# vita-epfl/collaborative-gan-sampling

Measured on AMD Instinct MI355X. Metric: refined samples/sec @ 20 refinement steps, higher is better.
Workload: dtype f32; 1 GPU; dcgan64 collaborative refinement (propose + K-step refine + render), batch 1024/GPU, K=20, momentum rate 0.1, refine at feature [8, 8, 256], random-init weights, z~U(-1,1) seed 2019+rank; global_batch=1024, refine_steps=20, parallelism=single GPU, hipgraph=True, batches_in_flight=2, fused_per_launch=1, sync_bn=False, contraction=f32

## Files before the change

collaborative-gan-sampling_amd/csrc/api.hip:

```cpp
#include <stdarg.h>
#include <stdio.h>

#include "cgs_internal.h"

static thread_local char g_err[512] = "";
static thread_local const char* g_last_kernel = "";

static thread_local double g_last_flops = 0.0;
static thread_local int g_last_tail[2] = {0, 0};
void cgs_note_tail(int tiles, int split) { g_last_tail[0] = tiles; g_last_tail[1] = split; }
static thread_local int g_contraction = CGS_CONTRACTION_F32;
int cgs_contraction_mode() { return g_contraction; }

void cgs_note_kernel(const char* name) { g_last_kernel = name; }
void cgs_note_flops(double f) { g_last_flops = f; }
void cgs_add_flops(double f) { g_last_flops += f; }

int cgs_set_error(int code, const char* fmt, ...) {
    va_list ap;
    va_start(ap, fmt);
    vsnprintf(g_err, sizeof(g_err), fmt, ap);
    va_end(ap);
    return code;
}

extern "C" {

int cgs_version(void) { return 116; }
const char* cgs_last_error(void) { return g_err; }
const char* cgs_last_kernel(void) { return g_last_kernel; }
double cgs_last_executed_flops(void) { return g_last_flops; }
int cgs_last_tail_tiles(void) { return g_last_tail[0]; }
int cgs_last_tail_split(void) { return g_last_tail[1]; }
int cgs_set_contraction(int mode) {
    if (mode < CGS_CONTRACTION_F32 || mode > CGS_CONTRACTION_BX6_ALL) return cgs_set_error(CGS_EINVAL, "set_contraction: mode %d", mode);
    g_contraction = mode;
    return CGS_OK;
}
int cgs_get_contraction(void) { return g_contraction; }

}

struct ConvCall { CgsLayer L; bool dirT, deconv, bwd; };

static ConvCall conv_call_of(int op, int H, int W, int Cin, int Ho, int Wo, int Cout, int kh, int kw, int sh, int sw) {
    ConvCall c;
    c.deconv = (op == CGS_DECONV_FWD || op == CGS_DECONV_BWD_DATA);
    c.bwd = (op == CGS_CONV_BWD_DATA || op == CGS_DECONV_BWD_DATA);
    c.dirT = (op == CGS_CONV_BWD_DATA || op == CGS_DECONV_FWD);
    CgsLayer& L = c.L;
    L.kh = kh; L.kw = kw; L.sh = sh; L.sw = sw;
    if (!c.deconv) { L.Hb = H; L.Wb = W; L.Cb = Cin; L.Hs = cgs_ceil_div(H, sh > 0 ? sh : 1); L.Ws = cgs_ceil_div(W, sw > 0 ? sw : 1); L.Cs = Cout; }
    else { L.Hs = H; L.Ws = W; L.Cs = Cin; L.Hb = Ho; L.Wb = Wo; L.Cb = Cout; }
    return c;
}

static int check_layer(const CgsLayer& L, const char* who) {
    if (L.kh <= 0 || L.kw <= 0 || L.sh <= 0 || L.sw <= 0 || L.Hb <= 0 || L.Wb <= 0 || L.Cb <= 0 || L.Cs <= 0)
        return cgs_set_error(CGS_EINVAL, "%s: non-positive dimension", who);
    if (L.Hs != cgs_ceil_div(L.Hb, L.sh) || L.Ws != cgs_ceil_div(L.Wb, L.sw))
        return cgs_set_error(CGS_EINVAL, "%s: 'SAME' geometry mismatch: big %dx%d stride %dx%d needs small %dx%d, got %dx%d", who,
                             L.Hb, L.Wb, L.sh, L.sw, cgs_ceil_div(L.Hb, L.sh), cgs_ceil_div(L.Wb, L.sw), L.Hs, L.Ws);
    return CGS_OK;
}

static IgemmParams igemm_geometry(const CgsLayer& L, bool dirT, int B, int epilogue) {
    IgemmParams p{};
    p.B = B; p.epilogue = epilogue;
    if (!dirT) cgs_geom_F(L, p);
    else if (L.sh <= 2 && L.sw <= 2) cgs_geom_T(L, p);
    return p;
}

static size_t in_image_floats(const IgemmParams& p) { return (size_t)p.Hin * p.Win * p.Cred; }
static size_t out_image_floats(const IgemmParams& p) { return (size_t)p.Hout * p.Wout * p.N; }
static size_t images_per_launch(const IgemmParams& p) {
    const size_t in_img = in_image_floats(p) * 4, out_img = out_image_floats(p) * 4;
    return 0x7fffffffUL / (in_img > out_img ? in_img : out_img);
}
static bool whole_batch_in_one_launch(const IgemmParams& p) { return images_per_launch(p) >= (size_t)p.B; }

static bool smalln_ok(const CgsLayer& L, int epilogue) {
    return L.Cb <= 4 && L.sh == 2 && L.sw == 2 && L.Hb == 2 * L.Hs && L.Wb == 2 * L.Ws && (L.Cs % 4) == 0 &&
           epilogue != CGS_EPI_AFFINE_RELU;
}

static int choose_family(const CgsLayer& L, bool dirT, const IgemmParams& g, bool have_ws, size_t ws_bytes, bool in_al, bool ws_al,
                         bool rest_al) {
    const int B = g.B, epilogue = g.epilogue;
    if (dirT && smalln_ok(L, epilogue)) {
        if ((L.Cs % 16) == 0 && have_ws && cgs_convt_quad_fits(L)) return CGS_FAMILY_QUAD;
        if (epilogue < CGS_EPI_RELU_BWD_AFFINE) return CGS_FAMILY_SMALLN_T;
    }
    if (!dirT && cgs_conv_smalln_f_ok(L, B, epilogue) && have_ws && ws_bytes >= cgs_conv_smalln_f_ws_floats(L) * sizeof(float) &&
        in_al && ws_al)
        return CGS_FAMILY_SMALLN_F;
    if (!dirT && cgs_conv_taps_ok(L, epilogue)) return CGS_FAMILY_TAPS;
    if (!dirT && cgs_conv_dot_ok(L, epilogue) && in_al) return CGS_FAMILY_DOT;
    const bool patch_f = !dirT && cgs_conv_patch_ok(L, epilogue), patch_t = dirT && cgs_conv_patch_T_ok(L);
    if ((patch_f || patch_t) && have_ws && ws_bytes >= cgs_conv_patch_ws_floats(L, dirT) * sizeof(float) && ws_al && rest_al)
        return CGS_FAMILY_PATCH;
    if (g_contraction != CGS_CONTRACTION_F32 && cgs_igemm_bx6_ok(L, dirT, B, g_contraction == CGS_CONTRACTION_BX6_ALL)) {
        if (have_ws && ws_bytes >= cgs_igemm_bx6_packed_bytes(g)) return CGS_FAMILY_IGEMM_BX6;
    }
    return CGS_FAMILY_IGEMM;
}

static int planned_family(const ConvCall& c, const IgemmParams& g, size_t ws_bytes) { return choose_family(c.L, c.dirT, g, ws_bytes > 0, ws_bytes, true, true, true); }

struct NsArgs { const float *mean, *invstd, *gamma, *beta; float leak; int group_images; };

enum ConvForm { FORM_PLAIN, FORM_STATS, FORM_NSTATS, FORM_SIGNS };
struct ConvExtras {
    ConvForm form = FORM_PLAIN;
    float* stat_part = nullptr; size_t stat_part_bytes = 0;
    NsArgs ns = {};
    unsigned* sign_out = nullptr; const unsigned* aux_signs = nullptr;
};

static int run_dir(const ConvCall& c, int B, const float* in, const float* w, const float* bias, float* out, int epilogue,
                   const float* ep_a, const float* ep_b, const float* ep_aux, void* ws, size_t ws_bytes, int prepacked, hipStream_t s,
                   const char* who, const ConvExtras& x) {
    const CgsLayer& L = c.L;
    const bool dirT = c.dirT, nstats = x.form == FORM_NSTATS;
    cgs_note_flops(0.0);
    cgs_note_tail(0, 0);
    if (B <= 0) return cgs_set_error(CGS_EINVAL, "%s: B=%d", who, B);
    if (!in || !w || !out) return cgs_set_error(CGS_EINVAL, "%s: null tensor", who);
    if (epilogue < CGS_EPI_NONE || epilogue > CGS_EPI_TANH_BWD) return cgs_set_error(CGS_EINVAL, "%s: epilogue %d", who, epilogue);
    if (epilogue == CGS_EPI_AFFINE_RELU && (!ep_a || !ep_b)) return cgs_set_error(CGS_EINVAL, "%s: affine epilogue needs a,b", who);
    if (epilogue >= CGS_EPI_RELU_BWD_AFFINE && ((!ep_aux && !x.aux_signs) || (epilogue == CGS_EPI_RELU_BWD_AFFINE && !ep_a)))
        return cgs_set_error(CGS_EINVAL, "%s: backward epilogue %d needs aux%s", who, epilogue, epilogue == CGS_EPI_RELU_BWD_AFFINE ? " and a" : "");
    if (dirT && (L.sh > 2 || L.sw > 2)) return cgs_set_error(CGS_EINVAL, "%s: transposed direction supports stride <= 2", who);
    const bool rest_al = !(((uintptr_t)out & 15) || ((uintptr_t)bias & 15) || ((uintptr_t)ep_a & 15) || ((uintptr_t)ep_b & 15) ||
                           ((uintptr_t)ep_aux & 15));
    IgemmParams p = igemm_geometry(L, dirT, B, epilogue);
    const int fam = choose_family(L, dirT, p, ws != nullptr, ws_bytes, !((uintptr_t)in & 15), !((uintptr_t)ws & 15), rest_al);
    if (x.stat_part && fam != CGS_FAMILY_IGEMM && fam != CGS_FAMILY_IGEMM_BX6) return cgs_set_error(CGS_EINVAL, "%s: fused statistics are an implicit-GEMM feature (see cgs_conv_stat_partials)", who);
    if (nstats && (!x.stat_part || fam != CGS_FAMILY_IGEMM)) return cgs_set_error(CGS_EINVAL, "%s: norm-backward statistics are a feature of the exact-fp32 implicit GEMM (see cgs_conv_stat_layout)", who);
    if (x.sign_out && fam != CGS_FAMILY_IGEMM && fam != CGS_FAMILY_IGEMM_BX6) return cgs_set_error(CGS_EINVAL, "%s: this call cannot leave a sign mask (see cgs_conv_signs_ok)", who);
    if (x.aux_signs && fam != CGS_FAMILY_PATCH && fam != CGS_FAMILY_TAPS) return cgs_set_error(CGS_EINVAL, "%s: this call cannot take a sign mask (see cgs_conv_signs_ok)", who);
    if (((uintptr_t)x.sign_out & 3) || ((uintptr_t)x.aux_signs & 3)) return cgs_set_error(CGS_EINVAL, "%s: sign mask must be 4-byte aligned", who);
    switch (fam) {
        case CGS_FAMILY_QUAD:
            return cgs_convt_quad_launch(L, B, in, w, bias, out, epilogue, ep_a, ep_aux, (float*)ws, ws_bytes, prepacked, s);
        case CGS_FAMILY_SMALLN_T:
            return cgs_convt_smalln_launch(L, B, in, w, bias, out, epilogue, s);
        case CGS_FAMILY_SMALLN_F:
            return cgs_conv_smalln_f_launch(L, B, in, w, bias, out, epilogue, (float*)ws, ws_bytes, prepacked, s);
        case CGS_FAMILY_DOT:
            return cgs_conv_dot_launch(L, B, in, w, bias, out, epilogue, ep_a, ep_b, s);
        case CGS_FAMILY_TAPS:
            return cgs_conv_taps_launch(L, B, in, w, bias, out, epilogue, ep_a, ep_b, ep_aux, x.aux_signs, s);
        case CGS_FAMILY_PATCH:
            return cgs_conv_patch_launch(L, dirT, B, in, w, bias, out, epilogue, ep_a, ep_b, ep_aux, (float*)ws, ws_bytes, prepacked, s, x.aux_signs);
        default: break;
    }
    p.in = in; p.bias = bias; p.ep_a = ep_a; p.ep_b = ep_b; p.ep_aux = ep_aux; p.out = out;
    p.stat_part = x.stat_part;
    if (nstats) { p.ns_mean = x.ns.mean; p.ns_inv = x.ns.invstd; p.ns_gamma = x.ns.gamma; p.ns_beta = x.ns.beta; p.ns_leak = x.ns.leak; p.ns_gimg = x.ns.group_images >= B ? 0 : x.ns.group_images; }
    p.sign_out = x.sign_out;
    p.sign_plane = (long)B * (dirT ? L.Hb * L.Wb : L.Hs * L.Ws);
    const bool bx6 = fam == CGS_FAMILY_IGEMM_BX6;
    const size_t need = bx6 ? cgs_igemm_bx6_packed_bytes(p) : cgs_packed_floats(p) * sizeof(float);
    if (!ws || ws_bytes < need) return cgs_set_error(CGS_EWORKSPACE, "%s: workspace %zu < %zu bytes", who, ws_bytes, need);
    if (((uintptr_t)ws & 15) || ((uintptr_t)in & 15) || ((uintptr_t)out & 15) || ((uintptr_t)bias & 15) ||
        ((uintptr_t)ep_a & 15) || ((uintptr_t)ep_b & 15) || ((uintptr_t)ep_aux & 15))
        return cgs_set_error(CGS_EINVAL, "%s: pointers must be 16-byte aligned", who);
    p.wp = (const float*)ws;
    if (!prepacked) {
        int rc = bx6 ? cgs_pack_weights_bx6(p, L, dirT, w, ws, s) : cgs_pack_weights(p, L, dirT, w, (float*)ws, s);
        if (rc) return rc;
    }
    const size_t chunk = images_per_launch(p), in_img = in_image_floats(p), out_img = out_image_floats(p);
    if (chunk < 1) return cgs_set_error(CGS_EINVAL, "%s: one image exceeds 2 GiB", who);
    if (x.stat_part && !whole_batch_in_one_launch(p)) return cgs_set_error(CGS_EINVAL, "%s: fused statistics need the batch in one launch", who);
    for (size_t b0 = 0; b0 < (size_t)B; b0 += chunk) {
        p.B = (int)(B - b0 < chunk ? B - b0 : chunk);
        p.in = in + b0 * in_img;
        p.out = out + b0 * out_img;
        p.ep_aux = ep_aux ? ep_aux + b0 * out_img : nullptr;
        p.sign_out = x.sign_out ? x.sign_out + b0 * p.Hout * p.Wout : nullptr;
        int rc = bx6 ? cgs_igemm_bx6_launch(p, s) : cgs_igemm_launch(p, (char*)ws + need, ws_bytes - need, s);
        if (rc) return rc;
    }
    return CGS_OK;
}

struct ConvPlan { int fam; ConvCall c; IgemmParams g; };

static ConvPlan conv_plan_of(int op, int B, int H, int W, int Cin, int Ho, int Wo, int Cout, int kh, int kw, int sh, int sw, int epilogue,
                             size_t ws_bytes) {
    ConvPlan q{};
    if (op < CGS_CONV_FWD || op > CGS_DECONV_BWD_DATA || B <= 0 || H <= 0 || W <= 0 || Cin <= 0 || Cout <= 0 || kh <= 0 || kw <= 0 ||
        sh <= 0 || sw <= 0) {
        q.fam = cgs_set_error(CGS_EINVAL, "conv_family: bad argument");
    } else {
        q.c = conv_call_of(op, H, W, Cin, Ho, Wo, Cout, kh, kw, sh, sw);
        q.g = igemm_geometry(q.c.L, q.c.dirT, B, epilogue);
        q.fam = planned_family(q.c, q.g, ws_bytes);
    }
    return q;
}

static int nstats_check(const char* who, const float* x_norm, const NsArgs& ns, const float* stat_part) {
    if (!x_norm || !ns.mean || !ns.invstd || !ns.gamma || !ns.beta) return cgs_set_error(CGS_EINVAL, "%s: null statistics argument", who);
    if (((uintptr_t)x_norm | (uintptr_t)ns.mean | (uintptr_t)ns.invstd | (uintptr_t)ns.gamma | (uintptr_t)ns.beta | (uintptr_t)stat_part) & 15)
        return cgs_set_error(CGS_EINVAL, "%s: pointers must be 16-byte aligned", who);
    return CGS_OK;
}

static int conv_entry(const char* who, int op, const float* in, const float* w, const float* bias, float* out, int B, int H, int W, int Cin,
                      int Ho, int Wo, int Cout, int kh, int kw, int sh, int sw, int epilogue, const float* ep_a, const float* ep_b,
                      const float* ep_aux, void* ws, size_t ws_bytes, int prepacked, void* stream, const ConvExtras& x = ConvExtras()) {
    const ConvCall c = conv_call_of(op, H, W, Cin, Ho, Wo, Cout, kh, kw, sh, sw);
    if (x.form == FORM_SIGNS) {
        if (!x.sign_out && !x.aux_signs) return cgs_set_error(CGS_EINVAL, "%s: null sign mask", who);
        if (!cgs_conv_signs_ok(op, B, H, W, Cin, Ho, Wo, Cout, kh, kw, sh, sw, epilogue, ws_bytes))
            return cgs_set_error(CGS_EINVAL, "%s: not available for this call (cgs_conv_signs_ok == 0)", who);
    }
    if (x.form == FORM_PLAIN && c.bwd && epilogue != CGS_EPI_NONE && epilogue < CGS_EPI_RELU_BWD_AFFINE)
        return cgs_set_error(CGS_EINVAL, "%s: epilogue %d", who, epilogue);
    int rc = check_layer(c.L, who);
    if (rc) return rc;
    if (x.form == FORM_STATS || x.form == FORM_NSTATS) {
        const bool conv_fwd = x.form == FORM_STATS && !c.deconv;
        int a, b, d;
        const int G = conv_fwd ? cgs_conv_stat_partials(B, H, W, Cin, Cout, kh, kw, sh, sw, ws_bytes)
                               : cgs_conv_stat_layout(op, B, H, W, Cin, Ho, Wo, Cout, kh, kw, sh, sw, x.form == FORM_NSTATS ? x.ns.group_images : B,
                                                      ws_bytes, &a, &b, &d);
        if (G == 0) return cgs_set_error(CGS_EINVAL, "%s: not available for this call (%s == 0)", who, conv_fwd ? "cgs_conv_stat_partials" : "cgs_conv_stat_layout");
        if (x.form == FORM_NSTATS && (rc = nstats_check(who, ep_aux, x.ns, x.stat_part))) return rc;
        const size_t need = (size_t)G * 2 * (c.bwd ? Cin : Cout) * sizeof(float);
        if (!x.stat_part || x.stat_part_bytes < need) return cgs_set_error(CGS_EWORKSPACE, "%s: partials buffer %zu < %zu bytes", who, x.stat_part_bytes, need);
        if ((uintptr_t)x.stat_part & 15) return cgs_set_error(CGS_EINVAL, "%s: partials buffer must be 16-byte aligned", who);
    }
    return run_dir(c, B, in, w, bias, out, epilogue, ep_a, ep_b, ep_aux, ws, ws_bytes, prepacked, (hipStream_t)stream, who, x);
}

extern "C" {

size_t cgs_conv_ws_bytes(int op, int kh, int kw, int sh, int sw, int Cin, int Cout) {
    if (kh <= 0 || kw <= 0 || sh <= 0 || sw <= 0 || Cin <= 0 || Cout <= 0) return 0;
    const ConvCall c = conv_call_of(op, 0, 0, Cin, 0, 0, Cout, kh, kw, sh, sw);
    const int Cb = c.L.Cb, Cs = c.L.Cs;
    const bool dirT = c.dirT;
    const int Cred = dirT ? Cs : Cb, Nn = dirT ? Cb : Cs;
    const size_t per_w = ((Cred % 32) == 0 && (Nn % 64) == 0 && kh <= 16 && kw <= 16) ? 6 : sizeof(float);
    if (!dirT) return (size_t)cgs_round_up(kh * kw * Cb, CGS_BK) * cgs_round_up(Cs, 64) * per_w;
    size_t n = 0;
    for (int a = 0; a < sh; ++a)
        for (int b = 0; b < sw; ++b) {
            const int nty = a < kh ? (kh - a + sh - 1) / sh : 0, ntx = b < kw ? (kw - b + sw - 1) / sw : 0;
            n += (size_t)cgs_round_up(nty * ntx * Cs, CGS_BK) * cgs_round_up(Cb, 64);
        }
    if (Cb <= 4 && sh == 2 && sw == 2) {
        const size_t q = cgs_convt_quad_ws_floats_bound(kh, kw, Cs);
        if (q > n) n = q;
    }
    return n * (per_w > sizeof(float) && !(Cb <= 4 && sh == 2 && sw == 2) ? per_w : sizeof(float));
}

size_t cgs_conv_ws_bytes_for(int op, int B, int H, int W, int Cin, int Cout, int kh, int kw, int sh, int sw) {
    const size_t packed = cgs_conv_ws_bytes(op, kh, kw, sh, sw, Cin, Cout);
    if (B <= 0 || H <= 0 || W <= 0 || packed == 0) return packed;
    const ConvCall c = conv_call_of(op, H, W, Cin, H * sh, W * sw, Cout, kh, kw, sh, sw);
    if (c.dirT && (sh > 2 || sw > 2)) return packed;
    return packed + cgs_igemm_slab_bytes(igemm_geometry(c.L, c.dirT, B, CGS_EPI_NONE));
}

int cgs_conv_family(int op, int B, int H, int W, int Cin, int Ho, int Wo, int Cout, int kh, int kw, int sh, int sw, int epilogue,
                    size_t ws_bytes) {
    return conv_plan_of(op, B, H, W, Cin, Ho, Wo, Cout, kh, kw, sh, sw, epilogue, ws_bytes).fam;
}

int cgs_conv_stat_partials(int B, int H, int W, int Cin, int Cout, int kh, int kw, int sh, int sw, size_t ws_bytes) {
    const ConvCall c = conv_call_of(CGS_CONV_FWD, H, W, Cin, 0, 0, Cout, kh, kw, sh, sw);
    if (check_layer(c.L, "conv_stat_partials")) return 0;
    const IgemmParams g = igemm_geometry(c.L, c.dirT, B, CGS_EPI_NONE);
    const int fam = planned_family(c, g, ws_bytes);
    if (B <= 0 || (Cout & 3) || (fam != CGS_FAMILY_IGEMM && fam != CGS_FAMILY_IGEMM_BX6)) return 0;
    if (!whole_batch_in_one_launch(g)) return 0;
    const long M = (long)B * c.L.Hs * c.L.Ws;
    return (int)(2 * ((M + 127) / 128));
}

int cgs_conv_stat_layout(int op, int B, int H, int W, int Cin, int Ho, int Wo, int Cout, int kh, int kw, int sh, int sw, int group_images,
                         size_t ws_bytes, int* rows_per_seg, int* nseg, int* seg_stride) {
    if (op < CGS_CONV_FWD || op > CGS_DECONV_BWD_DATA || B <= 0 || group_images <= 0 || (B % group_images) || !rows_per_seg || !nseg || !seg_stride)
        return 0;
    const ConvCall c = conv_call_of(op, H, W, Cin, Ho, Wo, Cout, kh, kw, sh, sw);
    if ((c.bwd ? Cin : Cout) & 3) return 0;
    if (check_layer(c.L, "conv_stat_layout")) return 0;
    if (c.dirT && (sh > 2 || sw > 2)) return 0;
    const IgemmParams p = igemm_geometry(c.L, c.dirT, B, CGS_EPI_NONE);
    const int fam = planned_family(c, p, ws_bytes);
    if (fam != CGS_FAMILY_IGEMM && (c.bwd || fam != CGS_FAMILY_IGEMM_BX6)) return 0;
    if (!whole_batch_in_one_launch(p)) return 0;
    const int RC = p.cls[0].R * p.cls[0].C;
    for (int i = 1; i < p.nclasses; ++i)
        if (p.cls[i].R * p.cls[i].C != RC) return 0;
    if (RC <= 0) return 0;
    const long M = (long)B * RC;
    const long cls_rows = 2 * ((M + 127) / 128);
    if (cls_rows * p.nclasses > 0x7fffffffL) return 0;
    if (group_images == B) {
        *rows_per_seg = (int)(cls_rows * p.nclasses); *nseg = 1; *seg_stride = 0;
        return (int)(cls_rows * p.nclasses);
    }
    const int order = cgs_igemm_row_order(p);
    if (order == 0) {
        if (((long)group_images * RC) % 64) return 0;
        *rows_per_seg = (int)((long)group_images * RC / 64); *nseg = p.nclasses; *seg_stride = (int)cls_rows;
    } else if (order == 2) {
        if (group_images % 64) return 0;
        *rows_per_seg = group_images / 64; *nseg = p.nclasses * RC; *seg_stride = B / 64;
    } else {
        return 0;
    }
    return (int)(cls_rows * p.nclasses);
}

int cgs_conv_signs_ok(int op, int B, int H, int W, int Cin, int Ho, int Wo, int Cout, int kh, int kw, int sh, int sw, int epilogue,
                      size_t ws_bytes) {
    const ConvPlan q = conv_plan_of(op, B, H, W, Cin, Ho, Wo, Cout, kh, kw, sh, sw, epilogue, ws_bytes);
    const int fam = q.fam;
    if (fam < 0) return 0;
    if (epilogue >= CGS_EPI_RELU_BWD_AFFINE)
        return (fam == CGS_FAMILY_PATCH && cgs_conv_patch_signs_ok(q.c.L, q.c.dirT, epilogue)) || (fam == CGS_FAMILY_TAPS && cgs_conv_taps_signs_ok(q.c.L, epilogue));
    if (fam == CGS_FAMILY_IGEMM_BX6)
        return (epilogue == CGS_EPI_AFFINE_RELU || epilogue == CGS_EPI_LRELU) && whole_batch_in_one_launch(q.g);
    if (fam != CGS_FAMILY_IGEMM || (q.c.dirT && (sh > 2 || sw > 2))) return 0;
    if (!whole_batch_in_one_launch(q.g)) return 0;
    return cgs_igemm_signs_ok(q.g);
}

int cgs_conv2d_nhwc_fwd(const float* x, const float* w, const float* bias, float* y, int B, int H, int W, int Cin,
                        int Cout, int kh, int kw, int sh, int sw, int epilogue, const float* ep_a, const float* ep_b,
                        void* ws, size_t ws_bytes, int ws_prepacked, void* stream) {
    return conv_entry("conv2d_nhwc_fwd", CGS_CONV_FWD, x, w, bias, y, B, H, W, Cin, 0, 0, Cout, kh, kw, sh, sw, epilogue, ep_a, ep_b, nullptr, ws, ws_bytes,
                      ws_prepacked, stream);
}

int cgs_conv2d_nhwc_bwd_data(const float* dy, const float* w, float* dx, int B, int H, int W, int Cin, int Cout, int kh,
                             int kw, int sh, int sw, int epilogue, const float* ep_a, const float* ep_aux, void* ws,
                             size_t ws_bytes, int ws_prepacked, void* stream) {
    return conv_entry("conv2d_nhwc_bwd_data", CGS_CONV_BWD_DATA, dy, w, nullptr, dx, B, H, W, Cin, 0, 0, Cout, kh, kw, sh, sw, epilogue, ep_a, nullptr, ep_aux, ws,
                      ws_bytes, ws_prepacked, stream);
}

int cgs_deconv2d_nhwc_fwd(const float* x, const float* w, const float* bias, float* y, int B, int H, int W, int Cin,
                          int Ho, int Wo, int Cout, int kh, int kw, int sh, int sw, int epilogue, const float* ep_a,
                          const float* ep_b, void* ws, size_t ws_bytes, int ws_prepacked, void* stream) {
    return conv_entry("deconv2d_nhwc_fwd", CGS_DECONV_FWD, x, w, bias, y, B, H, W, Cin, Ho, Wo, Cout, kh, kw, sh, sw, epilogue, ep_a, ep_b, nullptr, ws, ws_bytes,
                      ws_prepacked, stream);
}

int cgs_deconv2d_nhwc_bwd_data(const float* dy, const float* w, float* dx, int B, int H, int W, int Cin, int Ho, int Wo,
                               int Cout, int kh, int kw, int sh, int sw, int epilogue, const float* ep_a,
                               const float* ep_aux, void* ws, size_t ws_bytes, int ws_prepacked, void* stream) {
    return conv_entry("deconv2d_nhwc_bwd_data", CGS_DECONV_BWD_DATA, dy, w, nullptr, dx, B, H, W, Cin, Ho, Wo, Cout, kh, kw, sh, sw, epilogue, ep_a, nullptr, ep_aux,
                      ws, ws_bytes, ws_prepacked, stream);
}

int cgs_conv2d_nhwc_fwd_stats(const float* x, const float* w, const float* bias, float* y, int B, int H, int W, int Cin,
                              int Cout, int kh, int kw, int sh, int sw, void* ws, size_t ws_bytes, int ws_prepacked,
                              float* stat_part, size_t stat_part_bytes, void* stream) {
    return conv_entry("conv2d_nhwc_fwd_stats", CGS_CONV_FWD, x, w, bias, y, B, H, W, Cin, 0, 0, Cout, kh, kw, sh, sw, CGS_EPI_NONE, nullptr, nullptr, nullptr, ws,
                      ws_bytes, ws_prepacked, stream, ConvExtras{FORM_STATS, stat_part, stat_part_bytes});
}

int cgs_deconv2d_nhwc_fwd_stats(const float* x, const float* w, const float* bias, float* y, int B, int H, int W, int Cin, int Ho, int Wo,
                                int Cout, int kh, int kw, int sh, int sw, void* ws, size_t ws_bytes, int ws_prepacked, float* stat_part,
                                size_t stat_part_bytes, void* stream) {
    return conv_entry("deconv2d_nhwc_fwd_stats", CGS_DECONV_FWD, x, w, bias, y, B, H, W, Cin, Ho, Wo, Cout, kh, kw, sh, sw, CGS_EPI_NONE, nullptr, nullptr, nullptr,
                      ws, ws_bytes, ws_prepacked, stream, ConvExtras{FORM_STATS, stat_part, stat_part_bytes});
}

int cgs_conv2d_nhwc_bwd_data_nstats(const float* dy, const float* w, float* dx, int B, int H, int W, int Cin, int Cout, int kh, int kw, int sh,
                                    int sw, const float* x_norm, const float* mean, const float* invstd, const float* gamma, const float* beta,
                                    float leak, int group_images, void* ws, size_t ws_bytes, int ws_prepacked, float* stat_part,
                                    size_t stat_part_bytes, void* stream) {
    return conv_entry("conv2d_nhwc_bwd_data_nstats", CGS_CONV_BWD_DATA, dy, w, nullptr, dx, B, H, W, Cin, 0, 0, Cout, kh, kw, sh, sw, CGS_EPI_NONE, nullptr, nullptr,
                      x_norm, ws, ws_bytes, ws_prepacked, stream, ConvExtras{FORM_NSTATS, stat_part, stat_part_bytes, NsArgs{mean, invstd, gamma, beta, leak,
                      group_images}});
}

int cgs_deconv2d_nhwc_bwd_data_nstats(const float* dy, const float* w, float* dx, int B, int H, int W, int Cin, int Ho, int Wo, int Cout, int kh,
                                      int kw, int sh, int sw, const float* x_norm, const float* mean, const float* invstd, const float* gamma,
                                      const float* beta, float leak, int group_images, void* ws, size_t ws_bytes, int ws_prepacked,
                                      float* stat_part, size_t stat_part_bytes, void* stream) {
    return conv_entry("deconv2d_nhwc_bwd_data_nstats", CGS_DECONV_BWD_DATA, dy, w, nullptr, dx, B, H, W, Cin, Ho, Wo, Cout, kh, kw, sh, sw, CGS_EPI_NONE, nullptr,
                      nullptr, x_norm, ws, ws_bytes, ws_prepacked, stream, ConvExtras{FORM_NSTATS, stat_part, stat_part_bytes, NsArgs{mean, invstd, gamma, beta,
                      leak, group_images}});
}

int cgs_deconv2d_nhwc_fwd_signs(const float* x, const float* w, const float* bias, float* y, int B, int H, int W, int Cin,
                                int Ho, int Wo, int Cout, int kh, int kw, int sh, int sw, int epilogue, const float* ep_a,
                                const float* ep_b, unsigned* signs, void* ws, size_t ws_bytes, int ws_prepacked, void* stream) {
    return conv_entry("deconv2d_nhwc_fwd_signs", CGS_DECONV_FWD, x, w, bias, y, B, H, W, Cin, Ho, Wo, Cout, kh, kw, sh, sw, epilogue, ep_a, ep_b, nullptr, ws,
                      ws_bytes, ws_prepacked, stream, ConvExtras{FORM_SIGNS, nullptr, 0, NsArgs{}, signs, nullptr});
}

int cgs_deconv2d_nhwc_bwd_data_signs(const float* dy, const float* w, float* dx, int B, int H, int W, int Cin, int Ho, int Wo,
                                     int Cout, int kh, int kw, int sh, int sw, int epilogue, const float* ep_a,
                                     const unsigned* aux_signs, void* ws, size_t ws_bytes, int ws_prepacked, void* stream) {
    return conv_entry("deconv2d_nhwc_bwd_data_signs", CGS_DECONV_BWD_DATA, dy, w, nullptr, dx, B, H, W, Cin, Ho, Wo, Cout, kh, kw, sh, sw, epilogue, ep_a, nullptr,
                      nullptr, ws, ws_bytes, ws_prepacked, stream, ConvExtras{FORM_SIGNS, nullptr, 0, NsArgs{}, nullptr, aux_signs});
}

}

__global__ __launch_bounds__(256) void linear_out1_fwd_kernel(const float* __restrict__ x, const float* __restrict__ w,
                                                              const float* __restrict__ bias, float* __restrict__ y,
                                                              int B, int K, int epilogue) {
    const int b = blockIdx.x * 4 + (threadIdx.x >> 6);
    const int lane = threadIdx.x & 63;
    if (b >= B) return;
    const float* row = x + (size_t)b * K;
    float s = 0.f;
    if ((K & 3) == 0) {
        for (int k = lane * 4; k < K; k += 256) {
            const float4 a = *(const float4*)(row + k), ww = *(const float4*)(w + k);
            s = fmaf(a.x, ww.x, s); s = fmaf(a.y, ww.y, s); s = fmaf(a.z, ww.z, s); s = fmaf(a.w, ww.w, s);
        }
    } else {
        for (int k = lane; k < K; k += 64) s = fmaf(row[k], w[k], s);
    }
#pragma unroll
    for (int off = 32; off > 0; off >>= 1) s += __shfl_down(s, off, 64);
    if (lane == 0) {
        float v = s + (bias ? bias[0] : 0.f);
        if (epilogue == CGS_EPI_LRELU) v = fmaxf(v, 0.2f * v);
        y[b] = v;
    }
}

template <int KIND, bool LADAM>
__device__ __forceinline__ void linear_out1_seed_body(const float* __restrict__ x, const float* __restrict__ w, const float* __restrict__ bias,
                                                      float* __restrict__ y, float* __restrict__ dl, float* __restrict__ lm, int B, int K,
                                                      const cgs_ladam_seed& la) {
    const int b = blockIdx.x * 4 + (threadIdx.x >> 6);
    const int lane = threadIdx.x & 63;
    if (b >= B) return;
    const float* row = x + (size_t)b * K;
    float s = 0.f;
    if ((K & 3) == 0) {
        for (int k = lane * 4; k < K; k += 256) {
            const float4 a = *(const float4*)(row + k), ww = *(const float4*)(w + k);
            s = fmaf(a.x, ww.x, s); s = fmaf(a.y, ww.y, s); s = fmaf(a.z, ww.z, s); s = fmaf(a.w, ww.w, s);
        }
    } else {
        for (int k = lane; k < K; k += 64) s = fmaf(row[k], w[k], s);
    }
#pragma unroll
    for (int off = 32; off > 0; off >>= 1) s += __shfl_down(s, off, 64);
    if (lane == 0) {
        const float v = s + (bias ? bias[0] : 0.f);
        y[b] = v;
        dl[b] = loss_seed1<KIND>(v);
        lm[b] = v;
        if (LADAM) ladam_seed1(la, b, sigmoid_stable(v));
    }
}

__global__ __launch_bounds__(256) void linear_out1_bce_kernel(const float* __restrict__ x, const float* __restrict__ w, const float* __restrict__ bias,
                                                              float* __restrict__ y, float* __restrict__ dl, float* __restrict__ lm, int B, int K) {
    linear_out1_seed_body<CGS_LOSS_BCE, false>(x, w, bias, y, dl, lm, B, K, cgs_ladam_seed{});
}

template <int KIND, bool LADAM>
__global__ __launch_bounds__(256) void linear_out1_seed_kernel(const float* __restrict__ x, const float* __restrict__ w, const float* __restrict__ bias,
                                                               float* __restrict__ y, float* __restrict__ dl, float* __restrict__ lm, int B, int K,
                                                               cgs_ladam_seed la) {
    linear_out1_seed_body<KIND, LADAM>(x, w, bias, y, dl, lm, B, K, la);
}

// ... 66 lines not shown
```

collaborative-gan-sampling_amd/csrc/cgs_internal.h:

```cpp
#pragma once
#include <hip/hip_runtime.h>
#include <stddef.h>
#include <stdint.h>

#include "cgs_hip.h"

int cgs_set_error(int code, const char* fmt, ...);
void cgs_note_kernel(const char* name);
void cgs_note_flops(double executed);
void cgs_add_flops(double executed);
void cgs_note_tail(int tiles, int split);

#define CGS_CHECK_LAUNCH(name)                                                        \
    do {                                                                              \
        hipError_t e_ = hipGetLastError();                                            \
        if (e_ != hipSuccess) return cgs_set_error(CGS_ELAUNCH, "%s: %s", name, hipGetErrorString(e_)); \
    } while (0)

static inline int cgs_ceil_div(int a, int b) { return (a + b - 1) / b; }
static inline int cgs_round_up(int a, int b) { return cgs_ceil_div(a, b) * b; }

static inline int cgs_same_pad_before(int size, int k, int s) {
    int out = cgs_ceil_div(size, s);
    int tot = (out - 1) * s + k - size;
    if (tot < 0) tot = 0;
    return tot / 2;
}

struct CgsLayer {
    int kh, kw, sh, sw;
    int Hb, Wb, Cb, Hs, Ws, Cs;
};

#define CGS_BN_MAX_BLOCKS 512
size_t cgs_bn_stat2_offset(int C);
size_t cgs_instnorm_stat2_offset(int B, int HW, int C);
#define CGS_BK 32
#define CGS_MAX_CLASSES 4

struct IgemmClass {
    int R, C;
    int py, px;
    int nty, ntx;
    int dy0, dx0;
    int ky0, kx0;
    int K;
    int w_off;
    int slab_off;
};

struct IgemmParams {
    const float* in;
    const float* wp;
    const float* bias;
    const float* ep_a;
    const float* ep_b;
    const float* ep_aux;
    float* out;
    int B, Hin, Win, Cred;
    int Hout, Wout, N, Np;
    int S, So, dstep, kstep;
    int epilogue;
    int pix_major;
    int splitk;
    float* slab;
    int tap_parity;
    int xcd_map;
    int cls_flip;
    int uni;
    int lpt;
    unsigned* sign_out;
    long sign_plane;
    float* stat_part;
    int stat_cls_rows;
    const float* ns_mean = nullptr;
    const float* ns_inv = nullptr;
    const float* ns_gamma = nullptr;
    const float* ns_beta = nullptr;
    float ns_leak = 1.f;
    int ns_gimg = 0;
    int vec;
    int prio_t[3];
    int tail_from, tail_n, tail_s;
    int nclasses;
    IgemmClass cls[CGS_MAX_CLASSES];
    unsigned char perm[CGS_MAX_CLASSES][256];
};

__host__ __device__ inline int cgs_tap_order(int i, int n, int parity_first) {
    if (!parity_first) return i;
    const int ne = (n + 1) >> 1;
    return i < ne ? 2 * i : 2 * (i - ne) + 1;
}

void cgs_geom_F(const CgsLayer& L, IgemmParams& p);
void cgs_geom_T(const CgsLayer& L, IgemmParams& p);
size_t cgs_packed_floats(const IgemmParams& p);

int cgs_pack_weights(const IgemmParams& p, const CgsLayer& L, bool dirT, const float* w, float* packed, hipStream_t s);
int cgs_igemm_launch(const IgemmParams& p, void* slab, size_t slab_bytes, hipStream_t s);
size_t cgs_igemm_splitk_bytes(const IgemmParams& p);
size_t cgs_igemm_slab_bytes(const IgemmParams& p);
void cgs_igemm_row_policy(IgemmParams& p, int BM);
void cgs_igemm_count_flops(const IgemmParams& p, int BM);
int cgs_igemm_bx6_ok(const CgsLayer& L, bool dirT, int B, bool any_size);
size_t cgs_igemm_bx6_packed_bytes(const IgemmParams& p);
int cgs_pack_weights_bx6(const IgemmParams& p, const CgsLayer& L, bool dirT, const float* w, void* packed, hipStream_t s);
int cgs_igemm_bx6_launch(const IgemmParams& p, hipStream_t s);
int cgs_contraction_mode();
int cgs_igemm_row_order(const IgemmParams& p);
size_t cgs_convt_quad_ws_floats_bound(int kh, int kw, int Cs);
int cgs_convt_taps_ok(const CgsLayer& L);
int cgs_convt_taps_launch(const CgsLayer& L, int B, const float* in, const float* w, const float* bias, float* out, int epilogue,
                          const float* ep_a, const float* ep_aux, hipStream_t s);
int cgs_conv_dot_ok(const CgsLayer& L, int epilogue);
int cgs_conv_dot_launch(const CgsLayer& L, int B, const float* in, const float* w, const float* bias, float* out, int epilogue,
                        const float* ep_a, const float* ep_b, hipStream_t s);
int cgs_conv_taps_ok(const CgsLayer& L, int epilogue);
int cgs_conv_taps_signs_ok(const CgsLayer& L, int epilogue);
int cgs_conv_taps_launch(const CgsLayer& L, int B, const float* in, const float* w, const float* bias, float* out, int epilogue,
                         const float* ep_a, const float* ep_b, const float* ep_aux, const unsigned* aux_signs, hipStream_t s);
int cgs_convt_quad_launch(const CgsLayer& L, int B, const float* in, const float* w, const float* bias, float* out,
                          int epilogue, const float* ep_a, const float* ep_aux, float* ws, size_t ws_bytes, int prepacked,
                          hipStream_t s);
int cgs_convt_smalln_launch(const CgsLayer& L, int B, const float* in, const float* w, const float* bias,
                            float* out, int epilogue, hipStream_t s);

#ifdef __HIPCC__
__device__ __forceinline__ float epilogue_apply(float v, int mode, float a, float b, float aux) {
    switch (mode) {
        case CGS_EPI_LRELU: return fmaxf(v, 0.2f * v);
        case CGS_EPI_AFFINE_RELU: return fmaxf(fmaf(a, v, b), 0.f);
        case CGS_EPI_TANH: return tanhf(v);
        case CGS_EPI_RELU_BWD_AFFINE: return aux > 0.f ? v * a : 0.f;
        case CGS_EPI_LRELU_BWD: return aux > 0.f ? v : 0.2f * v;
        case CGS_EPI_TANH_BWD: return v * (1.f - aux * aux);
        default: return v;
    }
}

__device__ __forceinline__ float norm_fwd1(float x, float sc, float sh, float leak) {
    const float o = fmaf(x, sc, sh);
    return o > 0.f ? o : leak * o;
}
__device__ __forceinline__ float norm_d1(float x, float dy, float sc, float sh, float leak) {
    const float u = fmaf(x, sc, sh);
    return dy * (u > 0.f ? 1.f : leak);
}
__device__ __forceinline__ float norm_d_acc1(float x, float dy, float mu, float inv, float sc, float sh, float leak, float& sa, float& sb) {
    const float d = norm_d1(x, dy, sc, sh, leak);
    sa += d; sb = fmaf(d, (x - mu) * inv, sb);
    return d;
}
__device__ __forceinline__ float norm_dx1(float x, float d, float mu, float inv, float sc, float m1, float m2) {
    const float xh = (x - mu) * inv;
    return sc * (d - m1 - xh * m2);
}

__device__ __forceinline__ float sigmoid_stable(float v) { return v >= 0.f ? 1.f / (1.f + expf(-v)) : expf(v) / (1.f + expf(v)); }
template <int KIND>
__device__ __forceinline__ float loss_seed1(float v) {
    if (KIND == CGS_LOSS_BCE) return v >= 0.f ? -expf(-v) / (1.f + expf(-v)) : -1.f / (1.f + expf(v));
    if (KIND == CGS_LOSS_LSQ) return 2.f * (v - 1.f);
    return -1.f;
}
__device__ __forceinline__ void ladam_seed1(const cgs_ladam_seed& la, int b, float sig, const float* loss_in = nullptr) {
#pragma clang fp contract(off)
    const float loss = loss_in ? loss_in[b] : la.s_real[0] - sig;
    const float avg = la.first ? loss : 0.5f * la.loss_avg[b] + 0.5f * loss;
    la.loss_avg[b] = avg;
    const float c = fminf(fmaxf(avg + 0.5f, 0.f), 10000.f);
    la.gain[b] = c * c;
}
#endif


#define CGS_SMEM_ATTR(bytes, who, ...)                                                                                  \
    do {                                                                                                                \
        static bool smem_done_[64] = {};                                                                                \
        int smem_dev_ = 0;                                                                                              \
        (void)hipGetDevice(&smem_dev_);                                                                                 \
        smem_dev_ &= 63;                                                                                                \
        if (!smem_done_[smem_dev_]) {                                                                                   \
            hipError_t smem_e_ = hipFuncSetAttribute((const void*)(__VA_ARGS__), hipFuncAttributeMaxDynamicSharedMemorySize, (int)(bytes)); \
            if (smem_e_ != hipSuccess) return cgs_set_error(CGS_ELAUNCH, "%s: MaxDynamicSharedMemorySize: %s", who, hipGetErrorString(smem_e_)); \
            smem_done_[smem_dev_] = true;                                                                               \
        }                                                                                                               \
    } while (0)

int cgs_mlp2d_wide_saliency(const float* const* w, const float* const* b, int nlayers, int nh, const float* x, float* sig, float* sal, int B,
                            float inv_batch, hipStream_t st);
int cgs_refine2d_wide(const float* const* w, const float* const* b, int nlayers, int nh, const float* x, float mean_host,
                      const float* mean_dev, float inv_batch, int steps, float rate, int method, float* best_x, float* best_step,
                      float* traj, int B, hipStream_t st);
size_t cgs_mlp2d_wide_train_ws(int Bt, int nlayers, int nh);
int cgs_mlp2d_wide_train(float* const* w, float* const* b, int nlayers, int nh, const float* real, int B_real, const float* fake, int B_fake,
                         float lr, float* const* gw, float* const* gb, float* loss, void* ws, hipStream_t st);

bool cgs_convt_quad_fits(const CgsLayer& L);
int cgs_conv_smalln_f_ok(const CgsLayer& L, int B, int epilogue);
size_t cgs_conv_smalln_f_ws_floats(const CgsLayer& L);
int cgs_conv_smalln_f_launch(const CgsLayer& L, int B, const float* in, const float* w, const float* bias, float* out,
                             int epilogue, float* ws, size_t ws_bytes, int prepacked, hipStream_t s);
int cgs_conv_patch_ok(const CgsLayer& L, int epilogue);
int cgs_conv_patch_T_ok(const CgsLayer& L);
size_t cgs_conv_patch_ws_floats(const CgsLayer& L, bool dirT);
int cgs_conv_patch_launch(const CgsLayer& L, bool dirT, int B, const float* in, const float* w, const float* bias, float* out,
                          int epilogue, const float* ep_a, const float* ep_b, const float* ep_aux, float* ws, size_t ws_bytes,
                          int prepacked, hipStream_t s, const unsigned* aux_signs = nullptr);
int cgs_conv_patch_signs_ok(const CgsLayer& L, bool dirT, int epilogue);
int cgs_igemm_signs_ok(const IgemmParams& p);
```

collaborative-gan-sampling_amd/csrc/elementwise.hip:

```cpp
#include "cgs_internal.h"

static unsigned ew_blocks(size_t n) {
    size_t b = (n + 255) / 256;
    if (b > 8192) b = 8192;
    if (b == 0) b = 1;
    return (unsigned)b;
}

#define GRID_STRIDE(i, n) for (size_t i = (size_t)blockIdx.x * blockDim.x + threadIdx.x; i < (n); i += (size_t)gridDim.x * blockDim.x)

__global__ void bn_fold_kernel(const float* g, const float* b, const float* mm, const float* mv, float eps, float* a,
                               float* bo, int C) {
    const int c = blockIdx.x * blockDim.x + threadIdx.x;
    if (c >= C) return;
    const float s = g[c] / sqrtf(mv[c] + eps);
    a[c] = s; bo[c] = b[c] - s * mm[c];
}

int cgs_bn_fold(const float* gamma, const float* beta, const float* mm, const float* mv, float eps, float* a, float* b,
                int C, void* stream) {
    if (C <= 0) return cgs_set_error(CGS_EINVAL, "bn_fold: C=%d", C);
    hipLaunchKernelGGL(bn_fold_kernel, dim3(cgs_ceil_div(C, 128)), dim3(128), 0, (hipStream_t)stream, gamma, beta, mm, mv, eps, a, b, C);
    CGS_CHECK_LAUNCH("bn_fold");
    return CGS_OK;
// ... 188 lines not shown
    float s = 0.f;
    for (int i = lane; i < P; i += 64) s += sigmoid_stable(l[(size_t)b * P + i]);
#pragma unroll
    for (int o = 32; o > 0; o >>= 1) s += __shfl_xor(s, o);
    if (lane == 0) sig[b] = s / (float)P;
}

int cgs_sigmoid_rowmean(const float* logits, float* sigmoids, int B, int P, void* stream) {
    if (B <= 0 || P <= 0) return cgs_set_error(CGS_EINVAL, "sigmoid_rowmean: B=%d P=%d", B, P);
    if (P >= 64)
        hipLaunchKernelGGL(sigmoid_rowmean_wave_kernel, dim3(cgs_ceil_div(B, 4)), dim3(256), 0, (hipStream_t)stream, logits, sigmoids, B, P);
    else
        hipLaunchKernelGGL(sigmoid_rowmean_kernel, dim3(cgs_ceil_div(B, 128)), dim3(128), 0, (hipStream_t)stream, logits, sigmoids, B, P);
    CGS_CHECK_LAUNCH("sigmoid_rowmean");
    return CGS_OK;
}

template <int OP>
__global__ __launch_bounds__(256) void loss_unary_kernel(const float* __restrict__ p0, const float* __restrict__ p1, float lo, float hi,
                                                         float* __restrict__ o, size_t n) {
    GRID_STRIDE(i, n) {
        float r;
        if (OP == 0) { const float v = p0[i]; r = fmaxf(-v, 0.f) + log1pf(expf(-fabsf(v))); }
        else if (OP == 1) { const float v = p1[i]; r = p0[i] * (v >= 0.f ? -expf(-v) / (1.f + expf(-v)) : -1.f / (1.f + expf(v))); }
        else r = fminf(fmaxf(p0[i], lo), hi);
        o[i] = r;
    }
}

int cgs_bce_ones_fwd(const float* logits, float* loss, size_t n, void* stream) {
    if (n == 0) return CGS_OK;
    hipLaunchKernelGGL(loss_unary_kernel<0>, dim3(ew_blocks(n)), dim3(256), 0, (hipStream_t)stream, logits, nullptr, 0.f, 0.f, loss, n);
    CGS_CHECK_LAUNCH("bce_ones_fwd");
    return CGS_OK;
}

int cgs_bce_ones_bwd(const float* dloss, const float* logits, float* dlogits, size_t n, void* stream) {
    if (n == 0) return CGS_OK;
    hipLaunchKernelGGL(loss_unary_kernel<1>, dim3(ew_blocks(n)), dim3(256), 0, (hipStream_t)stream, dloss, logits, 0.f, 0.f, dlogits, n);
    CGS_CHECK_LAUNCH("bce_ones_bwd");
    return CGS_OK;
}

template <int KIND>
__global__ __launch_bounds__(256) void gan_loss_kernel(const float* __restrict__ l, float target, const float* __restrict__ dloss,
                                                       float* __restrict__ o, size_t n) {
#pragma clang fp contract(off)
    GRID_STRIDE(i, n) {
        const float v = l[i];
        float e, d;
        if (KIND == CGS_LOSS_LSQ) { const float r = v - target; e = r * r; d = 2.f * r; }
        else if (KIND == CGS_LOSS_HINGE) {
            const float u = target > 0.5f ? 1.f - v : 1.f + v;
            e = fmaxf(u, 0.f);
            d = u > 0.f ? (target > 0.5f ? -1.f : 1.f) : 0.f;
        } else { e = -v; d = -1.f; }
        o[i] = dloss ? dloss[i] * d : e;
    }
}

int cgs_gan_loss(const float* logits, int kind, float target, const float* dloss, float* out, size_t n, void* stream) {
    if (n == 0) return CGS_OK;
    if (!logits || !out) return cgs_set_error(CGS_EINVAL, "gan_loss: null pointer");
    const hipStream_t st = (hipStream_t)stream;
    if (kind == CGS_LOSS_LSQ) hipLaunchKernelGGL(gan_loss_kernel<CGS_LOSS_LSQ>, dim3(ew_blocks(n)), dim3(256), 0, st, logits, target, dloss, out, n);
    else if (kind == CGS_LOSS_HINGE && (target == 0.f || target == 1.f))
        hipLaunchKernelGGL(gan_loss_kernel<CGS_LOSS_HINGE>, dim3(ew_blocks(n)), dim3(256), 0, st, logits, target, dloss, out, n);
    else if (kind == CGS_LOSS_LINEAR) hipLaunchKernelGGL(gan_loss_kernel<CGS_LOSS_LINEAR>, dim3(ew_blocks(n)), dim3(256), 0, st, logits, target, dloss, out, n);
    else return cgs_set_error(CGS_EINVAL, "gan_loss: kind %d target %g", kind, (double)target);
    CGS_CHECK_LAUNCH("gan_loss");
    return CGS_OK;
}

int cgs_clip(const float* x, float vmin, float vmax, float* y, size_t n, void* stream) {
    if (n == 0) return CGS_OK;
    hipLaunchKernelGGL(loss_unary_kernel<2>, dim3(ew_blocks(n)), dim3(256), 0, (hipStream_t)stream, x, nullptr, vmin, vmax, y, n);
    CGS_CHECK_LAUNCH("clip");
    return CGS_OK;
}

__global__ __launch_bounds__(256) void refine_update_kernel(float* __restrict__ theta, float* __restrict__ m,
                                                            const float* __restrict__ g, float rate, float alpha,
                                                            int first, int use_clip, float vmin, float vmax, size_t n) {
#pragma clang fp contract(off)
    GRID_STRIDE(i, n) {
        const float lg = rate * g[i];
        const float am = alpha * m[i];
        const float mv = first ? lg : am + lg;
        m[i] = mv;
        float t = theta[i] - mv;
        if (use_clip) t = fminf(fmaxf(t, vmin), vmax);
        theta[i] = t;
    }
}

int cgs_refine_update(float* theta, float* m, const float* g, float rate, float alpha, int first, int use_clip,
                      float vmin, float vmax, size_t n, void* stream) {
    if (n == 0) return CGS_OK;
    hipLaunchKernelGGL(refine_update_kernel, dim3(ew_blocks(n)), dim3(256), 0, (hipStream_t)stream, theta, m, g, rate, alpha, first, use_clip, vmin, vmax, n);
    CGS_CHECK_LAUNCH("refine_update");
    return CGS_OK;
}

__global__ void ladam_gain_kernel(const float* __restrict__ loss, cgs_ladam_seed la, int B) {
    const int b = blockIdx.x * blockDim.x + threadIdx.x;
    if (b < B) ladam_seed1(la, b, 0.f, loss);
}

int cgs_ladam_gain(const float* loss, float* loss_avg, float* gain, int first, int B, void* stream) {
    if (B <= 0 || !loss || !loss_avg || !gain) return cgs_set_error(CGS_EINVAL, "ladam_gain: B=%d or a null pointer", B);
    hipLaunchKernelGGL(ladam_gain_kernel, dim3(cgs_ceil_div(B, 128)), dim3(128), 0, (hipStream_t)stream, loss, cgs_ladam_seed{nullptr, loss_avg, gain, first}, B);
    CGS_CHECK_LAUNCH("ladam_gain");
    return CGS_OK;
}

__device__ __forceinline__ void ladam_update1(float& th, float& m, float& v, float g, float gain, float rate, float c1, float c2, int first,
                                              int use_clip, float vmin, float vmax) {
#pragma clang fp contract(off)
    const float sq = g * g;
    const float mm = first ? g : 0.9f * m + c1 * g;
    const float vv = first ? sq : 0.5f * v + c2 * sq;
    m = mm; v = vv;
    const float dir = rate * mm / (sqrtf(vv) + 1e-8f);
    float t = th - dir * gain;
    if (use_clip) t = fminf(fmaxf(t, vmin), vmax);
    th = t;
}

template <bool VEC>
__global__ __launch_bounds__(256) void refine_update_ladam_kernel(float* __restrict__ theta, float* __restrict__ m, float* __restrict__ v,
                                                                  const float* __restrict__ g, const float* __restrict__ gain, float rate,
                                                                  float c1, float c2, int first, int use_clip, float vmin, float vmax,
                                                                  size_t n, int F) {
    if (VEC) {
        float4* t4 = (float4*)theta; float4* m4 = (float4*)m; float4* v4 = (float4*)v;
        const float4* g4 = (const float4*)g;
        GRID_STRIDE(i, n >> 2) {
            const float gn = gain[(i << 2) / (size_t)F];
            float4 t = t4[i], mm = first ? float4{0.f, 0.f, 0.f, 0.f} : m4[i], vv = first ? float4{0.f, 0.f, 0.f, 0.f} : v4[i];
            const float4 gg = g4[i];
            ladam_update1(t.x, mm.x, vv.x, gg.x, gn, rate, c1, c2, first, use_clip, vmin, vmax);
            ladam_update1(t.y, mm.y, vv.y, gg.y, gn, rate, c1, c2, first, use_clip, vmin, vmax);
            ladam_update1(t.z, mm.z, vv.z, gg.z, gn, rate, c1, c2, first, use_clip, vmin, vmax);
            ladam_update1(t.w, mm.w, vv.w, gg.w, gn, rate, c1, c2, first, use_clip, vmin, vmax);
            t4[i] = t; m4[i] = mm; v4[i] = vv;
        }
    } else {
        GRID_STRIDE(i, n) {
            float t = theta[i], mm = first ? 0.f : m[i], vv = first ? 0.f : v[i];
            ladam_update1(t, mm, vv, g[i], gain[i / (size_t)F], rate, c1, c2, first, use_clip, vmin, vmax);
            theta[i] = t; m[i] = mm; v[i] = vv;
        }
    }
}

int cgs_refine_update_ladam(float* theta, float* m, float* v, const float* g, const float* gain, float rate, int first, int use_clip,
                            float vmin, float vmax, int B, int F, void* stream) {
    if (B <= 0 || F <= 0 || !theta || !m || !v || !g || !gain) return cgs_set_error(CGS_EINVAL, "refine_update_ladam: B=%d F=%d or a null pointer", B, F);
    const size_t n = (size_t)B * F;
    const float c1 = (float)(1.0 - 0.9), c2 = (float)(1.0 - 0.5);
    const bool vec = (F & 3) == 0 && (((uintptr_t)theta | (uintptr_t)m | (uintptr_t)v | (uintptr_t)g) & 15) == 0;
    if (vec)
        hipLaunchKernelGGL(refine_update_ladam_kernel<true>, dim3(ew_blocks(n >> 2)), dim3(256), 0, (hipStream_t)stream, theta, m, v, g, gain, rate, c1, c2,
                           first, use_clip, vmin, vmax, n, F);
    else
        hipLaunchKernelGGL(refine_update_ladam_kernel<false>, dim3(ew_blocks(n)), dim3(256), 0, (hipStream_t)stream, theta, m, v, g, gain, rate, c1, c2,
                           first, use_clip, vmin, vmax, n, F);
    CGS_CHECK_LAUNCH("refine_update_ladam");
    return CGS_OK;
}

__device__ __forceinline__ void copy_row(const float* __restrict__ src, float* __restrict__ dst, int F, bool vec4) {
    const int t = blockIdx.x * blockDim.x + threadIdx.x, nt = gridDim.x * blockDim.x;
    if (vec4) {
// ... 95 lines not shown
```

collaborative-gan-sampling_amd/csrc/igemm.hip:

```cpp
#include <stdarg.h>
#include <stdio.h>

#include "cgs_internal.h"
#include "igemm_epilogue.h"

typedef float f32x16 __attribute__((ext_vector_type(16)));

static constexpr int BK = CGS_BK;

void cgs_geom_F(const CgsLayer& L, IgemmParams& p) {
    p.Hin = L.Hb; p.Win = L.Wb; p.Cred = L.Cb;
    p.Hout = L.Hs; p.Wout = L.Ws; p.N = L.Cs; p.Np = cgs_round_up(L.Cs, 64);
    p.S = L.sh; p.So = 1; p.dstep = 1; p.kstep = 1; p.nclasses = 1;
    p.tap_parity = (L.sh == 2 && L.sw == 2 && L.Hs * L.Ws > 64) ? 1 : 0;
    IgemmClass& c = p.cls[0];
    c.R = L.Hs; c.C = L.Ws; c.py = 0; c.px = 0; c.nty = L.kh; c.ntx = L.kw;
    c.dy0 = -cgs_same_pad_before(L.Hb, L.kh, L.sh); c.dx0 = -cgs_same_pad_before(L.Wb, L.kw, L.sw);
    c.ky0 = 0; c.kx0 = 0; c.K = L.kh * L.kw * L.Cb; c.w_off = 0;
    p.vec = (p.Cred % BK) == 0 && c.nty <= 16 && c.ntx <= 16;
}

void cgs_geom_T(const CgsLayer& L, IgemmParams& p) {
    p.Hin = L.Hs; p.Win = L.Ws; p.Cred = L.Cs;
    p.Hout = L.Hb; p.Wout = L.Wb; p.N = L.Cb; p.Np = cgs_round_up(L.Cb, 64);
    p.S = 1; p.So = L.sh; p.dstep = -1; p.kstep = L.sh; p.nclasses = L.sh * L.sw;
    p.tap_parity = 0;
    const int pt = cgs_same_pad_before(L.Hb, L.kh, L.sh), pl = cgs_same_pad_before(L.Wb, L.kw, L.sw);
    int off = 0;
    for (int py = 0; py < L.sh; ++py)
        for (int px = 0; px < L.sw; ++px) {
            IgemmClass& c = p.cls[py * L.sw + px];
            c.py = py; c.px = px;
            c.R = py < L.Hb ? (L.Hb - py + L.sh - 1) / L.sh : 0;
            c.C = px < L.Wb ? (L.Wb - px + L.sw - 1) / L.sw : 0;
            c.ky0 = (py + pt) % L.sh; c.kx0 = (px + pl) % L.sw;
            c.nty = c.ky0 < L.kh ? (L.kh - c.ky0 + L.sh - 1) / L.sh : 0;
            c.ntx = c.kx0 < L.kw ? (L.kw - c.kx0 + L.sw - 1) / L.sw : 0;
            c.dy0 = (py + pt - c.ky0) / L.sh; c.dx0 = (px + pl - c.kx0) / L.sw;
            c.K = c.nty * c.ntx * L.Cs; c.w_off = off;
            off += cgs_round_up(c.K, BK) * p.Np;
        }
    p.vec = (p.Cred % BK) == 0;
    for (int i = 0; i < p.nclasses; ++i) p.vec = p.vec && p.cls[i].nty <= 16 && p.cls[i].ntx <= 16;
    for (int i = 1; i < p.nclasses; ++i)
        for (int j = i; j > 0 && p.cls[j].K > p.cls[j - 1].K; --j) { IgemmClass t = p.cls[j]; p.cls[j] = p.cls[j - 1]; p.cls[j - 1] = t; }
}

size_t cgs_packed_floats(const IgemmParams& p) {
    size_t n = 0;
    for (int i = 0; i < p.nclasses; ++i) n += (size_t)cgs_round_up(p.cls[i].K, BK) * p.Np;
    return n;
}

__global__ void pack_weights_kernel(IgemmParams p, const float* __restrict__ w, float* __restrict__ packed,
                                    int kw, int Cb, int Cs, int dirT) {
    const IgemmClass& c = p.cls[blockIdx.y];
    const int Kpad = (c.K + BK - 1) / BK * BK;
    const size_t total = (size_t)Kpad * p.Np;
    for (size_t i = (size_t)blockIdx.x * blockDim.x + threadIdx.x; i < total; i += (size_t)gridDim.x * blockDim.x) {
        const int e = (int)(i & 3);
        const int n = (int)((i >> 2) % p.Np);
        const int k = (int)((i >> 2) / p.Np) * 4 + e;
        float v = 0.f;
        if (k < c.K && n < p.N) {
            int t, ci, ta, tb;
            if (p.vec) {
                const int ntaps = c.nty * c.ntx;
                const int kt = k / BK, chunk = kt / ntaps;
                t = kt - chunk * ntaps; ci = chunk * BK + (k - kt * BK);
                ta = t / c.ntx; tb = t - ta * c.ntx;
                ta = cgs_tap_order(ta, c.nty, p.tap_parity); tb = cgs_tap_order(tb, c.ntx, p.tap_parity);
            } else {
                t = k / p.Cred; ci = k - t * p.Cred;
                ta = t / c.ntx; tb = t - ta * c.ntx;
            }
            const int tap = (c.ky0 + ta * p.kstep) * kw + (c.kx0 + tb * p.kstep);
            const size_t src = dirT ? ((size_t)tap * Cb + n) * Cs + ci
                                    : ((size_t)tap * Cb + ci) * Cs + n;
            v = w[src];
        }
        packed[c.w_off + i] = v;
    }
}

int cgs_pack_weights(const IgemmParams& p, const CgsLayer& L, bool dirT, const float* w, float* packed, hipStream_t s) {
    size_t mx = 0;
    for (int i = 0; i < p.nclasses; ++i) {
        size_t n = (size_t)cgs_round_up(p.cls[i].K, BK) * p.Np;
        if (n > mx) mx = n;
    }
    if (mx == 0) return CGS_OK;
    int blocks = (int)((mx + 255) / 256);
    if (blocks > 4096) blocks = 4096;
    hipLaunchKernelGGL(pack_weights_kernel, dim3(blocks, p.nclasses), dim3(256), 0, s, p, w, packed, L.kw, L.Cb, L.Cs,
                       dirT ? 1 : 0);
    CGS_CHECK_LAUNCH("pack_weights");
    return CGS_OK;
}

template <int BM, int BN, int NW, bool VEC, int TBK, bool PAR, bool NS>
__device__ __forceinline__ void igemm_body(const IgemmParams& p) {
    constexpr int BK = TBK;
    constexpr int LDA = BK + 4;
    constexpr int NT = 64 * NW;
    constexpr int WM = BM / 64;
    constexpr int WN = NW / WM;
    constexpr int TM = BM / (32 * WM), TN = BN / (32 * WN);
    constexpr int QPR = BK / 4;
    constexpr int AI = BM * QPR / NT, BI = BN * QPR / NT;
    constexpr int AR = NT / QPR;
    extern __shared__ __attribute__((aligned(16))) float smem[];
    float* As = smem;
    float* Bs = smem + 2 * BM * LDA;
    constexpr int KLOOP_F = 2 * BM * LDA + 2 * BK * BN;
    constexpr int EH = (VEC && TBK == 16) ? 2 : 1;
    constexpr int STAGE_F = NW * (BM / WM / EH) * (BN / WN + 4);
    int* rowpix = (int*)(smem + (KLOOP_F > STAGE_F ? KLOOP_F : STAGE_F));

    const int nblk_n = p.Np / BN;
    unsigned wi = blockIdx.x;
    int cls_i = blockIdx.y;
    if (p.xcd_map == 2) {
        const unsigned xcd = wi & 7u;
        unsigned q = wi >> 3;
        cls_i = (int)(q % (unsigned)p.nclasses);
        q /= (unsigned)p.nclasses;
        wi = (q << 3) | xcd;
    }
    if (p.cls_flip && (((((unsigned)blockIdx.z * gridDim.y + (unsigned)cls_i) * gridDim.x) >> 8) & 1u)) {
        const int grp = cls_i / p.cls_flip;
        cls_i = grp * p.cls_flip + (p.cls_flip - 1 - (cls_i - grp * p.cls_flip));
    }
    int tsplit = 1, tz = 0, ttile = 0;
    if (p.tail_s > 1 && cls_i == p.nclasses - 1 && wi >= (unsigned)p.tail_from) {
        const unsigned t = wi - (unsigned)p.tail_from;
        ttile = (int)(t / (unsigned)p.tail_s); tz = (int)(t - (unsigned)ttile * (unsigned)p.tail_s); tsplit = p.tail_s;
        if (ttile >= p.tail_n) return;
        wi = (unsigned)p.tail_from + (unsigned)ttile;
    }
    int nb, mb;
    if (p.xcd_map) {
        const unsigned xcd = wi & 7u, q = wi >> 3;
        nb = (int)(q % (unsigned)nblk_n);
        mb = (int)(q / (unsigned)nblk_n) * 8 + (int)xcd;
    } else {
        nb = (int)(wi % (unsigned)nblk_n);
        mb = (int)(wi / (unsigned)nblk_n);
    }
    const IgemmClass& c = p.cls[cls_i];
    const int RC = c.R * c.C;
    const int M = p.B * RC;
    if (mb * BM >= M) return;
    if (p.lpt) {
        const int gpp = p.B / BM;
        const int rank = mb / gpp, grp = mb - rank * gpp;
        mb = (int)p.perm[cls_i][rank] * gpp + grp;
    }
    const int m0 = mb * BM, n0 = nb * BN;

    const int tid = threadIdx.x;
    __builtin_amdgcn_s_setprio(3);
    const int lane = tid & 63, wave = tid >> 6;
    const int wm = wave / WN, wn = wave - wm * WN;
    const int h = lane >> 5, j = lane & 31;

    const int mlast_ = m0 + BM - 1 < M ? m0 + BM - 1 : M - 1;
    const bool one_pix = p.pix_major && (m0 / p.B) == (mlast_ / p.B);
    const int t_pix = one_pix ? m0 / p.B : 0;
    const int t_b0 = m0 - t_pix * p.B, t_r = t_pix / c.C, t_cc = t_pix - (t_pix / c.C) * c.C;
#define DECODE_ROW(m_, b_, r_, cc_)                                        \
    do {                                                                   \
        if (one_pix) { b_ = t_b0 + ((m_) - m0); r_ = t_r; cc_ = t_cc; }    \
        else {                                                             \
            int rem_;                                                      \
            if (p.pix_major) { rem_ = (m_) / p.B; b_ = (m_) - rem_ * p.B; } \
            else { b_ = (m_) / RC; rem_ = (m_) - b_ * RC; }                \
            r_ = rem_ / c.C; cc_ = rem_ - r_ * c.C;                        \
        }                                                                  \
    } while (0)

    if (tid < BM) {
        const int m = m0 + tid;
        int pix = -1;
        if (m < M) {
// ... 377 lines not shown
            LOAD_TILE(kl);
#pragma unroll
            for (int jj = 1; jj < NG - 1; ++jj) MFMA_GROUP(jj);
            STORE_TILE(buf ^ 1);
            if (NG > 1) MFMA_GROUP(NG - 1);
            __syncthreads();
            kt = kn;
        }
    }
#undef KIT_SEL
#undef FRAG_READ
#undef MFMA_EXEC
#undef ADDR_TILE_V
#undef ISSUE_TILE_V
#undef ADDR_TILE_U
#undef ISSUE_TILE_U
#undef PRIO_STEP
#undef MFMA_GROUP

#undef LOAD_TILE
#undef STORE_TILE
#undef DECODE_ROW
    __builtin_amdgcn_s_setprio(3);
    if (tsplit > 1) {
        float* slab = p.slab + ((size_t)ttile * tsplit + tz) * (BM * BN);
#pragma unroll
        for (int tn = 0; tn < TN; ++tn) {
            const int nl = wn * (BN / WN) + tn * 32 + j;
#pragma unroll
            for (int tm = 0; tm < TM; ++tm)
#pragma unroll
                for (int r = 0; r < 16; ++r) {
                    const int ml = wm * (BM / WM) + tm * 32 + (r & 3) + 8 * (r >> 2) + 4 * h;
                    slab[ml * BN + nl] = acc[tm][tn][r];
                }
        }
        return;
    }
    if (p.splitk > 1) {
        float* slab = p.slab + c.slab_off + (size_t)blockIdx.z * M * p.Np;
#pragma unroll
        for (int tn = 0; tn < TN; ++tn) {
            const int n = n0 + wn * (BN / WN) + tn * 32 + j;
#pragma unroll
            for (int tm = 0; tm < TM; ++tm)
#pragma unroll
                for (int r = 0; r < 16; ++r) {
                    const int m = m0 + wm * (BM / WM) + tm * 32 + (r & 3) + 8 * (r >> 2) + 4 * h;
                    if (m < M) slab[(size_t)m * p.Np + n] = acc[tm][tn][r];
                }
        }
        return;
    }
    constexpr int WTN = BN / WN;
    if ((p.N & 3) == 0) {
        constexpr int LDE = WTN + 4;
        constexpr int ER = BM / WM / EH;
        float* E = smem + wave * ER * LDE;
        constexpr int LPR = WTN / 4;
        constexpr int RPP = 64 / LPR;
        const int c4 = (lane % LPR) * 4, rsub = lane / LPR;
        const int n = n0 + wn * WTN + c4;
        f32x4 bias = {0.f, 0.f, 0.f, 0.f}, ea = {1.f, 1.f, 1.f, 1.f}, eb = {0.f, 0.f, 0.f, 0.f};
        if (n < p.N) {
            if (p.bias) bias = *(const f32x4*)(p.bias + n);
            if (p.epilogue == CGS_EPI_AFFINE_RELU) { ea = *(const f32x4*)(p.ep_a + n); eb = *(const f32x4*)(p.ep_b + n); }
            if (p.epilogue == CGS_EPI_RELU_BWD_AFFINE) ea = *(const f32x4*)(p.ep_a + n);
        }
        f32x4 st_a = {0.f, 0.f, 0.f, 0.f}, st_b = {0.f, 0.f, 0.f, 0.f};
#pragma unroll
        for (int ph = 0; ph < EH; ++ph) {
#pragma unroll
            for (int tm = ph * (TM / EH); tm < (ph + 1) * (TM / EH); ++tm)
#pragma unroll
                for (int tn = 0; tn < TN; ++tn)
#pragma unroll
                    for (int r = 0; r < 16; ++r)
                        E[((tm - ph * (TM / EH)) * 32 + (r & 3) + 8 * (r >> 2) + 4 * h) * LDE + tn * 32 + j] = acc[tm][tn][r];
            __builtin_amdgcn_fence(__ATOMIC_RELEASE, "wavefront");
            __builtin_amdgcn_wave_barrier();
            __builtin_amdgcn_fence(__ATOMIC_ACQUIRE, "wavefront");
            if (n < p.N) {
                const int* rp = rowpix + wm * (BM / WM) + ph * ER;
                if constexpr (NS) {
                    const int mw = min(m0 + wm * (BM / WM), M - 1);
                    const int grp = p.ns_gimg <= 0 ? 0 : (p.pix_major ? (mw % p.B) : (mw / RC)) / p.ns_gimg;
                    const NsLane ns = ns_lane_params(p, grp, n);
                    epilogue_rows<CGS_EPI_NONE, ER, RPP, LDE, 2, ((VEC && TBK == 32) ? 4 : 1)>(p, E, rp, rsub, c4, n, bias, ea, eb, &st_a, &st_b, &ns);
                } else if (p.stat_part) {
                    epilogue_rows<CGS_EPI_NONE, ER, RPP, LDE, 1>(p, E, rp, rsub, c4, n, bias, ea, eb, &st_a, &st_b);
                } else if (p.sign_out) {
                    if (p.epilogue == CGS_EPI_AFFINE_RELU) epilogue_rows_signs<CGS_EPI_AFFINE_RELU, ER, RPP, LDE, true>(p, E, rp, rsub, c4, n, bias, ea, eb);
                    else epilogue_rows_signs<CGS_EPI_LRELU, ER, RPP, LDE, true>(p, E, rp, rsub, c4, n, bias, ea, eb);
                } else
                switch (p.epilogue) {
                    case CGS_EPI_NONE: epilogue_rows<CGS_EPI_NONE, ER, RPP, LDE>(p, E, rp, rsub, c4, n, bias, ea, eb); break;
                    case CGS_EPI_LRELU: epilogue_rows<CGS_EPI_LRELU, ER, RPP, LDE>(p, E, rp, rsub, c4, n, bias, ea, eb); break;
                    case CGS_EPI_AFFINE_RELU: epilogue_rows<CGS_EPI_AFFINE_RELU, ER, RPP, LDE>(p, E, rp, rsub, c4, n, bias, ea, eb); break;
                    case CGS_EPI_TANH: epilogue_rows<CGS_EPI_TANH, ER, RPP, LDE>(p, E, rp, rsub, c4, n, bias, ea, eb); break;
                    case CGS_EPI_RELU_BWD_AFFINE: epilogue_rows<CGS_EPI_RELU_BWD_AFFINE, ER, RPP, LDE>(p, E, rp, rsub, c4, n, bias, ea, eb); break;
                    case CGS_EPI_LRELU_BWD: epilogue_rows<CGS_EPI_LRELU_BWD, ER, RPP, LDE>(p, E, rp, rsub, c4, n, bias, ea, eb); break;
                    default: epilogue_rows<CGS_EPI_TANH_BWD, ER, RPP, LDE>(p, E, rp, rsub, c4, n, bias, ea, eb); break;
                }
            }
            if (ph + 1 < EH) {
                __builtin_amdgcn_fence(__ATOMIC_RELEASE, "wavefront");
                __builtin_amdgcn_wave_barrier();
                __builtin_amdgcn_fence(__ATOMIC_ACQUIRE, "wavefront");
            }
        }
        if (p.stat_part) {
#pragma unroll
            for (int off = LPR; off < 64; off <<= 1)
#pragma unroll
                for (int e = 0; e < 4; ++e) { st_a[e] += __shfl_xor(st_a[e], off); st_b[e] += __shfl_xor(st_b[e], off); }
            if (rsub == 0 && n < p.N) {
                float* dst = p.stat_part + ((size_t)(cls_i * p.stat_cls_rows + m0 / 64 + wm) * 2) * p.N + n;
                *(f32x4*)dst = st_a;
                *(f32x4*)(dst + p.N) = st_b;
            }
        }
        return;
    }
#pragma unroll
    for (int tn = 0; tn < TN; ++tn) {
        const int n = n0 + wn * WTN + tn * 32 + j;
        if (n >= p.N) continue;
        const float bias = p.bias ? p.bias[n] : 0.f;
        float ea = 1.f, eb = 0.f;
        if (p.epilogue == CGS_EPI_AFFINE_RELU) { ea = p.ep_a[n]; eb = p.ep_b[n]; }
        if (p.epilogue == CGS_EPI_RELU_BWD_AFFINE) ea = p.ep_a[n];
        const bool use_aux = p.epilogue >= CGS_EPI_RELU_BWD_AFFINE;
#pragma unroll
        for (int tm = 0; tm < TM; ++tm)
#pragma unroll
            for (int r = 0; r < 16; ++r) {
                const int row = wm * (BM / WM) + tm * 32 + (r & 3) + 8 * (r >> 2) + 4 * h;
                const int pix = rowpix[row];
                if (pix >= 0) {
                    const size_t o = (size_t)pix * p.N + n;
                    const float aux = use_aux ? p.ep_aux[o] : 0.f;
                    p.out[o] = epilogue_apply(acc[tm][tn][r] + bias, p.epilogue, ea, eb, aux);
                }
            }
    }
}

template <int BM, int BN, int NW, bool VEC, int TBK, bool PAR>
__global__ __launch_bounds__(64 * NW, 2) void igemm_kernel(IgemmParams p) { igemm_body<BM, BN, NW, VEC, TBK, PAR, false>(p); }
template <int BM, int BN, int NW, bool VEC, int TBK, bool PAR>
__global__ __launch_bounds__(64 * NW, 2) void igemm_ns_kernel(IgemmParams p) { igemm_body<BM, BN, NW, VEC, TBK, PAR, true>(p); }

__global__ __launch_bounds__(256) void splitk_reduce_kernel(IgemmParams p) {
    const IgemmClass& c = p.cls[blockIdx.y];
    const int RC = c.R * c.C;
    const int M = p.B * RC;
    const int nq = p.Np / 4;
    const long total = (long)M * nq;
    const float* slab = p.slab + c.slab_off;
    const int g = threadIdx.x & 3;
    const long stride = (long)gridDim.x * (blockDim.x >> 2);
    const long total_pad = (total + stride - 1) / stride * stride;
    for (long i = (long)blockIdx.x * (blockDim.x >> 2) + (threadIdx.x >> 2); i < total_pad; i += stride) {
        const bool live = i < total;
        const int m = live ? (int)(i / nq) : 0, n = live ? (int)(i - (long)m * nq) * 4 : 0;
        f32x4 a = {0.f, 0.f, 0.f, 0.f};
        if (live)
            for (int sidx = g; sidx < p.splitk; sidx += 4) a += *(const f32x4*)(slab + ((size_t)sidx * M + m) * p.Np + n);
#pragma unroll
        for (int e = 0; e < 4; ++e) {
            a[e] += __shfl_xor(a[e], 1);
            a[e] += __shfl_xor(a[e], 2);
        }
        if (!live || g != 0) continue;
        int b, r, cc, rem;
        if (p.pix_major) { rem = m / p.B; b = m - rem * p.B; } else { b = m / RC; rem = m - b * RC; }
        r = rem / c.C; cc = rem - r * c.C;
        const size_t o = (size_t)((b * p.Hout + r * p.So + c.py) * p.Wout + cc * p.So + c.px) * p.N;
#pragma unroll
        for (int e = 0; e < 4; ++e) {
            if (n + e >= p.N) break;
            const float bias = p.bias ? p.bias[n + e] : 0.f;
            float ea = 1.f, eb = 0.f;
            if (p.epilogue == CGS_EPI_AFFINE_RELU) { ea = p.ep_a[n + e]; eb = p.ep_b[n + e]; }
            if (p.epilogue == CGS_EPI_RELU_BWD_AFFINE) ea = p.ep_a[n + e];
            const float aux = p.epilogue >= CGS_EPI_RELU_BWD_AFFINE ? p.ep_aux[o + n + e] : 0.f;
            p.out[o + n + e] = epilogue_apply(a[e] + bias, p.epilogue, ea, eb, aux);
        }
    }
}

__global__ __launch_bounds__(256) void splitk_reduce_stats_kernel(IgemmParams p) {
    const int cls_i = blockIdx.z;
    const IgemmClass& c = p.cls[cls_i];
    const int RC = c.R * c.C;
    const int M = p.B * RC;
    const float* slab = p.slab + c.slab_off;
    const int cq = threadIdx.x & 7, rl = threadIdx.x >> 3;
    const int n = blockIdx.y * 32 + cq * 4;
    __shared__ f32x4 red[2][32][8];
    f32x4 sa = {0.f, 0.f, 0.f, 0.f}, sb = {0.f, 0.f, 0.f, 0.f};
    if (n < p.N) {
        f32x4 bias = {0.f, 0.f, 0.f, 0.f};
        if (p.bias) bias = *(const f32x4*)(p.bias + n);
#pragma unroll
        for (int i = 0; i < 2; ++i) {
            const int m = blockIdx.x * 64 + i * 32 + rl;
            if (m >= M) continue;
            f32x4 a = *(const f32x4*)(slab + (size_t)m * p.Np + n);
#pragma unroll 4
            for (int z = 1; z < p.splitk; ++z) a += *(const f32x4*)(slab + ((size_t)z * M + m) * p.Np + n);
            int b, rem;
            if (p.pix_major) { rem = m / p.B; b = m - rem * p.B; } else { b = m / RC; rem = m - b * RC; }
            const int r = rem / c.C, cc = rem - r * c.C;
            const size_t o = (size_t)((b * p.Hout + r * p.So + c.py) * p.Wout + cc * p.So + c.px) * p.N + n;
            const f32x4 y = a + bias;
            *(f32x4*)(p.out + o) = y;
            if (p.ns_mean) {
                const int grp = p.ns_gimg <= 0 ? 0 : b / p.ns_gimg;
                const NsLane ns = ns_lane_params(p, grp, n);
                const f32x4 xv = *(const f32x4*)(p.ep_aux + o);
#pragma unroll
                for (int e = 0; e < 4; ++e) {
                    const float u = fmaf(xv[e], ns.sc[e], ns.sh[e]);
                    const float d = y[e] * (u > 0.f ? 1.f : ns.leak);
                    sa[e] += d; sb[e] = fmaf(d, (xv[e] - ns.mu[e]) * ns.inv[e], sb[e]);
                }
            } else {
#pragma unroll
                for (int e = 0; e < 4; ++e) { sa[e] += y[e]; sb[e] = fmaf(y[e], y[e], sb[e]); }
            }
        }
    }
    red[0][rl][cq] = sa; red[1][rl][cq] = sb;
    __syncthreads();
    if (rl < 2 && n < p.N) {
        f32x4 t = red[rl][0][cq];
#pragma unroll 8
        for (int r = 1; r < 32; ++r) t += red[rl][r][cq];
        *(f32x4*)(p.stat_part + ((size_t)(cls_i * p.stat_cls_rows + blockIdx.x) * 2 + rl) * p.N + n) = t;
    }
}

#define TAIL_RSPLIT 16
__global__ __launch_bounds__(256) void tail_reduce_kernel(IgemmParams p, int BM, int BN) {
    const int cls_i = p.nclasses - 1;
    const IgemmClass& c = p.cls[cls_i];
    const int RC = c.R * c.C, M = p.B * RC;
    const int nblk_n = p.Np / BN;
    const unsigned wi = (unsigned)p.tail_from + blockIdx.x;
    int nb, mb;
    if (p.xcd_map) {
        const unsigned xcd = wi & 7u, q = wi >> 3;
        nb = (int)(q % (unsigned)nblk_n);
        mb = (int)(q / (unsigned)nblk_n) * 8 + (int)xcd;
    } else {
        nb = (int)(wi % (unsigned)nblk_n);
        mb = (int)(wi / (unsigned)nblk_n);
    }
    if (mb * BM >= M) return;
    if (p.lpt) {
        const int gpp = p.B / BM;
        const int rank = mb / gpp, grp = mb - rank * gpp;
        mb = (int)p.perm[cls_i][rank] * gpp + grp;
    }
    const int m0 = mb * BM, n0 = nb * BN;
    const float* slab = p.slab + (size_t)blockIdx.x * p.tail_s * (BM * BN);
    const int qpr = BN / 4;
    const int cq = threadIdx.x % qpr, rstep = 256 / qpr;
    const int rbeg = blockIdx.y * (BM / TAIL_RSPLIT), rend = rbeg + BM / TAIL_RSPLIT;
    const int r0 = rbeg + threadIdx.x / qpr;
    const int n = n0 + cq * 4;
    if (n >= p.N) return;
    f32x4 bias = {0.f, 0.f, 0.f, 0.f}, ea = {1.f, 1.f, 1.f, 1.f}, eb = {0.f, 0.f, 0.f, 0.f};
    if (p.bias) bias = *(const f32x4*)(p.bias + n);
    if (p.epilogue == CGS_EPI_AFFINE_RELU) { ea = *(const f32x4*)(p.ep_a + n); eb = *(const f32x4*)(p.ep_b + n); }
    if (p.epilogue == CGS_EPI_RELU_BWD_AFFINE) ea = *(const f32x4*)(p.ep_a + n);
    for (int rl = r0; rl < rend; rl += rstep) {
        const int m = m0 + rl;
        if (m >= M) break;
        f32x4 a = *(const f32x4*)(slab + rl * BN + cq * 4);
        for (int z = 1; z < p.tail_s; ++z) a += *(const f32x4*)(slab + (size_t)z * (BM * BN) + rl * BN + cq * 4);
        int b, rem;
        if (p.pix_major) { rem = m / p.B; b = m - rem * p.B; } else { b = m / RC; rem = m - b * RC; }
        const int r = rem / c.C, cc = rem - r * c.C;
        const size_t o = (size_t)((b * p.Hout + r * p.So + c.py) * p.Wout + cc * p.So + c.px) * p.N + n;
        f32x4 aux = {0.f, 0.f, 0.f, 0.f};
        if (p.epilogue >= CGS_EPI_RELU_BWD_AFFINE) aux = *(const f32x4*)(p.ep_aux + o);
        f32x4 y;
#pragma unroll
        for (int e = 0; e < 4; ++e) y[e] = epilogue_apply(a[e] + bias[e], p.epilogue, ea[e], eb[e], aux[e]);
        *(f32x4*)(p.out + o) = y;
    }
}

static long igemm_blocks(const IgemmParams& p, int BN, int BM = 128) {
    long blocks = 0;
    for (int i = 0; i < p.nclasses; ++i) blocks += (((long)p.B * p.cls[i].R * p.cls[i].C + BM - 1) / BM) * (p.Np / BN);
    return blocks;
}

static int choose_splitk(const IgemmParams& p) {
    const int BN = (p.Np % 128) == 0 ? 128 : 64;
    const long blocks = igemm_blocks(p, BN);
    int nk_min = 1 << 30;
    for (int i = 0; i < p.nclasses; ++i) {
        const int nk = cgs_ceil_div(p.cls[i].K, BK);
        if (p.cls[i].R * p.cls[i].C > 0 && nk < nk_min) nk_min = nk;
    }
    if (blocks == 0 || blocks >= 256 || nk_min < 8) return 1;
    long cap = nk_min / 4;
    if (cap > 64) cap = 64;
    if (cap < 2) return 1;
    int nk_max = 0;
    double slice_mb = 0.0;
    long maxM = 0;
    for (int i = 0; i < p.nclasses; ++i) {
        const long m = (long)p.B * p.cls[i].R * p.cls[i].C;
        if (m <= 0) continue;
        const int nk = cgs_ceil_div(p.cls[i].K, BK);
        if (nk > nk_max) nk_max = nk;
        if (m > maxM) maxM = m;
        slice_mb += (double)m * p.Np * 4e-6;
    }
    const double tile = (BN == 128 ? 1.0 : 0.5) * (maxM <= 64 ? 0.5 : 1.0);
    int best = 1;
    double best_cost = 1e30;
    for (long s = 2; s <= cap; ++s) {
        const long cps = (nk_max + s - 1) / s;
        if ((nk_max + cps - 1) / cps != s) continue;
        const long load = (blocks * s + 255) / 256;
        const double cost = (load == 1 ? 1.41 : (double)load) * (double)cps * tile + 0.3 * slice_mb * (double)s;
        if (cost < best_cost) { best_cost = cost; best = (int)s; }
    }
    return best;
}

struct IgemmTiles { bool wide, mid, deep, tall, wide_for_tail; };
struct IgemmTail { int from, n, s; };
static IgemmTail igemm_choose_tail(const IgemmParams& p, const IgemmTiles& t);

#define IGEMM_CUS 256
static bool igemm_round_rules_apply() {
    static int cus = -1;
    if (cus < 0) {
        int dev = 0, n = 0;
        if (hipGetDevice(&dev) != hipSuccess || hipDeviceGetAttribute(&n, hipDeviceAttributeMultiprocessorCount, dev) != hipSuccess) n = 0;
        cus = n;
    }
    return cus == IGEMM_CUS || cus == 0;
}

static IgemmTiles igemm_choose_tiles(const IgemmParams& p, bool tail_wide = true) {
    const bool vec = p.vec != 0;
    int maxRC = 0;
    for (int i = 0; i < p.nclasses; ++i) maxRC = p.cls[i].R * p.cls[i].C > maxRC ? p.cls[i].R * p.cls[i].C : maxRC;
    bool wide = (p.Np % 128) == 0, wide_for_tail = false;
    if (wide && p.lpt && maxRC <= 64) {
        long blocks = 0;
        for (int i = 0; i < p.nclasses; ++i) blocks += ((long)p.B * p.cls[i].R * p.cls[i].C / 128) * (p.Np / 128);
        if (blocks < 1024) wide = false;
        if (!wide && tail_wide && vec && p.splitk == 1 && !p.stat_part && !p.sign_out && (p.N & 3) == 0 && p.nclasses == 1 && blocks >= 512 && blocks <= 1024 &&
            (blocks % 256) != 0 && (blocks % 256) <= 176 && igemm_choose_tail(p, IgemmTiles{true, false, false, false, true}).s > 1) {
            wide = true;
            wide_for_tail = true;
        }
    }
    bool mid = false;
    if (wide && vec && p.splitk == 1) {
        const long wb = igemm_blocks(p, 128);
        if (wb >= 256 && wb < 512) { wide = false; mid = true; }
        else if (wb < 256 && (p.stat_part || p.sign_out)) { wide = false; mid = true; }
    }
    bool deep = true;
    if (vec && p.splitk == 1 && !mid) {
        long min_blocks = 1L << 40, tot_blocks = 0;
        for (int i = 0; i < p.nclasses; ++i) {
            const long m = (long)p.B * p.cls[i].R * p.cls[i].C;
            if (m > 0) { const long bl = (m + 127) / 128 * (p.Np / (wide ? 128 : 64)); if (bl < min_blocks) min_blocks = bl; tot_blocks += bl; }
        }
        deep = min_blocks < 512;
        if (deep && !p.pix_major && p.nclasses > 1 && tot_blocks >= 1024) deep = false;
    }
    bool tall = false;
    {
        int kmax = 0;
        for (int i = 0; i < p.nclasses; ++i) kmax = p.cls[i].K > kmax ? p.cls[i].K : kmax;
        tall = vec && !wide && !mid && !deep && p.splitk == 1 && p.Np == 64 && p.pix_major && (p.B % 256) == 0 && kmax <= 512 &&
               igemm_blocks(p, 64, 256) >= 1536;
    }
    return IgemmTiles{wide, mid, deep, tall, wide_for_tail && wide};
}

static int igemm_blocks_per_cu(bool wide, bool deep) { return deep ? (wide ? 2 : 3) : (wide ? 4 : 5); }

static IgemmTail igemm_choose_tail(const IgemmParams& p, const IgemmTiles& t) {
    IgemmTail none{0, 0, 0};
    if (!igemm_round_rules_apply()) return none;
    if (!p.vec || p.splitk > 1 || p.stat_part || p.sign_out || (p.N & 3) || t.tall) return none;
    const int bn = t.wide ? 128 : 64, tbk = t.deep ? 32 : 16;
    const IgemmClass& cl = p.cls[p.nclasses - 1];
    const long Ml = (long)p.B * cl.R * cl.C;
    if (Ml <= 0) return none;
    const long mtl = (Ml + 127) / 128, Tl = mtl * (p.Np / bn);
    const long T = igemm_blocks(p, bn);
    const long L = 256L * igemm_blocks_per_cu(t.wide, t.deep);
    const int nk = cgs_ceil_div(cl.K, tbk);
    if (T < 256) return none;
    if (T > L) return none;
    long r = T % 256;
    if (r == 0 || r > 176) return none;
    int S = (int)((256 + r / 2) / r);
    if (S > 16) S = 16;
    if (S > nk / 4) S = nk / 4;
    if (S < 2) return none;
    if (r > Tl) r = Tl;
    for (int i = 0; i < p.nclasses; ++i)
        if ((long)p.B * p.cls[i].R * p.cls[i].C != Ml) return none;
    const bool xcd_map = (mtl % 8 == 0 || mtl >= 64);
    const long ids = (xcd_map ? (mtl + 7) / 8 * 8 : mtl) * (p.Np / bn);
    if (xcd_map && (mtl % 8) != 0) return none;
    return IgemmTail{(int)(ids - r), (int)r, S};
}

static size_t igemm_tail_bytes(const IgemmTail& tl, bool wide) { return (size_t)tl.n * tl.s * 128 * (wide ? 128 : 64) * sizeof(float); }

size_t cgs_igemm_slab_bytes(const IgemmParams& p_in) {
    const size_t sk = cgs_igemm_splitk_bytes(p_in);
    if (sk) return sk;
    IgemmParams p = p_in;
    p.splitk = 1; p.stat_part = nullptr; p.sign_out = nullptr;
    cgs_igemm_row_policy(p, 128);
    const IgemmTiles t = igemm_choose_tiles(p);
    const IgemmTail tl = igemm_choose_tail(p, t);
    return tl.s > 1 ? igemm_tail_bytes(tl, t.wide) : 0;
}

int cgs_igemm_signs_ok(const IgemmParams& p) {
    return (p.N % 32) == 0 && (p.epilogue == CGS_EPI_AFFINE_RELU || p.epilogue == CGS_EPI_LRELU) && choose_splitk(p) <= 1;
}

size_t cgs_igemm_splitk_bytes(const IgemmParams& p) {
    const int s = choose_splitk(p);
    if (s <= 1) return 0;
    size_t n = 0;
    for (int i = 0; i < p.nclasses; ++i) n += (size_t)s * p.B * p.cls[i].R * p.cls[i].C * p.Np;
    return n * sizeof(float);
}

template <int BM, int BN, int NW, bool VEC, int TBK, bool PAR, bool NS>
static int launch_cfg(const IgemmParams& p, hipStream_t s) {
    void (*const kern)(IgemmParams) = NS ? igemm_ns_kernel<BM, BN, NW, VEC, TBK, PAR> : igemm_kernel<BM, BN, NW, VEC, TBK, PAR>;
    constexpr int EH = (VEC && TBK == 16) ? 2 : 1;
    constexpr int WM = BM / 64;
    constexpr size_t kloop_f = (size_t)2 * BM * (TBK + 4) + 2 * TBK * BN, stage_f = (size_t)NW * (BM / WM / EH) * (BN / (NW / WM) + 4);
    constexpr size_t smem = (kloop_f > stage_f ? kloop_f : stage_f) * sizeof(float) + BM * sizeof(int);
    static bool attr_done[64] = {};
    int dev_ = 0;
    (void)hipGetDevice(&dev_);
    dev_ &= 63;
    if (!attr_done[dev_]) {
        hipError_t e = hipFuncSetAttribute((const void*)kern, hipFuncAttributeMaxDynamicSharedMemorySize, (int)smem);
        if (e != hipSuccess) return cgs_set_error(CGS_ELAUNCH, "igemm smem attr: %s", hipGetErrorString(e));
        attr_done[dev_] = true;
    }
    long maxM = 0;
    for (int i = 0; i < p.nclasses; ++i) {
        long m = (long)p.B * p.cls[i].R * p.cls[i].C;
        if (m > maxM) maxM = m;
    }
    if (maxM == 0) return CGS_OK;
    const long mtiles = (maxM + BM - 1) / BM;
    IgemmParams q = p;
    q.xcd_map = (mtiles % 8 == 0 || mtiles >= 64) ? 1 : 0;
    long gx = (q.xcd_map ? (mtiles + 7) / 8 * 8 : mtiles) * (p.Np / BN);
    if (p.tail_s > 1) {
        if ((long)p.tail_from + p.tail_n != gx) return cgs_set_error(CGS_EINVAL, "igemm: tail split planned for another grid (%d + %d != %ld)", p.tail_from, p.tail_n, gx);
        gx = (long)p.tail_from + (long)p.tail_n * p.tail_s;
    }
    unsigned gy = (unsigned)p.nclasses;
    {
        const long total = gx * (long)p.nclasses * (p.splitk > 1 ? p.splitk : 1);
        q.cls_flip = 0;
        if (igemm_round_rules_apply() && p.nclasses > 1 && !p.pix_major && total > 256 && total <= 512 && gx > 0 && (256 % gx) == 0 && p.tail_s <= 1) {
            const long per_round = 256 / gx;
            if (p.splitk > 1 && (per_round % p.nclasses) == 0) q.cls_flip = p.nclasses;
            else if (p.splitk == 1 && per_round < p.nclasses && (p.nclasses % per_round) == 0) q.cls_flip = (int)per_round;
        }
    }
    if (gx > 0x7fffffffL) return cgs_set_error(CGS_EINVAL, "igemm: grid too large");
    hipLaunchKernelGGL(kern, dim3((unsigned)gx, gy, p.splitk > 1 ? p.splitk : 1), dim3(64 * NW), smem, s, q);
    CGS_CHECK_LAUNCH("igemm");
    if (p.tail_s > 1) {
        hipLaunchKernelGGL(tail_reduce_kernel, dim3((unsigned)p.tail_n, TAIL_RSPLIT), dim3(256), 0, s, q, BM, BN);
        CGS_CHECK_LAUNCH("tail_reduce");
    }
    if (p.splitk > 1) {
        long tot = 0;
        for (int i = 0; i < p.nclasses; ++i) { long t = (long)p.B * p.cls[i].R * p.cls[i].C * (p.Np / 4); if (t > tot) tot = t; }
        unsigned rb = (unsigned)((tot + 63) / 64 > 4096 ? 4096 : (tot + 63) / 64);
        if (p.stat_part) hipLaunchKernelGGL(splitk_reduce_stats_kernel, dim3((unsigned)p.stat_cls_rows, (unsigned)((p.N + 31) / 32), p.nclasses), dim3(256), 0, s, p);
        else hipLaunchKernelGGL(splitk_reduce_kernel, dim3(rb, p.nclasses), dim3(256), 0, s, p);
        CGS_CHECK_LAUNCH("splitk_reduce");
    }
    static char name[64];
    snprintf(name, sizeof(name), "%s<%d, %d, %d, %s, %d, %s>", NS ? "igemm_ns_kernel" : "igemm_kernel", BM, BN, NW, VEC ? "true" : "false", TBK, PAR ? "true" : "false");
    cgs_note_kernel(name);
    return CGS_OK;
}

static bool igemm_pix_major(const IgemmParams& p) {
    int maxRC = 0;
    for (int i = 0; i < p.nclasses; ++i) maxRC = p.cls[i].R * p.cls[i].C > maxRC ? p.cls[i].R * p.cls[i].C : maxRC;
    const size_t in_bytes = (size_t)p.B * p.Hin * p.Win * p.Cred * 4;
    return p.vec && p.B >= 128 && maxRC <= 256 && maxRC > 1 && in_bytes <= ((size_t)384 << 20);
}

void cgs_igemm_row_policy(IgemmParams& p, int BM) {
    p.pix_major = igemm_pix_major(p);
    p.lpt = p.pix_major && (p.B % BM) == 0;
    if (p.lpt)
        for (int ci = 0; ci < p.nclasses; ++ci) {
            const IgemmClass& c = p.cls[ci];
            int cnt[256];
            for (int pix = 0; pix < c.R * c.C; ++pix) {
                const int r = pix / c.C, cc = pix - r * c.C;
                int ny = 0, nx = 0;
                for (int ta = 0; ta < c.nty; ++ta) { const int iy = r * p.S + c.dy0 + ta * p.dstep; ny += (iy >= 0 && iy < p.Hin); }
                for (int tb = 0; tb < c.ntx; ++tb) { const int ix = cc * p.S + c.dx0 + tb * p.dstep; nx += (ix >= 0 && ix < p.Win); }
                cnt[pix] = ny * nx;
                p.perm[ci][pix] = (unsigned char)pix;
            }
            for (int i = 1; i < c.R * c.C; ++i)
                for (int j = i; j > 0 && cnt[p.perm[ci][j]] > cnt[p.perm[ci][j - 1]]; --j) {
                    unsigned char t = p.perm[ci][j]; p.perm[ci][j] = p.perm[ci][j - 1]; p.perm[ci][j - 1] = t;
                }
        }
}

void cgs_igemm_count_flops(const IgemmParams& p, int BM) {
    double macs = 0.0;
    for (int ci = 0; ci < p.nclasses; ++ci) {
        const IgemmClass& c = p.cls[ci];
        const long M = (long)p.B * c.R * c.C;
        const int ntaps = c.nty * c.ntx;
        if (!(p.vec && p.pix_major)) { macs += (double)M * p.N * p.Cred * ntaps; continue; }
        for (long m0 = 0; m0 < M; m0 += BM) {
            const long ml = m0 + BM - 1 < M ? m0 + BM - 1 : M - 1;
            const int pf = (int)(m0 / p.B), pl = (int)(ml / p.B);
            int taps = ntaps;
            if (pf == pl) {
                const int r = pf / c.C, cc = pf - r * c.C;
                int ny = 0, nx = 0;
                for (int ta = 0; ta < c.nty; ++ta) { const int iy = r * p.S + c.dy0 + ta * p.dstep; ny += (iy >= 0 && iy < p.Hin); }
                for (int tb = 0; tb < c.ntx; ++tb) { const int ix = cc * p.S + c.dx0 + tb * p.dstep; nx += (ix >= 0 && ix < p.Win); }
                taps = ny * nx;
            }
            macs += (double)(ml - m0 + 1) * p.N * p.Cred * taps;
        }
    }
    cgs_add_flops(2.0 * macs);
}

int cgs_igemm_row_order(const IgemmParams& p) {
    if (!igemm_pix_major(p)) return 0;
    return (p.B % 128) == 0 ? 2 : 1;
}

int cgs_igemm_launch(const IgemmParams& p_in, void* slab, size_t slab_bytes, hipStream_t s) {
    IgemmParams p = p_in;
    p.splitk = 1; p.slab = nullptr;
    p.tail_from = p.tail_n = p.tail_s = 0;
    p.prio_t[0] = p.prio_t[1] = p.prio_t[2] = 0;
    int maxRC = 0;
    for (int i = 0; i < p.nclasses; ++i) maxRC = p.cls[i].R * p.cls[i].C > maxRC ? p.cls[i].R * p.cls[i].C : maxRC;
    cgs_igemm_row_policy(p, 128);
    if ((long)p.B * p.Hout * p.Wout * p.N * 4 > 0x7fffffffL || (long)p.B * p.Hin * p.Win * p.Cred * 4 > 0x7fffffffL)
        return cgs_set_error(CGS_EINVAL, "igemm: a tensor of one launch exceeds 2 GiB (the caller splits the batch)");
    if (p.stat_part && ((p.N & 3) || p.epilogue != CGS_EPI_NONE))
        return cgs_set_error(CGS_EINVAL, "igemm: fused statistics need N %% 4 == 0 and no epilogue");
    if (p.stat_part && p.ns_mean && (!p.ns_inv || !p.ns_gamma || !p.ns_beta || !p.ep_aux || p.ns_gimg < 0))
        return cgs_set_error(CGS_EINVAL, "igemm: norm-backward statistics need x (ep_aux), mean, invstd, gamma and beta");
    p.stat_cls_rows = 0;
    if (p.stat_part) {
        const long M0 = (long)p.B * p.cls[0].R * p.cls[0].C;
        for (int i = 1; i < p.nclasses; ++i)
            if ((long)p.B * p.cls[i].R * p.cls[i].C != M0) return cgs_set_error(CGS_EINVAL, "igemm: fused statistics need parity classes of equal size");
        p.stat_cls_rows = (int)(2 * ((M0 + 127) / 128));
    }
    if (p.sign_out && !cgs_igemm_signs_ok(p))
        return cgs_set_error(CGS_EINVAL, "igemm: a sign mask needs N %% 32 == 0, the relu / lrelu forward epilogues and a grid that is not split over K");
    {
        const size_t need = p.sign_out ? 0 : cgs_igemm_splitk_bytes(p);
        if (need && slab && slab_bytes >= need) {
            p.splitk = choose_splitk(p); p.slab = (float*)slab;
            size_t off = 0;
            for (int i = 0; i < p.nclasses; ++i) {
                p.cls[i].slab_off = (int)off;
                off += (size_t)p.splitk * p.B * p.cls[i].R * p.cls[i].C * p.Np;
            }
        }
    }
    const bool vec = p.vec != 0;
    IgemmTiles tiles = igemm_choose_tiles(p);
    IgemmTail tl = igemm_choose_tail(p, tiles);
    bool tail_fits = tl.s > 1 && slab && slab_bytes >= igemm_tail_bytes(tl, tiles.wide);
    if (tiles.wide_for_tail && !tail_fits) {
        tiles = igemm_choose_tiles(p, false);
        tl = igemm_choose_tail(p, tiles);
        tail_fits = tl.s > 1 && slab && slab_bytes >= igemm_tail_bytes(tl, tiles.wide);
    }
    bool wide = tiles.wide, deep = tiles.deep;
    const bool tall = tiles.tall;
    if (tall) cgs_igemm_row_policy(p, 256);
    cgs_igemm_count_flops(p, tall ? 256 : 128);
    if (tail_fits) {
        p.tail_from = tl.from; p.tail_n = tl.n; p.tail_s = tl.s; p.slab = (float*)slab;
        cgs_note_tail(tl.n, tl.s);
    }
    {
        const int bn_sel = wide ? 128 : 64, per_cu = vec ? igemm_blocks_per_cu(wide, deep) : 2;
        const long total_blocks = igemm_blocks(p, bn_sel);
        const bool one_round = igemm_round_rules_apply() && vec && p.splitk == 1 && !tall && total_blocks <= (long)IGEMM_CUS * per_cu && total_blocks >= IGEMM_CUS;
        if (vec && !deep && p.splitk == 1 && p.pix_major && total_blocks >= 256) { p.prio_t[0] = 85; p.prio_t[1] = 170; p.prio_t[2] = 0; }
        const int nblk_n = p.Np / bn_sel;
        if (one_round && p.lpt && p.nclasses == 1 && p.B / 128 == 8 && (32 % nblk_n) == 0) {
            const IgemmClass& c = p.cls[0];
            const int RC = c.R * c.C, nbins = 32 / nblk_n, cap = (RC + nbins - 1) / nbins;
            int cnt[256], load[32] = {}, used[32] = {};
            unsigned char bin_items[32][256];
            for (int pix = 0; pix < RC; ++pix) {
                const int r = pix / c.C, cc = pix - r * c.C;
                int ny = 0, nx = 0;
                for (int ta = 0; ta < c.nty; ++ta) { const int iy = r * p.S + c.dy0 + ta * p.dstep; ny += (iy >= 0 && iy < p.Hin); }
                for (int tb = 0; tb < c.ntx; ++tb) { const int ix = cc * p.S + c.dx0 + tb * p.dstep; nx += (ix >= 0 && ix < p.Win); }
                cnt[pix] = ny * nx;
            }
            for (int i = 0; i < RC; ++i) {
                const int pix = p.perm[0][i];
                int best = -1;
                for (int b = 0; b < nbins; ++b) {
                    const int slots = (RC - b + nbins - 1) / nbins;
                    if (used[b] < slots && used[b] < cap && (best < 0 || load[b] < load[best])) best = b;
                }
                bin_items[best][used[best]++] = (unsigned char)pix;
                load[best] += cnt[pix];
            }
            for (int b = 0; b < nbins; ++b)
                for (int k = 0; k < used[b]; ++k) p.perm[0][b + k * nbins] = bin_items[b][k];
        }
    }
    p.uni = !(p.nclasses > 1 && wide && maxRC <= 64);
    bool half = vec && wide && deep && p.splitk > 1 && !p.tap_parity && (long)p.B * maxRC <= 64;
    const bool ns = p.stat_part && p.ns_mean;
#define LC(...) (ns ? launch_cfg<__VA_ARGS__, true>(p, s) : launch_cfg<__VA_ARGS__, false>(p, s))
    if (half) return LC(64, 128, 4, true, 32, false);
    if (tall) return p.tap_parity ? LC(256, 64, 4, true, 16, true) : LC(256, 64, 4, true, 16, false);
    if (vec && !deep && !p.tap_parity) return wide ? LC(128, 128, 4, true, 16, false) : LC(128, 64, 4, true, 16, false);
    if (vec && !deep && p.tap_parity) return wide ? LC(128, 128, 4, true, 16, true) : LC(128, 64, 4, true, 16, true);
    if (vec && p.tap_parity) return wide ? LC(128, 128, 4, true, 32, true) : LC(128, 64, 4, true, 32, true);
    if (vec) return wide ? LC(128, 128, 4, true, 32, false) : LC(128, 64, 4, true, 32, false);
    return wide ? LC(128, 128, 4, false, 16, false) : LC(128, 64, 4, false, 16, false);
#undef LC
}
```

collaborative-gan-sampling_amd/csrc/igemm_epilogue.h:

```cpp
#pragma once
#include "cgs_internal.h"

typedef float f32x4 __attribute__((ext_vector_type(4)));

template <int EPI, int ROWS, int RPP, int LDE, bool SG>
__device__ __forceinline__ void epilogue_rows_signs(const IgemmParams& p, const float* E, const int* rowpix_tile, int rsub, int c4,
                                                    int n, f32x4 bias, f32x4 ea, f32x4 eb) {
    const int lane = threadIdx.x & 63;
    unsigned* plane = p.sign_out + (size_t)(n >> 5) * p.sign_plane;
#pragma unroll
    for (int it = 0; it < ROWS / RPP; ++it) {
        const int lrow = it * RPP + rsub;
        const int pix = rowpix_tile[lrow];
        const bool live = pix >= 0;
        const f32x4 v = *(const f32x4*)(E + lrow * LDE + c4);
        const size_t o = (size_t)(live ? pix : 0) * p.N + n;
        f32x4 y;
#pragma unroll
        for (int e = 0; e < 4; ++e) y[e] = epilogue_apply(v[e] + bias[e], EPI, ea[e], eb[e], 0.f);
        if (live) *(f32x4*)(p.out + o) = y;
        unsigned word = 0;
#pragma unroll
        for (int e = 0; e < 4; ++e) {
            const unsigned long long bal = __builtin_amdgcn_ballot_w64(live && y[e] > 0.f);
            word |= ((unsigned)(bal >> (lane & ~7)) & 0xffu) << (8 * e);
        }
        if (live && (lane & 7) == 0) plane[pix] = word;
    }
}

struct NsLane { f32x4 mu, inv, sc, sh; float leak; };
__device__ __forceinline__ NsLane ns_lane_params(const IgemmParams& p, int group, int n) {
    NsLane L;
    L.mu = *(const f32x4*)(p.ns_mean + (size_t)group * p.N + n);
    L.inv = *(const f32x4*)(p.ns_inv + (size_t)group * p.N + n);
    const f32x4 g = *(const f32x4*)(p.ns_gamma + n), b = *(const f32x4*)(p.ns_beta + n);
#pragma unroll
    for (int e = 0; e < 4; ++e) { L.sc[e] = g[e] * L.inv[e]; L.sh[e] = fmaf(-L.mu[e], L.sc[e], b[e]); }
    L.leak = p.ns_leak;
    return L;
}

__device__ __forceinline__ void ns_acc(const NsLane& L, float x, float dy, int e, f32x4& sa, f32x4& sb) {
    float a = sa[e], b = sb[e];
    norm_d_acc1(x, dy, L.mu[e], L.inv[e], L.sc[e], L.sh[e], L.leak, a, b);
    sa[e] = a; sb[e] = b;
}

template <int EPI, int ROWS, int RPP, int LDE, int ST = 0, int NSU = 1>
__device__ __forceinline__ void epilogue_rows(const IgemmParams& p, const float* E, const int* rowpix_tile, int rsub, int c4,
                                              int n, f32x4 bias, f32x4 ea, f32x4 eb, f32x4* sa = nullptr, f32x4* sb = nullptr,
                                              const NsLane* ns = nullptr) {
    if constexpr (ST == 2 && NSU > 1) {
        constexpr int ITERS = ROWS / RPP;
        static_assert(ITERS % NSU == 0, "row groups");
#pragma unroll
        for (int it0 = 0; it0 < ITERS; it0 += NSU) {
            f32x4 xs[NSU];
            int pixs[NSU];
#pragma unroll
            for (int u = 0; u < NSU; ++u) {
                pixs[u] = rowpix_tile[(it0 + u) * RPP + rsub];
                xs[u] = f32x4{0.f, 0.f, 0.f, 0.f};
                if (pixs[u] >= 0) xs[u] = *(const f32x4*)(p.ep_aux + (size_t)pixs[u] * p.N + n);
            }
#pragma unroll
            for (int u = 0; u < NSU; ++u) {
                if (pixs[u] < 0) continue;
                const f32x4 v = *(const f32x4*)(E + ((it0 + u) * RPP + rsub) * LDE + c4);
                f32x4 y;
#pragma unroll
                for (int e = 0; e < 4; ++e) y[e] = v[e] + bias[e];
                *(f32x4*)(p.out + (size_t)pixs[u] * p.N + n) = y;
#pragma unroll
                for (int e = 0; e < 4; ++e) ns_acc(*ns, xs[u][e], y[e], e, *sa, *sb);
            }
        }
        return;
    }
#pragma unroll
    for (int it = 0; it < ROWS / RPP; ++it) {
        const int lrow = it * RPP + rsub;
        const int pix = rowpix_tile[lrow];
        if (pix < 0) continue;
        const f32x4 v = *(const f32x4*)(E + lrow * LDE + c4);
        const size_t o = (size_t)pix * p.N + n;
        f32x4 aux = {0.f, 0.f, 0.f, 0.f};
        if (EPI >= CGS_EPI_RELU_BWD_AFFINE || ST == 2) aux = *(const f32x4*)(p.ep_aux + o);
        f32x4 y;
#pragma unroll
        for (int e = 0; e < 4; ++e) y[e] = epilogue_apply(v[e] + bias[e], EPI, ea[e], eb[e], aux[e]);
        *(f32x4*)(p.out + o) = y;
        if (ST == 1) {
#pragma unroll
            for (int e = 0; e < 4; ++e) { (*sa)[e] += y[e]; (*sb)[e] = fmaf(y[e], y[e], (*sb)[e]); }
        }
        if (ST == 2) {
#pragma unroll
            for (int e = 0; e < 4; ++e) ns_acc(*ns, aux[e], y[e], e, *sa, *sb);
        }
    }
}
```

collaborative-gan-sampling_amd/engine.py:

```python
import gc

import numpy as np
import torch

from . import kernels as K
from . import lib as L
from .nets import ARCHS, _same_out, g_input_shape, layer_ks


class _Stage:
    out = None
    bwd_epi = (L.EPI_NONE, None, None)
    pre_folded = False
    bwd_nstat = None
    bstat = None

    def fwd(self, x):
        raise NotImplementedError

    def bwd(self, dy):
        raise NotImplementedError


class _View(_Stage):
    def __init__(self, in_shape, out_shape):
        self.in_shape, self.out_shape = in_shape, out_shape

    def fwd(self, x):
        return x.view(self.out_shape)

    def bwd(self, dy):
        return dy.view(self.in_shape)


class _Conv(_Stage):

    def __init__(self, B, in_shape, w, b, stride, epi, dev):
        self.w, self.b, self.s, self.epi = w, b, stride, epi
        H, W, _ = in_shape
        self.in_hw = (H, W)
        self.out = torch.empty((B, _same_out(H, stride), _same_out(W, stride), w.shape[3]), dtype=torch.float32, device=dev)
        self.dx = torch.empty((B,) + tuple(in_shape), dtype=torch.float32, device=dev)

    part = None
    part_layout = None

    def want_stats(self, B, group_images=None):
        if self.epi != L.EPI_NONE:
            return None
        H, W, Cin = self.dx.shape[1:]
        kh, kw, _, Cout = self.w.shape
        if group_images is None:
            G = K.conv_stat_partials((B, H, W, Cin), tuple(self.w.shape), self.s, self.s)
            lay = (G, G, 1, 0) if G > 0 else None
        else:
            lay = K.conv_stat_layout(L.CONV_FWD, B, H, W, Cin, 0, 0, Cout, kh, kw, self.s, self.s, group_images)
        if lay is not None:
            self.part = torch.empty((lay[0], 2, Cout), dtype=torch.float32, device=self.out.device)
            self.part_layout = lay
        return self.part

    def fwd(self, x):
        self.x_in = x
        if self.part is not None:
            return K.conv2d_fwd_stats(x, self.w, self.b, self.part, self.s, self.s, out=self.out)
        return K.conv2d_fwd(x, self.w, self.b, self.s, self.s, self.epi, out=self.out)

    def bwd(self, dy):
        if not self.pre_folded:
            if self.epi == L.EPI_LRELU:
                dy = K.lrelu_bwd(dy, self.out, out=dy)
            elif self.epi == L.EPI_TANH:
                dy = K.tanh_bwd(dy, self.out, out=dy)
        e, a, aux = self.bwd_epi
        return K.conv2d_bwd_data(dy, self.w, self.in_hw, self.s, self.s, out=self.dx, epilogue=e, ep_a=a, ep_aux=aux, nstat=self.bwd_nstat)


class _Deconv(_Stage):

    def __init__(self, B, in_shape, out_shape, w, b, stride, epi, a, c, dev):
        self.w, self.b, self.s, self.epi, self.a, self.c = w, b, stride, epi, a, c
        self.in_hw, self.out_hw = (in_shape[0], in_shape[1]), (out_shape[0], out_shape[1])
        self.out = torch.empty((B,) + tuple(out_shape), dtype=torch.float32, device=dev)
        self.dx = torch.empty((B,) + tuple(in_shape), dtype=torch.float32, device=dev)

    signs = None
    bwd_signs = None
    part = None
    part_layout = None

    def want_stats(self, B, group_images=None):
        if self.epi != L.EPI_NONE:
            return None
        lay = K.conv_stat_layout(L.DECONV_FWD, *self.call_dims(), self.s, self.s, group_images or B)
        if lay is not None:
            self.part = torch.empty((lay[0], 2, self.w.shape[2]), dtype=torch.float32, device=self.out.device)
            self.part_layout = lay
        return self.part

    def fwd(self, x):
        return K.deconv2d_fwd(x, self.w, self.b, self.out_hw, self.s, self.s, self.epi, self.a, self.c, out=self.out, signs=self.signs,
                              part=self.part)

    def bwd(self, dy):
        if not self.pre_folded:
            if self.epi == L.EPI_AFFINE_RELU:
                dy = K.affine_relu_bwd(dy, self.out, self.a, out=dy)
            elif self.epi == L.EPI_TANH:
                dy = K.tanh_bwd(dy, self.out, out=dy)
        e, a, aux = self.bwd_epi
        return K.deconv2d_bwd_data(dy, self.w, self.in_hw, self.s, self.s, out=self.dx, epilogue=e, ep_a=a, ep_aux=aux,
                                   ep_signs=self.bwd_signs, nstat=self.bwd_nstat)

    def call_dims(self):
        kh, kw, Cout, Cin = self.w.shape
        return (self.out.shape[0], self.in_hw[0], self.in_hw[1], Cin, self.out_hw[0], self.out_hw[1], Cout, kh, kw)


class _Linear(_Stage):
    def __init__(self, B, w, b, epi, dev):
        self.w, self.b, self.epi = w, b, epi
        self.out = torch.empty((B, w.shape[1]), dtype=torch.float32, device=dev)
        self.dx = torch.empty((B, w.shape[0]), dtype=torch.float32, device=dev)

    def fwd(self, x):
        self.x_in = x
        return K.linear_fwd(x, self.w, self.b, self.epi, out=self.out)

    def bwd(self, dy):
        if self.epi == L.EPI_LRELU:
            dy = K.lrelu_bwd(dy, self.out, out=dy)
        return K.linear_bwd_data(dy, self.w, out=self.dx)


class _BnTrainLrelu(_Stage):

    def __init__(self, B, shape, gamma, beta, leak, dev):
        self.gamma, self.beta, self.leak = gamma, beta, leak
        self.out = torch.empty((B,) + tuple(shape), dtype=torch.float32, device=dev)
        self.mean = torch.empty(shape[-1], dtype=torch.float32, device=dev)
        self.invstd = torch.empty(shape[-1], dtype=torch.float32, device=dev)
        self.x = None

    sync = None
    groups = 1
    part = None

    part_layout = None

    def set_groups(self, groups, producer=None):
        self.groups = int(groups)
        self.part = self.part_layout = None
        if producer is not None:
            producer.part = producer.part_layout = None
            B = self.out.shape[0]
            self.part = producer.want_stats(B, B // self.groups)
            self.part_layout = producer.part_layout
        C = self.out.shape[-1]
        self.mean = torch.empty((self.groups, C), dtype=torch.float32, device=self.out.device)
        self.invstd = torch.empty((self.groups, C), dtype=torch.float32, device=self.out.device)

    def _g(self, t):
        return t.view(self.groups, -1, t.shape[-1])

    def fwd(self, x):
        self.x = x
        if self.bstat is not None:
            self.bstat.x = x
        if self.groups > 1:
            if self.part is not None:
                K.groupnorm_lrelu_fwd_from_partials(x, self.part, self.part_layout, self.groups, self.gamma, self.beta, self.leak,
                                                    out=self.out, stats=(self.mean, self.invstd))
            else:
                K.instnorm_lrelu_fwd(self._g(x), self.gamma, self.beta, self.leak, out=self._g(self.out), stats=(self.mean, self.invstd))
            return self.out
        if self.sync is None:
            if self.part is not None:
                K.bn_train_lrelu_fwd_from_partials(x, self.part, self.gamma, self.beta, self.leak, out=self.out, stats=(self.mean, self.invstd))
            else:
                K.bn_train_lrelu_fwd(x, self.gamma, self.beta, self.leak, out=self.out, stats=(self.mean, self.invstd))
            return self.out
        M = x.numel() // x.shape[-1]
        sums = self.sync.sums(x.shape[-1], x.device)
        K.bn_sync_fwd_sums(x, sums)
        self.sync.all_reduce(sums)
        K.bn_sync_fwd_apply(x, self.gamma, self.beta, sums, self.sync.world * M, self.leak, out=self.out,
                            stats=(self.mean, self.invstd))
        return self.out

    def bwd(self, dy):
        if self.bstat is not None:
            return K.norm_lrelu_bwd_from_partials(dy, self.x, self.bstat, self.groups, out=dy)
        if self.groups > 1:
# ... 143 lines not shown
            w, b = P[f"{scope}/{Lr[1]}/w"], P[f"{scope}/{Lr[1]}/biases"]
            _, stride_l = layer_ks(Lr, k, stride)
            epi, a, c, used = L.EPI_NONE, None, None, 1
            if kind(i + 1) == "bn" and kind(i + 2) == "relu" and not bn_training:
                a, c = fold(layers[i + 1][1]); epi, used = L.EPI_AFFINE_RELU, 3
            elif kind(i + 1) == "tanh":
                epi, used = L.EPI_TANH, 2
            stages.append(_Deconv(B, shape, Lr[2], w, b, stride_l, epi, a, c, dev))
            shape = tuple(Lr[2]); i += used
        elif t == "conv":
            w, b = P[f"{scope}/{Lr[1]}/w"], P[f"{scope}/{Lr[1]}/biases"]
            _, stride_l = layer_ks(Lr, k, stride)
            epi, used = (L.EPI_LRELU, 2) if kind(i + 1) == "lrelu" else (L.EPI_TANH, 2) if kind(i + 1) == "tanh" else (L.EPI_NONE, 1)
            st = _Conv(B, shape, w, b, stride_l, epi, dev)
            stages.append(st)
            shape = tuple(st.out.shape[1:]); i += used
        elif t == "linear":
            w, b = P[f"{scope}/{Lr[1]}/Matrix"], P[f"{scope}/{Lr[1]}/bias"]
            epi, used = (L.EPI_LRELU, 2) if kind(i + 1) == "lrelu" else (L.EPI_NONE, 1)
            stages.append(_Linear(B, w, b, epi, dev))
            shape = (Lr[2],); i += used
        elif t == "bn":
            s = f"{scope}/{Lr[1]}"
            if bn_training:
                leak, used = (K.LEAK, 2) if kind(i + 1) == "lrelu" else (0.0, 2) if kind(i + 1) == "relu" else (1.0, 1)
                bn_stage = _BnTrainLrelu(B, shape, P[s + "/gamma"], P[s + "/beta"], leak, dev)
                if stages and isinstance(stages[-1], _Conv):
                    bn_stage.part = stages[-1].want_stats(B)
                stages.append(bn_stage)
                i += used
            else:
                if kind(i + 1) != "relu":
                    raise NotImplementedError("inference-mode bn is only supported when followed by relu")
                a, c = fold(Lr[1])
                stages.append(_AffineRelu(B, shape, a, c, dev)); i += 2
        elif t == "instnorm":
            sc = f"{scope}/{Lr[1]}"
            leak, used = (K.LEAK, 2) if kind(i + 1) == "lrelu" else (0.0, 2) if kind(i + 1) == "relu" else (1.0, 1)
            in_stage = _InstNormAct(B, shape, P[sc + "/scale"], P[sc + "/offset"], leak, dev)
            if stages and isinstance(stages[-1], (_Conv, _Deconv)):
                in_stage.part = stages[-1].want_stats(B, 1)
                in_stage.part_layout = stages[-1].part_layout
            stages.append(in_stage); i += used
        elif t == "res":
            inner, ishape = compile_layers(Lr[1], shape, P, scope, B, k, stride, bn_training, dev, folds)
            assert tuple(ishape) == tuple(shape)
            stages.append(_Residual(B, shape, inner, dev)); i += 1
        elif t in ("relu", "lrelu", "tanh"):
            stages.append(_Unary(B, shape, t, dev)); i += 1
        elif t == "reshape":
            stages.append(_View((B,) + shape, (B,) + tuple(Lr[1]))); shape = tuple(Lr[1]); i += 1
        elif t == "flatten":
            flat = (int(np.prod(shape)),)
            stages.append(_View((B,) + shape, (B,) + flat)); shape = flat; i += 1
        else:
            raise KeyError(t)
    return stages, shape


def link_backward_fusion(stages):
    for below, above in zip(stages[:-1], stages[1:]):
        if not isinstance(above, (_Conv, _Deconv)) or below.pre_folded:
            continue
        if isinstance(below, _Deconv) and below.epi == L.EPI_AFFINE_RELU:
            above.bwd_epi = (L.EPI_RELU_BWD_AFFINE, below.a, below.out)
            import os
            if isinstance(above, _Deconv) and not os.environ.get("CGS_NO_SIGN_MASKS"):
                s_ = (below.s, below.s)
                if (K.conv_signs_ok(L.DECONV_FWD, *below.call_dims(), *s_, L.EPI_AFFINE_RELU)
                        and K.conv_signs_ok(L.DECONV_BWD_DATA, *above.call_dims(), above.s, above.s, L.EPI_RELU_BWD_AFFINE)):
                    below.signs = torch.empty(below.out.numel() // 32, dtype=torch.int32, device=below.out.device)
                    above.bwd_signs = below.signs
        elif isinstance(below, _Deconv) and below.epi == L.EPI_TANH:
            above.bwd_epi = (L.EPI_TANH_BWD, None, below.out)
        elif isinstance(below, _Conv) and below.epi == L.EPI_LRELU:
            above.bwd_epi = (L.EPI_LRELU_BWD, None, below.out)
        elif isinstance(below, _Conv) and below.epi == L.EPI_TANH:
            above.bwd_epi = (L.EPI_TANH_BWD, None, below.out)
        else:
            continue
        below.pre_folded = True


NSTAT_MAX_BYTES = 48 * 2 ** 20


def link_norm_backward_stats(stages, B):
    for below, above in zip(stages[:-1], stages[1:]):
        if isinstance(below, _Residual):
            link_norm_backward_stats(below.inner, B)
        if not isinstance(above, (_Conv, _Deconv)) or above.bwd_epi[0] != L.EPI_NONE or above.bwd_nstat is not None:
            continue
        if isinstance(below, _BnTrainLrelu) and below.sync is None:
            gamma, beta, gimg = below.gamma, below.beta, B // below.groups
        elif isinstance(below, _InstNormAct):
            gamma, beta, gimg = below.scale, below.offset, 1
        else:
            continue
        C = below.out.shape[-1]
        if below.out.numel() * 4 > NSTAT_MAX_BYTES:
            continue
        if isinstance(above, _Conv):
            H, W, Cin = above.dx.shape[1:]
            kh, kw, _, Cout = above.w.shape
            lay = K.conv_stat_layout(L.CONV_BWD_DATA, B, H, W, Cin, 0, 0, Cout, kh, kw, above.s, above.s, gimg)
        else:
            lay = K.conv_stat_layout(L.DECONV_BWD_DATA, *above.call_dims(), above.s, above.s, gimg)
        if lay is None:
            continue
        part = torch.empty((lay[0], 2, C), dtype=torch.float32, device=below.out.device)
        below.bstat = above.bwd_nstat = K.NormBwdStats(None, below.mean, below.invstd, gamma, beta, below.leak, gimg, part, lay)
    if stages and isinstance(stages[-1], _Residual):
        link_norm_backward_stats(stages[-1].inner, B)


class Tape:

    def __init__(self, layers, in_shape, P, scope, B, k, stride, bn_training, dev):
        self.folds = []
        self.stages, self.out_shape = compile_layers(layers, in_shape, P, scope, B, k, stride, bn_training, dev, self.folds)

    def forward(self, x):
        for st in self.stages:
            x = st.fwd(x)
        return x

    def backward(self, dy):
        for st in reversed(self.stages):
            dy = st.bwd(dy)
        return dy


def _entry(fn):
    import functools

    @functools.wraps(fn)
    def wrapped(self, *a, **kw):
        prev = K.set_contraction(self.contraction)
        try:
            return fn(self, *a, **kw)
        finally:
            if prev != self.contraction:
                K.set_contraction(prev)
    return wrapped


class RefineEngine:

    def __init__(self, arch, params, batch_size, device=None, use_graph=False, sync_bn=None, bn_groups=1, contraction="f32"):
        self.A = ARCHS[arch] if isinstance(arch, str) else arch
        if contraction not in L.CONTRACTIONS:
            raise L.CgsError(f"contraction {contraction!r}: expected one of {sorted(L.CONTRACTIONS)}")
        self.contraction = contraction
        self.dev = torch.device(device if device is not None else "cuda:0")
        if self.dev.type != "cuda":
            raise L.CgsError("RefineEngine needs a GPU device (there is no CPU path)")
        L.load()
        prev_mode = K.set_contraction(self.contraction)
        try:
            self._build(params, batch_size, use_graph, sync_bn, bn_groups)
        finally:
            if prev_mode != self.contraction:
                K.set_contraction(prev_mode)

    def _build(self, params, batch_size, use_graph, sync_bn, bn_groups):
        A, B = self.A, int(batch_size)
        self.B, self.P = B, params
        with torch.cuda.device(self.dev):
            self.g_head = Tape(A["g_head"], g_input_shape(A), params, "generator", B, A["k"], A["stride"], False, self.dev)
            self.g_tail = Tape(A["g_tail"], A["feature"], params, "generator", B, A["k"], A["stride"], False, self.dev)
            self.d = Tape(A["d"], A["img"], params, "discriminator", B, A["k"], A["stride"], True, self.dev)
            link_backward_fusion(self.g_tail.stages + self.d.stages)
            fs = (B,) + tuple(A["feature"])
            f32 = dict(dtype=torch.float32, device=self.dev)
            self.theta, self.mom, self.best_theta = torch.empty(fs, **f32), torch.empty(fs, **f32), torch.empty(fs, **f32)
            self.logit, self.best_logit = torch.empty(B, **f32), torch.empty(B, **f32)
            self.default_logit, self.best_step = torch.empty(B, **f32), torch.empty(B, **f32)
            self.tickets = torch.zeros(B, dtype=torch.int32, device=self.dev)
            self.dlogits = torch.empty((B,) + tuple(self.d.out_shape), **f32)
            self.forced = torch.zeros(B, dtype=torch.int32, device=self.dev)
            self.images = torch.empty((B,) + tuple(A["img"]), **f32)
        self.use_graph = use_graph
        self._graphs = {}
        self._ladam, self.mean_square = None, None
        self._gstream = None
        self._ws_epoch = K.WS.epoch
        self.bn_groups = int(bn_groups)
        if self.bn_groups > 1:
            if B % self.bn_groups:
                raise L.CgsError(f"bn_groups={bn_groups} does not divide the engine batch {B}")
            if sync_bn:
                raise L.CgsError("bn_groups and sync_bn are mutually exclusive")

            def walk_g(stages):
                for below, st in zip([None] + stages[:-1], stages):
                    if isinstance(st, _BnTrainLrelu):
                        st.set_groups(self.bn_groups, below if isinstance(below, _Conv) else None)
                    if isinstance(st, _Residual):
                        walk_g(st.inner)
            walk_g(self.d.stages); walk_g(self.g_tail.stages)
        self.sync_bn = None
        if sync_bn is not None and sync_bn is not False:
            if use_graph:
                raise L.CgsError("sync_bn runs eagerly: the all-reduce between the two halves of a bn pass is not captured")
            self.sync_bn = BnSync(None if sync_bn is True else sync_bn)

            def walk(stages):
                for st in stages:
                    if isinstance(st, _BnTrainLrelu):
                        st.sync = self.sync_bn
                    if isinstance(st, _Residual):
                        walk(st.inner)
            walk(self.d.stages); walk(self.g_tail.stages)

        def drop_partials(stages):
            for below, st in zip([None] + stages[:-1], stages):
                if isinstance(st, _BnTrainLrelu) and st.sync is not None:
                    st.part = None
                    if isinstance(below, _Conv):
                        below.part = None
                if isinstance(st, _Residual):
                    drop_partials(st.inner)
        drop_partials(self.d.stages); drop_partials(self.g_tail.stages)
        link_norm_backward_stats(self.g_tail.stages + self.d.stages, B)

    def _sync_weights(self):
        if self._ws_epoch != K.WS.epoch:
            self._resync()

    def _resync(self):
        K.set_contraction(self.contraction)
        epoch = K.WS.epoch
        with torch.cuda.device(self.dev):
            for tape in (self.g_head, self.g_tail, self.d):
                for a, c, gamma, beta, mm, mv in tape.folds:
                    K.bn_fold(gamma, beta, mm, mv, out=(a, c))
            if self._gstream is not None and self._graphs:
                cur = torch.cuda.current_stream(self.dev)
                self._gstream.wait_stream(cur)
                with torch.cuda.stream(self._gstream):
                    self.forward_logits(self.theta, self.logit)
                    self.backward_to_feature()
                cur.wait_stream(self._gstream)
        self._ws_epoch = epoch

    @_entry
    def input_to_feature(self, z):
        self._sync_weights()
        return self.g_head.forward(z)

    @_entry
    def feature_to_data(self, feat):
        self._sync_weights()
        return self.g_tail.forward(feat)

    @_entry
    def discriminator(self, x):
        self._sync_weights()
        return self.d.forward(x)

    @_entry
    def generate(self, z):
        self._sync_weights()
        return self.g_tail.forward(self.g_head.forward(z))

    @_entry
    def score(self, images, out=None):
        self._sync_weights()
        return K.sigmoid_rowmean(self.d.forward(images), out=out)

    def _feature_stage(self):
        stages = self.d.stages
        head = max(i for i, st in enumerate(stages) if isinstance(st, (_Linear, _Conv)))
        i = head - 1
        while i >= 0 and isinstance(stages[i], _View):
            i -= 1
        st = stages[i] if i >= 0 else None
        active = (isinstance(st, (_Conv, _Linear)) and st.epi != L.EPI_NONE) or (isinstance(st, (_BnTrainLrelu, _InstNormAct)) and st.leak != 1.0) \
            or isinstance(st, _Unary)
        if not active:
            raise L.CgsError("score_with_features: no nonlinearity in front of the discriminator's logit layer")
        return st

    def feature_width(self):
        return int(self._feature_stage().out.shape[-1])

    @_entry
    def score_with_features(self, images, out=None, feat_out=None):
        self._sync_weights()
        st = self._feature_stage()
        sig = K.sigmoid_rowmean(self.d.forward(images), out=out)
        act = st.out
        if act.dim() == 2:
            if feat_out is None:
                return sig, act
            feat_out.copy_(act)
            return sig, feat_out
        if feat_out is None:
            if getattr(self, "_feat", None) is None:
                self._feat = torch.empty((act.shape[0], act.shape[-1]), dtype=torch.float32, device=self.dev)
            feat_out = self._feat
        return sig, K.spatial_mean(act, out=feat_out)

    def forward_logits(self, theta, logit_out, loss="bce", ladam=None, first=False):
        x = self.g_tail.forward(theta)
        head = self.d.stages[-1]
        plain = loss == "bce" and ladam is None
        if isinstance(head, _Linear) and head.w.shape[1] == 1 and head.epi == L.EPI_NONE:
            for st in self.d.stages[:-1]:
                x = st.fwd(x)
            head.x_in = x
            if plain:
                return K.linear_out1_bce(x, head.w, head.b, head.out, self.dlogits, logit_out)
            return K.linear_out1_seed(x, head.w, head.b, head.out, self.dlogits, logit_out, loss, ladam, first)
        logits = self.d.forward(x)
        if plain:
            K.bce_ones_grad_rowmean(logits, self.dlogits, logit_out)
        else:
            K.refine_loss_seed(logits, loss, self.dlogits, logit_out, ladam, first)
        return logits

    def backward_to_feature(self):
        return self.g_tail.backward(self.d.backward(self.dlogits))

    @_entry
    def compute_forward_logits_and_grad(self, feature, loss="bce"):
        if loss not in ("bce", "lsq", "linear"):
            raise L.CgsError(f"loss {loss!r}: the engine differentiates 'bce', 'lsq' and 'linear'")
        self._sync_weights()
        self.forward_logits(feature, self.logit, loss)
        return self.logit, self.backward_to_feature()

    def _program(self, steps, rate, alpha, probabilistic, vmin, vmax, loss="bce", ladam=None):
        th = self.theta
        render = self.g_tail.stages[-1].out
        self.forward_logits(th, self.logit, loss, ladam, True)
        self.default_logit.copy_(self.logit)
        self.best_logit.copy_(self.logit)
        self.best_theta.copy_(th)
        self.images.copy_(render)
        self.best_step.fill_(1.0)
        self.tickets.zero_()
        forced = self.forced if probabilistic else None
        for i in range(steps):
            g = self.backward_to_feature()
            if ladam is None:
                K.refine_update(th, self.mom, g, rate, alpha, first=(i == 0), vmin=vmin, vmax=vmax)
            else:
                K.refine_update_ladam(th, self.mom, self.mean_square, g, ladam.gain, rate, first=(i == 0), vmin=vmin, vmax=vmax)
            self.forward_logits(th, self.logit, loss, ladam, False)
            K.refine_select2(render, self.images, th, self.best_theta, self.logit, forced, i, self.best_logit, self.best_step, self.tickets)

    @_entry
    def refine(self, feature0, steps, rate, method="momentum", mode="deterministic", indices=None,
               vmin=None, vmax=None, loss="bce", real_sigmoid_mean=None):
        ladam = None
        if method == "momentum":
            alpha = 0.9
        elif method == "sgd":
            alpha = 0.0
        elif method == "ladam":
            if real_sigmoid_mean is None:
                raise L.CgsError("ladam needs a loss argument the map-space refiner never passes "
                                 "(sampling/collaborator.py:66 vs policy.py:48-51); use momentum or sgd, or pass real_sigmoid_mean")
            alpha = None
        else:
            raise NotImplementedError(method)
        if loss not in ("bce", "lsq", "linear"):
            raise L.CgsError(f"loss {loss!r}: the engine differentiates 'bce', 'lsq' and 'linear'")
        if mode not in ("deterministic", "probabilistic"):
            raise NotImplementedError(mode)
        prob = mode == "probabilistic"
        if prob:
            if indices is None:
                raise L.CgsError("probabilistic mode needs the step indices (np.random.randint(K+1, size=B))")
            self.forced.copy_(torch.as_tensor(np.asarray(indices), dtype=torch.int32))
        if tuple(feature0.shape) != tuple(self.theta.shape):
            raise L.CgsError(f"feature batch {tuple(feature0.shape)} != engine shape {tuple(self.theta.shape)}")
        self._sync_weights()
        with torch.cuda.device(self.dev):
            self.theta.copy_(feature0)
            if method == "ladam":
                if self._ladam is None:
                    self._ladam = K.LadamState(self.B, self.dev)
                    self.mean_square = torch.empty_like(self.mom)
                ladam = self._ladam
                ladam.set_real(real_sigmoid_mean)
            key = (steps, float(rate), alpha, prob, vmin, vmax, loss, method)
            if not self.use_graph:
                self._program(steps, rate, alpha, prob, vmin, vmax, loss, ladam)
            else:
                g = self._graphs.get(key)
                if g is None:
                    if self._gstream is None:
                        self._gstream = torch.cuda.Stream(self.dev)
                    cur = torch.cuda.current_stream(self.dev)
                    self._gstream.wait_stream(cur)
                    with torch.cuda.stream(self._gstream):
                        self._program(steps, rate, alpha, prob, vmin, vmax, loss, ladam)
                        self.theta.copy_(feature0)
                    torch.cuda.synchronize(self.dev)
                    gc_was_on = gc.isenabled()
                    gc.disable()
                    try:
                        g = torch.cuda.CUDAGraph()
                        with torch.cuda.graph(g, stream=self._gstream, capture_error_mode="thread_local"):
                            self._program(steps, rate, alpha, prob, vmin, vmax, loss, ladam)
                    except L.CgsError:
                        raise
                    except Exception as ex:
                        raise L.GraphCaptureError(f"{type(ex).__name__}: {str(ex)[:300]}") from ex
                    finally:
                        if gc_was_on:
                            gc.enable()
                    cur.wait_stream(self._gstream)
                    self._graphs[key] = g
                g.replay()
        return self.images, self.default_logit, self.best_logit, self.best_step, self.best_theta

    @_entry
    def refresh_weights(self):
        K.WS.invalidate()
        self._resync()

    @_entry
    def refine_from_z(self, z, steps, rate, **kw):
        return self.refine(self.input_to_feature(z), steps, rate, **kw)
```

collaborative-gan-sampling_amd/kernels.py:

```python
import math
import operator
import weakref

import torch

from . import lib as L

LEAK = 0.2
BN_EPS = 1e-5


def _chk(t, name):
    if not (isinstance(t, torch.Tensor) and t.is_cuda and t.dtype == torch.float32 and t.is_contiguous()):
        raise L.CgsError(f"{name}: expected a contiguous fp32 tensor on the GPU, got "
                         f"{type(t).__name__} {getattr(t, 'dtype', None)} {getattr(t, 'device', None)}")
    return t


def _ptr(t):
    return None if t is None else t.data_ptr()


def _stream():
    return torch.cuda.current_stream().cuda_stream
# ... 143 lines not shown
    L.call("cgs_conv2d_nhwc_fwd", _ptr(x), _ptr(w), _ptr(bias), _ptr(y), B, H, W, Cin, Cout, kh, kw, sh, sw,
           epilogue, _ptr(ep_a), _ptr(ep_b), _ptr(ws), ws.numel() * 4, pre, _stream())
    if pr is not None:
        pr.done()
    return y


def conv_stat_partials(x_shape, w_shape, sh=2, sw=2):
    B, H, W, Cin = x_shape
    kh, kw, _, Cout = w_shape
    _, nbytes = WS.plan(L.CONV_FWD, B, H, W, Cin, 0, 0, Cout, kh, kw, sh, sw, L.EPI_NONE)
    return int(L.load().cgs_conv_stat_partials(B, H, W, Cin, Cout, kh, kw, sh, sw, nbytes))


def conv_stat_layout(op, B, H, W, Cin, Ho, Wo, Cout, kh, kw, sh, sw, group_images):
    import ctypes as C
    _, nbytes = WS.plan(op, B, H, W, Cin, Ho, Wo, Cout, kh, kw, sh, sw, L.EPI_NONE)
    a, b, c = C.c_int(0), C.c_int(0), C.c_int(0)
    rows = int(L.load().cgs_conv_stat_layout(op, B, H, W, Cin, Ho, Wo, Cout, kh, kw, sh, sw, int(group_images), nbytes,
                                             C.addressof(a), C.addressof(b), C.addressof(c)))
    return (rows, a.value, b.value, c.value) if rows > 0 else None


def groupnorm_lrelu_fwd_from_partials(x, part, layout, groups, scale, offset, leak=1.0, eps=BN_EPS, out=None, stats=None):
    _chk(x, "x"); _chk(part, "part")
    C_ = x.shape[-1]
    Mg = x.numel() // (groups * C_)
    y = out if out is not None else torch.empty_like(x)
    mean, invstd = stats if stats is not None else (torch.empty((groups, C_), dtype=torch.float32, device=x.device),
                                                     torch.empty((groups, C_), dtype=torch.float32, device=x.device))
    ws = _in_workspace(groups, Mg, C_, x.device)
    pr = _Prof(0.0, "", _nb(x, y), op="groupnorm_lrelu_fwd_from_partials") if PROFILE is not None else None
    L.call("cgs_groupnorm_lrelu_fwd_from_partials", _ptr(x), _ptr(part), groups, layout[1], layout[2], layout[3], _ptr(scale), _ptr(offset),
           eps, leak, _ptr(y), _ptr(mean), _ptr(invstd), Mg, C_, _ptr(ws), ws.numel() * 4, _stream())
    if pr is not None:
        pr.done()
    return y, mean, invstd


def conv2d_fwd_stats(x, w, bias, part, sh=2, sw=2, out=None):
    _chk(x, "x"); _chk(w, "w"); _chk(part, "part")
    B, H, W, Cin = x.shape
    kh, kw, Cin2, Cout = w.shape
    if Cin2 != Cin:
        raise L.CgsError(f"conv2d: weight Cin {Cin2} != input channels {Cin}")
    y = out if out is not None else torch.empty((B, same_out(H, sh), same_out(W, sw), Cout), dtype=torch.float32, device=x.device)
    ws, pre = WS.get(w, L.CONV_FWD, kh, kw, sh, sw, Cin, Cout, (B, H, W), L.EPI_NONE, ptrs=(_ptr(x), _ptr(bias), _ptr(y), _ptr(part)))
    Ho, Wo = y.shape[1], y.shape[2]
    pr = _Prof(2.0 * B * Ho * Wo * Cout * kh * kw * Cin, f"conv_fwd {H}x{W} {Cin}->{Cout}", _nb(x, w, y)) if PROFILE is not None else None
    L.call("cgs_conv2d_nhwc_fwd_stats", _ptr(x), _ptr(w), _ptr(bias), _ptr(y), B, H, W, Cin, Cout, kh, kw, sh, sw,
           _ptr(ws), ws.numel() * 4, pre, _ptr(part), part.numel() * 4, _stream())
    if pr is not None:
        pr.done()
    return y


def bn_train_lrelu_fwd_from_partials(x, part, gamma, beta, leak=LEAK, eps=BN_EPS, out=None, stats=None):
    _chk(x, "x")
    C = x.shape[-1]
    M = x.numel() // C
    y = out if out is not None else torch.empty_like(x)
    mean, invstd = stats if stats is not None else (torch.empty(C, dtype=torch.float32, device=x.device),
                                                    torch.empty(C, dtype=torch.float32, device=x.device))
    ws = _bn_workspace(M, C, x.device)
    pr = _Prof(0.0, "", _nb(x, y), op="bn_train_lrelu_fwd_from_partials") if PROFILE is not None else None
    L.call("cgs_bn_train_lrelu_fwd_from_partials", _ptr(x), _ptr(part), part.shape[0], _ptr(gamma), _ptr(beta), eps, leak, _ptr(y),
           _ptr(mean), _ptr(invstd), M, C, _ptr(ws), ws.numel() * 4, _stream())
    if pr is not None:
        pr.done()
    return y, mean, invstd


class NormBwdStats:
    __slots__ = ("x", "mean", "invstd", "gamma", "beta", "leak", "group_images", "part", "layout")

    def __init__(self, x, mean, invstd, gamma, beta, leak, group_images, part, layout):
        self.x, self.mean, self.invstd, self.gamma, self.beta = x, mean, invstd, gamma, beta
        self.leak, self.group_images, self.part, self.layout = float(leak), int(group_images), part, layout

    def args(self):
        return (_ptr(self.x), _ptr(self.mean), _ptr(self.invstd), _ptr(self.gamma), _ptr(self.beta), self.leak, self.group_images)


def conv2d_bwd_data(dy, w, in_hw, sh=2, sw=2, out=None, epilogue=L.EPI_NONE, ep_a=None, ep_aux=None, nstat=None):
    _chk(dy, "dy"); _chk(w, "w")
    kh, kw, Cin, Cout = w.shape
    B = dy.shape[0]
    H, W = in_hw
    dx = out if out is not None else torch.empty((B, H, W, Cin), dtype=torch.float32, device=dy.device)
    ws, pre = WS.get(w, L.CONV_BWD_DATA, kh, kw, sh, sw, Cin, Cout, (B, H, W), epilogue,
                     ptrs=(_ptr(dy), _ptr(dx), _ptr(ep_a), _ptr(ep_aux)))
    Ho, Wo = dy.shape[1], dy.shape[2]
    pr = _Prof(2.0 * B * Ho * Wo * Cout * kh * kw * Cin, f"conv_bwd {H}x{W} {Cin}<-{Cout}",
               _nb(dy, w, dx, ep_aux, nstat.x if nstat is not None else None)) if PROFILE is not None else None
    if nstat is not None:
        if epilogue != L.EPI_NONE:
            raise L.CgsError("conv2d_bwd_data: norm-backward statistics come with no epilogue")
        L.call("cgs_conv2d_nhwc_bwd_data_nstats", _ptr(dy), _ptr(w), _ptr(dx), B, H, W, Cin, Cout, kh, kw, sh, sw, *nstat.args(),
               _ptr(ws), ws.numel() * 4, pre, _ptr(nstat.part), nstat.part.numel() * 4, _stream())
    else:
        L.call("cgs_conv2d_nhwc_bwd_data", _ptr(dy), _ptr(w), _ptr(dx), B, H, W, Cin, Cout, kh, kw, sh, sw,
               epilogue, _ptr(ep_a), _ptr(ep_aux), _ptr(ws), ws.numel() * 4, pre, _stream())
    if pr is not None:
        pr.done()
    return dx


def conv_signs_ok(op, B, H, W, Cin, Ho, Wo, Cout, kh, kw, sh, sw, epilogue):
    _, nbytes = WS.plan(op, B, H, W, Cin, Ho, Wo, Cout, kh, kw, sh, sw, epilogue)
    return bool(L.load().cgs_conv_signs_ok(op, B, H, W, Cin, Ho, Wo, Cout, kh, kw, sh, sw, epilogue, nbytes))


def deconv2d_fwd(x, w, bias, out_hw, sh=2, sw=2, epilogue=L.EPI_NONE, ep_a=None, ep_b=None, out=None, signs=None, part=None):
    _chk(x, "x"); _chk(w, "w")
    B, H, W, Cin = x.shape
    kh, kw, Cout, Cin2 = w.shape
    if Cin2 != Cin:
        raise L.CgsError(f"deconv2d: weight Cin {Cin2} != input channels {Cin}")
    Ho, Wo = out_hw
    y = out if out is not None else torch.empty((B, Ho, Wo, Cout), dtype=torch.float32, device=x.device)
    ws, pre = WS.get(w, L.DECONV_FWD, kh, kw, sh, sw, Cin, Cout, (B, H, W), epilogue, (Ho, Wo),
                     ptrs=(_ptr(x), _ptr(bias), _ptr(y), _ptr(ep_a), _ptr(ep_b)))
    pr = _Prof(2.0 * B * H * W * Cin * kh * kw * Cout, f"deconv_fwd {H}x{W} {Cin}->{Cout}", _nb(x, w, y)) if PROFILE is not None else None
    if part is not None:
        if epilogue != L.EPI_NONE or signs is not None:
            raise L.CgsError("deconv2d_fwd: the statistics partials are those of the plain output (no epilogue, no sign mask)")
        L.call("cgs_deconv2d_nhwc_fwd_stats", _ptr(x), _ptr(w), _ptr(bias), _ptr(y), B, H, W, Cin, Ho, Wo, Cout, kh, kw, sh, sw,
               _ptr(ws), ws.numel() * 4, pre, _ptr(part), part.numel() * 4, _stream())
    elif signs is not None:
        L.call("cgs_deconv2d_nhwc_fwd_signs", _ptr(x), _ptr(w), _ptr(bias), _ptr(y), B, H, W, Cin, Ho, Wo, Cout, kh, kw, sh, sw,
               epilogue, _ptr(ep_a), _ptr(ep_b), signs.data_ptr(), _ptr(ws), ws.numel() * 4, pre, _stream())
    else:
        L.call("cgs_deconv2d_nhwc_fwd", _ptr(x), _ptr(w), _ptr(bias), _ptr(y), B, H, W, Cin, Ho, Wo, Cout, kh, kw, sh, sw,
               epilogue, _ptr(ep_a), _ptr(ep_b), _ptr(ws), ws.numel() * 4, pre, _stream())
    if pr is not None:
        pr.done()
    return y


def deconv2d_bwd_data(dy, w, in_hw, sh=2, sw=2, out=None, epilogue=L.EPI_NONE, ep_a=None, ep_aux=None, ep_signs=None, nstat=None):
    _chk(dy, "dy"); _chk(w, "w")
    kh, kw, Cout, Cin = w.shape
    B, Ho, Wo, _ = dy.shape
    H, W = in_hw
    dx = out if out is not None else torch.empty((B, H, W, Cin), dtype=torch.float32, device=dy.device)
    ws, pre = WS.get(w, L.DECONV_BWD_DATA, kh, kw, sh, sw, Cin, Cout, (B, H, W), epilogue, (Ho, Wo),
                     ptrs=(_ptr(dy), _ptr(dx), _ptr(ep_a), _ptr(ep_aux)))
    pr = _Prof(2.0 * B * H * W * Cin * kh * kw * Cout, f"deconv_bwd {H}x{W} {Cin}<-{Cout}",
               _nb(dy, w, dx, ep_aux if ep_signs is None else ep_signs, nstat.x if nstat is not None else None)) if PROFILE is not None else None
    if nstat is not None:
        if epilogue != L.EPI_NONE or ep_signs is not None:
            raise L.CgsError("deconv2d_bwd_data: norm-backward statistics come with no epilogue")
        L.call("cgs_deconv2d_nhwc_bwd_data_nstats", _ptr(dy), _ptr(w), _ptr(dx), B, H, W, Cin, Ho, Wo, Cout, kh, kw, sh, sw, *nstat.args(),
               _ptr(ws), ws.numel() * 4, pre, _ptr(nstat.part), nstat.part.numel() * 4, _stream())
    elif ep_signs is not None:
        L.call("cgs_deconv2d_nhwc_bwd_data_signs", _ptr(dy), _ptr(w), _ptr(dx), B, H, W, Cin, Ho, Wo, Cout, kh, kw, sh, sw,
               epilogue, _ptr(ep_a), ep_signs.data_ptr(), _ptr(ws), ws.numel() * 4, pre, _stream())
    else:
        L.call("cgs_deconv2d_nhwc_bwd_data", _ptr(dy), _ptr(w), _ptr(dx), B, H, W, Cin, Ho, Wo, Cout, kh, kw, sh, sw,
               epilogue, _ptr(ep_a), _ptr(ep_aux), _ptr(ws), ws.numel() * 4, pre, _stream())
    if pr is not None:
        pr.done()
    return dx


def linear_fwd(x, w, bias, epilogue=L.EPI_NONE, out=None):
    _chk(x, "x"); _chk(w, "w")
    B, K = x.shape
    K2, N = w.shape
    if K2 != K:
        raise L.CgsError(f"linear: Matrix rows {K2} != input features {K}")
    y = out if out is not None else torch.empty((B, N), dtype=torch.float32, device=x.device)
    if N == 1:
        pr = _Prof(2.0 * B * K, "", _nb(x, w, y), op="linear_out1_fwd") if PROFILE is not None else None
        L.call("cgs_linear_fwd", _ptr(x), _ptr(w), _ptr(bias), _ptr(y), B, K, N, epilogue, None, 0, 0, _stream())
        if pr is not None:
            pr.done()
        return y
    ws, pre = WS.get(w, L.CONV_FWD, 1, 1, 1, 1, K, N, (B, 1, 1), epilogue, ptrs=(_ptr(x), _ptr(bias), _ptr(y)))
    pr = _Prof(2.0 * B * K * N, f"linear_fwd {K}->{N}", _nb(x, w, y)) if PROFILE is not None else None
    L.call("cgs_linear_fwd", _ptr(x), _ptr(w), _ptr(bias), _ptr(y), B, K, N, epilogue, _ptr(ws), ws.numel() * 4, pre, _stream())
    if pr is not None:
        pr.done()
    return y


def linear_bwd_data(dy, w, out=None):
    _chk(dy, "dy"); _chk(w, "w")
    B, N = dy.shape
    K = w.shape[0]
    dx = out if out is not None else torch.empty((B, K), dtype=torch.float32, device=dy.device)
    if N == 1:
        pr = _Prof(2.0 * B * K, "", _nb(dy, w, dx), op="linear_out1_bwd") if PROFILE is not None else None
        L.call("cgs_linear_bwd_data", _ptr(dy), _ptr(w), _ptr(dx), B, K, N, None, 0, 0, _stream())
        if pr is not None:
            pr.done()
        return dx
    ws, pre = WS.get(w, L.CONV_BWD_DATA, 1, 1, 1, 1, K, N, (B, 1, 1), ptrs=(_ptr(dy), _ptr(dx)))
    pr = _Prof(2.0 * B * K * N, f"linear_bwd {K}<-{N}", _nb(dy, w, dx)) if PROFILE is not None else None
    L.call("cgs_linear_bwd_data", _ptr(dy), _ptr(w), _ptr(dx), B, K, N, _ptr(ws), ws.numel() * 4, pre, _stream())
    if pr is not None:
        pr.done()
    return dx


def bn_train_lrelu_fwd(x, gamma, beta, leak=LEAK, eps=BN_EPS, out=None, stats=None):
    _chk(x, "x")
    C = x.shape[-1]
    M = x.numel() // C
    y = out if out is not None else torch.empty_like(x)
    if stats is not None:
        mean, invstd = stats
    else:
        mean = torch.empty(C, dtype=torch.float32, device=x.device)
        invstd = torch.empty(C, dtype=torch.float32, device=x.device)
    ws = _bn_workspace(M, C, x.device)
    pr = _Prof(0.0, "", _nb(x, x, y), op="bn_train_lrelu_fwd") if PROFILE is not None else None
    L.call("cgs_bn_train_lrelu_fwd", _ptr(x), _ptr(gamma), _ptr(beta), eps, leak, _ptr(y), _ptr(mean), _ptr(invstd),
           M, C, _ptr(ws), ws.numel() * 4, _stream())
    if pr is not None:
        pr.done()
    return y, mean, invstd


def bn_train_lrelu_bwd_data(dy, x, gamma, beta, mean, invstd, leak=LEAK, out=None):
    _chk(dy, "dy"); _chk(x, "x")
    C = x.shape[-1]
# ... 848 lines not shown
```

collaborative-gan-sampling_amd/lib.py:

```python
import ctypes as C
import os

_HERE = os.path.dirname(os.path.abspath(__file__))
LIB_PATH = os.environ.get("CGS_LIB") or os.path.join(_HERE, "libcgs_hip.so")

OK, EINVAL, EWORKSPACE, ELAUNCH = 0, -1, -2, -3
EPI_NONE, EPI_LRELU, EPI_AFFINE_RELU, EPI_TANH = 0, 1, 2, 3
EPI_RELU_BWD_AFFINE, EPI_LRELU_BWD, EPI_TANH_BWD = 4, 5, 6
CONV_FWD, CONV_BWD_DATA, DECONV_FWD, DECONV_BWD_DATA = 0, 1, 2, 3
FAMILY_IGEMM, FAMILY_QUAD, FAMILY_SMALLN_T, FAMILY_SMALLN_F, FAMILY_PATCH, FAMILY_TAPS, FAMILY_DOT, FAMILY_IGEMM_BX6 = 0, 1, 2, 3, 4, 5, 6, 7
CONTRACTION_F32, CONTRACTION_BX6, CONTRACTION_BX6_ALL = 0, 1, 2
CONTRACTIONS = {"f32": CONTRACTION_F32, "bx6": CONTRACTION_BX6, "bx6_all": CONTRACTION_BX6_ALL}
LOSS_BCE, LOSS_LSQ, LOSS_LINEAR, LOSS_HINGE = 0, 1, 2, 3
LOSSES = {"bce": LOSS_BCE, "lsq": LOSS_LSQ, "linear": LOSS_LINEAR, "hinge": LOSS_HINGE}


class LadamSeed(C.Structure):
    _fields_ = [("s_real", C.c_void_p), ("loss_avg", C.c_void_p), ("gain", C.c_void_p), ("first", C.c_int)]


_p, _i, _f, _z = C.c_void_p, C.c_int, C.c_float, C.c_size_t
_ll = C.c_longlong

SIGNATURES = {
    "cgs_version": (_i, []),
    "cgs_source_sha": (C.c_char_p, []),
    "cgs_last_error": (C.c_char_p, []),
    "cgs_last_kernel": (C.c_char_p, []),
    "cgs_last_executed_flops": (C.c_double, []),
    "cgs_last_tail_tiles": (_i, []),
    "cgs_last_tail_split": (_i, []),
    "cgs_set_contraction": (_i, [_i]),
    "cgs_get_contraction": (_i, []),
    "cgs_conv_ws_bytes": (_z, [_i] * 7),
    "cgs_conv_ws_bytes_for": (_z, [_i] * 10),
    "cgs_conv_family": (_i, [_i] * 13 + [_z]),
    "cgs_conv2d_nhwc_fwd": (_i, [_p] * 4 + [_i] * 9 + [_i, _p, _p, _p, _z, _i, _p]),
    "cgs_conv_stat_partials": (_i, [_i] * 9 + [_z]),
    "cgs_conv2d_nhwc_fwd_stats": (_i, [_p] * 4 + [_i] * 9 + [_p, _z, _i, _p, _z, _p]),
    "cgs_conv_stat_layout": (_i, [_i] * 13 + [_z, _p, _p, _p]),
    "cgs_deconv2d_nhwc_fwd_stats": (_i, [_p] * 4 + [_i] * 11 + [_p, _z, _i, _p, _z, _p]),
    "cgs_conv2d_nhwc_bwd_data_nstats": (_i, [_p] * 3 + [_i] * 9 + [_p] * 5 + [_f, _i, _p, _z, _i, _p, _z, _p]),
    "cgs_deconv2d_nhwc_bwd_data_nstats": (_i, [_p] * 3 + [_i] * 11 + [_p] * 5 + [_f, _i, _p, _z, _i, _p, _z, _p]),
    "cgs_norm_lrelu_bwd_from_partials": (_i, [_p] * 3 + [_i] * 4 + [_p] * 4 + [_f, _p, _i, _i, _p, _z, _p]),
    "cgs_groupnorm_lrelu_fwd_from_partials": (_i, [_p, _p, _i, _i, _i, _i, _p, _p, _f, _f, _p, _p, _p, _i, _i, _p, _z, _p]),
    "cgs_bn_train_lrelu_fwd_from_partials": (_i, [_p, _p, _i, _p, _p, _f, _f, _p, _p, _p, _i, _i, _p, _z, _p]),
    "cgs_conv2d_nhwc_bwd_data": (_i, [_p] * 3 + [_i] * 9 + [_i, _p, _p, _p, _z, _i, _p]),
    "cgs_deconv2d_nhwc_fwd": (_i, [_p] * 4 + [_i] * 11 + [_i, _p, _p, _p, _z, _i, _p]),
    "cgs_deconv2d_nhwc_bwd_data": (_i, [_p] * 3 + [_i] * 11 + [_i, _p, _p, _p, _z, _i, _p]),
    "cgs_conv_signs_ok": (_i, [_i] * 13 + [_z]),
    "cgs_deconv2d_nhwc_fwd_signs": (_i, [_p] * 4 + [_i] * 11 + [_i, _p, _p, _p, _p, _z, _i, _p]),
    "cgs_deconv2d_nhwc_bwd_data_signs": (_i, [_p] * 3 + [_i] * 11 + [_i, _p, _p, _p, _z, _i, _p]),
    "cgs_linear_fwd": (_i, [_p] * 4 + [_i] * 4 + [_p, _z, _i, _p]),
    "cgs_linear_bwd_data": (_i, [_p] * 3 + [_i] * 3 + [_p, _z, _i, _p]),
    "cgs_bn_ws_bytes": (_z, [_i, _i]),
    "cgs_bn_train_lrelu_fwd": (_i, [_p, _p, _p, _f, _f, _p, _p, _p, _i, _i, _p, _z, _p]),
    "cgs_bn_train_lrelu_bwd_data": (_i, [_p] * 6 + [_f, _p, _i, _i, _p, _z, _p]),
    "cgs_bn_sync_fwd_sums": (_i, [_p, _p, _i, _i, _p, _z, _p]),
    "cgs_bn_sync_fwd_apply": (_i, [_p, _p, _p, _f, _f, _p, _ll, _p, _p, _p, _i, _i, _p, _z, _p]),
    "cgs_bn_sync_bwd_sums": (_i, [_p] * 6 + [_f, _p, _i, _i, _p, _z, _p]),
    "cgs_bn_sync_bwd_apply": (_i, [_p] * 6 + [_f, _p, _ll, _p, _i, _i, _p, _z, _p]),
    "cgs_instnorm_ws_bytes": (_z, [_i, _i, _i]),
    "cgs_instnorm_lrelu_fwd": (_i, [_p, _p, _p, _f, _f, _p, _p, _p, _i, _i, _i, _p, _z, _p]),
    "cgs_instnorm_lrelu_bwd_data": (_i, [_p] * 6 + [_f, _p, _i, _i, _i, _p, _z, _p]),
    "cgs_add": (_i, [_p, _p, _p, _z, _p]),
    "cgs_bn_fold": (_i, [_p] * 4 + [_f, _p, _p, _i, _p]),
    "cgs_affine_relu_fwd": (_i, [_p] * 4 + [_i, _i, _p]),
    "cgs_affine_relu_bwd": (_i, [_p] * 4 + [_i, _i, _p]),
    "cgs_affine_fwd": (_i, [_p] * 4 + [_i, _i, _p]),
    "cgs_affine_bwd": (_i, [_p] * 3 + [_i, _i, _p]),
    "cgs_lrelu_fwd": (_i, [_p, _f, _p, _z, _p]),
    "cgs_lrelu_bwd": (_i, [_p, _p, _f, _p, _z, _p]),
    "cgs_tanh_fwd": (_i, [_p, _p, _z, _p]),
    "cgs_tanh_bwd": (_i, [_p, _p, _p, _z, _p]),
    "cgs_bce_ones_grad_rowmean": (_i, [_p, _p, _p, _i, _i, _p]),
    "cgs_bce_ones_fwd": (_i, [_p, _p, _z, _p]),
    "cgs_bce_ones_bwd": (_i, [_p, _p, _p, _z, _p]),
    "cgs_sigmoid_rowmean": (_i, [_p, _p, _i, _i, _p]),
    "cgs_clip": (_i, [_p, _f, _f, _p, _z, _p]),
    "cgs_refine_update": (_i, [_p, _p, _p, _f, _f, _i, _i, _f, _f, _z, _p]),
    "cgs_refine_select": (_i, [_p, _p, _p, _i, _p, _p, _p, _i, _i, _p]),
    "cgs_refine_select_rows": (_i, [_p, _p, _p, _i, _p, _p, _i, _i, _p]),
    "cgs_refine_select2": (_i, [_p, _p, _i, _p, _p, _i, _p, _p, _i, _p, _p, _p, _i, _p]),
    "cgs_linear_out1_bce": (_i, [_p, _p, _p, _p, _p, _p, _i, _i, _p]),
    "cgs_linear_out1_seed": (_i, [_p, _p, _p, _p, _p, _p, _i, _i, _i, _p, _p]),
    "cgs_refine_loss_seed": (_i, [_p, _i, _p, _p, _i, _i, _p, _p]),
    "cgs_refine_update_ladam": (_i, [_p, _p, _p, _p, _p, _f, _i, _i, _f, _f, _i, _i, _p]),
    "cgs_ladam_gain": (_i, [_p, _p, _p, _i, _i, _p]),
    "cgs_gan_logits_grad": (_i, [_p, _i, _f, _f, _p, _p, _i, _p]),
    "cgs_gan_loss": (_i, [_p, _i, _f, _p, _p, _z, _p]),
    "cgs_mlp2d_sigmoid_saliency": (_i, [_p, _p, _i, _i, _p, _p, _p, _i, _f, _p]),
    "cgs_refine2d": (_i, [_p, _p, _i, _i, _p, _f, _f, _i, _f, _i, _p, _p, _p, _i, _p]),
    "cgs_refine2d_devbase": (_i, [_p, _p, _i, _i, _p, _p, _f, _i, _f, _i, _p, _p, _p, _i, _p]),
    "cgs_mlp2d_train_ws_bytes": (_z, [_i, _i]),
    "cgs_mlp2d_d_step": (_i, [_p, _p, _i, _i, _p, _i, _p, _i, _f, _p, _p, _p, _p, _z, _p]),
    "cgs_mlp2d_wide_train_ws_bytes": (_z, [_i, _i, _i]),
    "cgs_mlp2d_wide_d_step": (_i, [_p, _p, _i, _i, _p, _i, _p, _i, _f, _p, _p, _p, _p, _z, _p]),
    "cgs_mlp2d_gen_ws_bytes": (_z, [_i, _i, _i]),
    "cgs_mlp2d_gen_fwd": (_i, [_p] * 6 + [_i, _i, _p, _p, _i, _i, _f, _p, _p, _z, _p]),
    "cgs_mlp2d_wide_gen_ws_bytes": (_z, [_i, _i, _i]),
    "cgs_mlp2d_wide_gen_fwd": (_i, [_p] * 6 + [_i, _i, _p, _p, _i, _i, _f, _p, _p, _z, _p]),
    "cgs_mlp2d_g_step": (_i, [_p] * 6 + [_i, _i, _p, _p, _i, _f, _f, _p, _p, _p, _p, _z, _p]),
    "cgs_mlp2d_wide_g_step_ws_bytes": (_z, [_i, _i, _i]),
    "cgs_mlp2d_wide_g_step": (_i, [_p] * 6 + [_i, _i, _p, _p, _i, _f, _f, _p, _p, _p, _p, _z, _p]),
    "cgs_conv_wgrad_ws_bytes": (_z, [_i] * 9),
    "cgs_conv2d_nhwc_bwd_weight": (_i, [_p] * 3 + [_i] * 9 + [_i, _p, _z, _p]),
    "cgs_deconv_wgrad_ws_bytes": (_z, [_i] * 11),
    "cgs_deconv2d_nhwc_bwd_weight": (_i, [_p] * 3 + [_i] * 11 + [_i, _p, _z, _p]),
    "cgs_linear_bwd_weight": (_i, [_p] * 3 + [_i] * 3 + [_i, _p, _z, _p]),
    "cgs_bias_grad": (_i, [_p, _p, _i, _i, _i, _p, _z, _p]),
    "cgs_bn_train_param_grads": (_i, [_p, _i, _i, _p, _p, _i, _p]),
    "cgs_instnorm_param_grads": (_i, [_p, _i, _i, _i, _p, _p, _i, _p]),
    "cgs_conv_wgrad_cout1_ws_bytes": (_z, [_i] * 8),
    "cgs_conv2d_nhwc_bwd_weight_cout1": (_i, [_p] * 3 + [_i] * 8 + [_i, _p, _z, _p]),
    "cgs_bce_logits_grad": (_i, [_p, _f, _f, _p, _p, _i, _p]),
    "cgs_adam_step": (_i, [_p, _p, _p, _p, _f, _f, _f, _f, _z, _p]),
    "cgs_adam_multi": (_i, [_p, _i, _p, _i, _p, _f, _f, _f, _p]),
    "cgs_bn_moving_update": (_i, [_p, _p, _p, _p, _i, C.c_double, _f, _p]),
    "cgs_pool_moments_ws_bytes": (_z, [_i, _i]),
    "cgs_pool_moments_accumulate": (_i, [_p, _i, _i, _p, _i, _p, _p, _p, _p, _z, _p]),
    "cgs_spatial_mean": (_i, [_p, _p, _i, _i, _i, _p]),
    "cgs_f64_matmul": (_i, [_p, _p, _p, _i, C.c_double, C.c_double, _p]),
    "cgs_frechet_ws_bytes": (_z, [_i]),
    "cgs_frechet_from_moments": (_i, [_p, _p, _p, _ll, _p, _p, _p, _ll, _i, _i, _i, _p, _p, _z, _p]),
    "cgs_calibration_ws_bytes": (_z, [_i, _i]),
    "cgs_calibration_accumulate": (_i, [_p, _i, _i, _p, _i, _p, _p, _z, _p]),
    "cgs_mode_stats_ws_bytes": (_z, [_i, _i]),
    "cgs_mode_stats_accumulate": (_i, [_p, _i, _p, _i, C.c_double, _p, _p, _z, _p]),
    "cgs_kde2d_ws_bytes": (_z, [_i, _i, _i]),
    "cgs_kde2d_accumulate": (_i, [_p, _i, _p, _i, _p, _i, _p, _p, _p, _z, _p]),
    "cgs_drs_ws_bytes": (_z, [_i, _i]),
    "cgs_drs_decide": (_i, [_p, _i, _i, _p, C.c_double, C.c_double, _p, _p, _p, _p, _p, _p, _z, _p]),
# ... 110 lines not shown
```

include/cgs_hip.h:

```cpp
#ifndef CGS_HIP_H
#define CGS_HIP_H

#include <stddef.h>
#include <stdint.h>

#ifdef __cplusplus
extern "C" {
#endif

#define CGS_OK 0
#define CGS_EINVAL (-1)
#define CGS_EWORKSPACE (-2)
#define CGS_ELAUNCH (-3)

#define CGS_EPI_NONE 0
#define CGS_EPI_LRELU 1
#define CGS_EPI_AFFINE_RELU 2
#define CGS_EPI_TANH 3
#define CGS_EPI_RELU_BWD_AFFINE 4
#define CGS_EPI_LRELU_BWD 5
#define CGS_EPI_TANH_BWD 6

#define CGS_CONV_FWD 0
#define CGS_CONV_BWD_DATA 1
// ... 6 lines not shown
#define CGS_LOSS_HINGE 3

typedef struct cgs_ladam_seed {
    const float* s_real;
    float* loss_avg;
    float* gain;
    int first;
} cgs_ladam_seed;

int cgs_version(void);
const char* cgs_source_sha(void);
const char* cgs_last_error(void);
const char* cgs_last_kernel(void);
double cgs_last_executed_flops(void);
int cgs_last_tail_tiles(void);
int cgs_last_tail_split(void);

#define CGS_CONTRACTION_F32 0
#define CGS_CONTRACTION_BX6 1
#define CGS_CONTRACTION_BX6_ALL 2
int cgs_set_contraction(int mode);
int cgs_get_contraction(void);

size_t cgs_conv_ws_bytes(int op, int kh, int kw, int sh, int sw, int Cin, int Cout);
size_t cgs_conv_ws_bytes_for(int op, int B, int H, int W, int Cin, int Cout, int kh, int kw, int sh, int sw);

#define CGS_FAMILY_IGEMM 0
#define CGS_FAMILY_QUAD 1
#define CGS_FAMILY_SMALLN_T 2
#define CGS_FAMILY_SMALLN_F 3
#define CGS_FAMILY_PATCH 4
#define CGS_FAMILY_TAPS 5
#define CGS_FAMILY_DOT 6
#define CGS_FAMILY_IGEMM_BX6 7
int cgs_conv_family(int op, int B, int H, int W, int Cin, int Ho, int Wo, int Cout, int kh, int kw, int sh, int sw,
                    int epilogue, size_t ws_bytes);

int cgs_conv2d_nhwc_fwd(const float* x, const float* w, const float* bias, float* y,
                        int B, int H, int W, int Cin, int Cout, int kh, int kw, int sh, int sw,
                        int epilogue, const float* ep_a, const float* ep_b,
                        void* ws, size_t ws_bytes, int ws_prepacked, void* stream);

int cgs_conv_stat_partials(int B, int H, int W, int Cin, int Cout, int kh, int kw, int sh, int sw, size_t ws_bytes);
int cgs_conv2d_nhwc_fwd_stats(const float* x, const float* w, const float* bias, float* y,
                              int B, int H, int W, int Cin, int Cout, int kh, int kw, int sh, int sw,
                              void* ws, size_t ws_bytes, int ws_prepacked,
                              float* stat_part, size_t stat_part_bytes, void* stream);

int cgs_conv_stat_layout(int op, int B, int H, int W, int Cin, int Ho, int Wo, int Cout, int kh, int kw, int sh, int sw,
                         int group_images, size_t ws_bytes, int* rows_per_seg, int* nseg, int* seg_stride);
int cgs_deconv2d_nhwc_fwd_stats(const float* x, const float* w, const float* bias, float* y,
                                int B, int H, int W, int Cin, int Ho, int Wo, int Cout, int kh, int kw, int sh, int sw,
                                void* ws, size_t ws_bytes, int ws_prepacked,
                                float* stat_part, size_t stat_part_bytes, void* stream);

int cgs_conv2d_nhwc_bwd_data_nstats(const float* dy, const float* w, float* dx,
                                    int B, int H, int W, int Cin, int Cout, int kh, int kw, int sh, int sw,
                                    const float* x_norm, const float* mean, const float* invstd, const float* gamma, const float* beta,
                                    float leak, int group_images, void* ws, size_t ws_bytes, int ws_prepacked,
                                    float* stat_part, size_t stat_part_bytes, void* stream);
int cgs_deconv2d_nhwc_bwd_data_nstats(const float* dy, const float* w, float* dx,
                                      int B, int H, int W, int Cin, int Ho, int Wo, int Cout, int kh, int kw, int sh, int sw,
                                      const float* x_norm, const float* mean, const float* invstd, const float* gamma, const float* beta,
                                      float leak, int group_images, void* ws, size_t ws_bytes, int ws_prepacked,
                                      float* stat_part, size_t stat_part_bytes, void* stream);
int cgs_norm_lrelu_bwd_from_partials(const float* dy, const float* x, const float* part, int groups, int rows_per_seg, int nseg,
                                     int seg_stride, const float* gamma, const float* beta, const float* mean, const float* invstd,
                                     float leak, float* dx, int M_group, int C, void* ws, size_t ws_bytes, void* stream);

int cgs_conv2d_nhwc_bwd_data(const float* dy, const float* w, float* dx,
                             int B, int H, int W, int Cin, int Cout, int kh, int kw, int sh, int sw,
                             int epilogue, const float* ep_a, const float* ep_aux,
                             void* ws, size_t ws_bytes, int ws_prepacked, void* stream);

int cgs_deconv2d_nhwc_fwd(const float* x, const float* w, const float* bias, float* y,
                          int B, int H, int W, int Cin, int Ho, int Wo, int Cout, int kh, int kw, int sh, int sw,
                          int epilogue, const float* ep_a, const float* ep_b,
                          void* ws, size_t ws_bytes, int ws_prepacked, void* stream);

int cgs_deconv2d_nhwc_bwd_data(const float* dy, const float* w, float* dx,
                               int B, int H, int W, int Cin, int Ho, int Wo, int Cout, int kh, int kw, int sh, int sw,
                               int epilogue, const float* ep_a, const float* ep_aux,
                               void* ws, size_t ws_bytes, int ws_prepacked, void* stream);

int cgs_conv_signs_ok(int op, int B, int H, int W, int Cin, int Ho, int Wo, int Cout, int kh, int kw, int sh, int sw,
                      int epilogue, size_t ws_bytes);
int cgs_deconv2d_nhwc_fwd_signs(const float* x, const float* w, const float* bias, float* y,
                                int B, int H, int W, int Cin, int Ho, int Wo, int Cout, int kh, int kw, int sh, int sw,
                                int epilogue, const float* ep_a, const float* ep_b, unsigned* signs,
                                void* ws, size_t ws_bytes, int ws_prepacked, void* stream);
int cgs_deconv2d_nhwc_bwd_data_signs(const float* dy, const float* w, float* dx,
                                     int B, int H, int W, int Cin, int Ho, int Wo, int Cout, int kh, int kw, int sh, int sw,
                                     int epilogue, const float* ep_a, const unsigned* aux_signs,
                                     void* ws, size_t ws_bytes, int ws_prepacked, void* stream);

int cgs_linear_fwd(const float* x, const float* w, const float* bias, float* y, int B, int in, int out,
                   int epilogue, void* ws, size_t ws_bytes, int ws_prepacked, void* stream);
int cgs_linear_out1_bce(const float* x, const float* w, const float* bias, float* logits, float* dlogits, float* logit_mean, int B, int in,
                        void* stream);
int cgs_linear_out1_seed(const float* x, const float* w, const float* bias, float* logits, float* dlogits, float* logit_mean, int B, int in,
                         int kind, const cgs_ladam_seed* ladam, void* stream);
int cgs_linear_bwd_data(const float* dy, const float* w, float* dx, int B, int in, int out,
                        void* ws, size_t ws_bytes, int ws_prepacked, void* stream);

size_t cgs_bn_ws_bytes(int M, int C);
int cgs_bn_train_lrelu_fwd(const float* x, const float* gamma, const float* beta, float eps, float leak,
                           float* y, float* mean, float* invstd, int M, int C,
                           void* ws, size_t ws_bytes, void* stream);
int cgs_bn_train_lrelu_fwd_from_partials(const float* x, const float* part, int G, const float* gamma, const float* beta,
                                         float eps, float leak, float* y, float* mean, float* invstd, int M, int C,
                                         void* ws, size_t ws_bytes, void* stream);
int cgs_bn_train_lrelu_bwd_data(const float* dy, const float* x, const float* gamma, const float* beta,
                                const float* mean, const float* invstd, float leak, float* dx, int M, int C,
                                void* ws, size_t ws_bytes, void* stream);

int cgs_bn_sync_fwd_sums(const float* x, double* sums, int M, int C, void* ws, size_t ws_bytes, void* stream);
int cgs_bn_sync_fwd_apply(const float* x, const float* gamma, const float* beta, float eps, float leak, const double* sums,
                          long long M_total, float* y, float* mean, float* invstd, int M, int C,
                          void* ws, size_t ws_bytes, void* stream);
int cgs_bn_sync_bwd_sums(const float* dy, const float* x, const float* gamma, const float* beta, const float* mean,
                         const float* invstd, float leak, double* sums, int M, int C, void* ws, size_t ws_bytes, void* stream);
int cgs_bn_sync_bwd_apply(const float* dy, const float* x, const float* gamma, const float* beta, const float* mean,
                          const float* invstd, float leak, const double* sums, long long M_total, float* dx, int M, int C,
                          void* ws, size_t ws_bytes, void* stream);

size_t cgs_instnorm_ws_bytes(int B, int HW, int C);
int cgs_instnorm_lrelu_fwd(const float* x, const float* scale, const float* offset, float eps, float leak, float* y,
                           float* mean, float* invstd, int B, int HW, int C, void* ws, size_t ws_bytes, void* stream);
int cgs_instnorm_lrelu_bwd_data(const float* dy, const float* x, const float* scale, const float* offset,
                                const float* mean, const float* invstd, float leak, float* dx, int B, int HW, int C,
                                void* ws, size_t ws_bytes, void* stream);
int cgs_groupnorm_lrelu_fwd_from_partials(const float* x, const float* part, int groups, int rows_per_seg, int nseg, int seg_stride,
                                          const float* gamma, const float* beta, float eps, float leak, float* y, float* mean,
                                          float* invstd, int M_group, int C, void* ws, size_t ws_bytes, void* stream);
int cgs_add(const float* a, const float* b, float* out, size_t n, void* stream);

int cgs_bn_fold(const float* gamma, const float* beta, const float* moving_mean, const float* moving_var,
                float eps, float* a, float* b, int C, void* stream);
int cgs_affine_relu_fwd(const float* x, const float* a, const float* b, float* y, int M, int C, void* stream);
int cgs_affine_relu_bwd(const float* dy, const float* y, const float* a, float* dx, int M, int C, void* stream);
int cgs_affine_fwd(const float* x, const float* a, const float* b, float* y, int M, int C, void* stream);
int cgs_affine_bwd(const float* dy, const float* a, float* dx, int M, int C, void* stream);
int cgs_lrelu_fwd(const float* x, float leak, float* y, size_t n, void* stream);
int cgs_lrelu_bwd(const float* dy, const float* y, float leak, float* dx, size_t n, void* stream);
int cgs_tanh_fwd(const float* x, float* y, size_t n, void* stream);
int cgs_tanh_bwd(const float* dy, const float* y, float* dx, size_t n, void* stream);

int cgs_bce_ones_grad_rowmean(const float* logits, float* dlogits, float* logit_mean, int B, int P, void* stream);
int cgs_refine_loss_seed(const float* logits, int kind, float* dlogits, float* logit_mean, int B, int P, const cgs_ladam_seed* ladam,
                         void* stream);

int cgs_bce_ones_fwd(const float* logits, float* loss, size_t n, void* stream);
int cgs_bce_ones_bwd(const float* dloss, const float* logits, float* dlogits, size_t n, void* stream);
int cgs_sigmoid_rowmean(const float* logits, float* sigmoids, int B, int P, void* stream);
int cgs_gan_loss(const float* logits, int kind, float target, const float* dloss, float* out, size_t n, void* stream);
int cgs_clip(const float* x, float vmin, float vmax, float* y, size_t n, void* stream);

int cgs_refine_update(float* theta, float* m, const float* g, float rate, float alpha, int first,
                      int use_clip, float vmin, float vmax, size_t n, void* stream);
int cgs_ladam_gain(const float* loss, float* loss_avg, float* gain, int first, int B, void* stream);
int cgs_refine_update_ladam(float* theta, float* m, float* v, const float* g, const float* gain, float rate, int first, int use_clip,
                            float vmin, float vmax, int B, int F, void* stream);
int cgs_refine_select(const float* theta, const float* logit, const int32_t* forced, int step_index,
                      float* best_theta, float* best_logit, float* best_step, int B, int F, void* stream);
int cgs_refine_select2(const float* rows, float* best_rows, int Frows, const float* theta, float* best_theta, int F, const float* logit,
                       const int32_t* forced, int step_index, float* best_logit, float* best_step, int* tickets, int B, void* stream);
// ... 115 lines not shown
```

Measured before the change: 6639 samples/s.

## Fuse momentum refine update into the final backward-data implicit GEMM epilogue

Adds an update variant of the implicit-GEMM backward-data kernel, plus its split-K and tail reducers, that applies the momentum step to theta and m directly instead of writing the feature gradient. The refine loop uses it when available, which removes the separate elementwise refine_update kernel and the gradient write and re-read each step. This adds kernel template instantiations, restrictions (no clip, no LAdam, whole batch in one launch) and a new graph key.

```diff
diff --git a/collaborative-gan-sampling_amd/csrc/api.hip b/collaborative-gan-sampling_amd/csrc/api.hip
--- a/collaborative-gan-sampling_amd/csrc/api.hip
+++ b/collaborative-gan-sampling_amd/csrc/api.hip
@@ -26,7 +26,7 @@
 
 extern "C" {
 
-int cgs_version(void) { return 116; }
+int cgs_version(void) { return 117; }
 const char* cgs_last_error(void) { return g_err; }
 const char* cgs_last_kernel(void) { return g_last_kernel; }
 double cgs_last_executed_flops(void) { return g_last_flops; }
@@ -110,12 +110,13 @@
 
 struct NsArgs { const float *mean, *invstd, *gamma, *beta; float leak; int group_images; };
 
-enum ConvForm { FORM_PLAIN, FORM_STATS, FORM_NSTATS, FORM_SIGNS };
+enum ConvForm { FORM_PLAIN, FORM_STATS, FORM_NSTATS, FORM_SIGNS, FORM_UPDATE };
 struct ConvExtras {
     ConvForm form = FORM_PLAIN;
     float* stat_part = nullptr; size_t stat_part_bytes = 0;
     NsArgs ns = {};
     unsigned* sign_out = nullptr; const unsigned* aux_signs = nullptr;
+    float* up_mom = nullptr; float up_rate = 0.f, up_alpha = 0.f; int up_first = 0;
 };
 
 static int run_dir(const ConvCall& c, int B, const float* in, const float* w, const float* bias, float* out, int epilogue,
@@ -138,6 +139,7 @@
     const int fam = choose_family(L, dirT, p, ws != nullptr, ws_bytes, !((uintptr_t)in & 15), !((uintptr_t)ws & 15), rest_al);
     if (x.stat_part && fam != CGS_FAMILY_IGEMM && fam != CGS_FAMILY_IGEMM_BX6) return cgs_set_error(CGS_EINVAL, "%s: fused statistics are an implicit-GEMM feature (see cgs_conv_stat_partials)", who);
     if (nstats && (!x.stat_part || fam != CGS_FAMILY_IGEMM)) return cgs_set_error(CGS_EINVAL, "%s: norm-backward statistics are a feature of the exact-fp32 implicit GEMM (see cgs_conv_stat_layout)", who);
+    if (x.form == FORM_UPDATE && (!x.up_mom || fam != CGS_FAMILY_IGEMM)) return cgs_set_error(CGS_EINVAL, "%s: the fused update is a feature of the exact-fp32 implicit GEMM (see cgs_conv_update_form)", who);
     if (x.sign_out && fam != CGS_FAMILY_IGEMM && fam != CGS_FAMILY_IGEMM_BX6) return cgs_set_error(CGS_EINVAL, "%s: this call cannot leave a sign mask (see cgs_conv_signs_ok)", who);
     if (x.aux_signs && fam != CGS_FAMILY_PATCH && fam != CGS_FAMILY_TAPS) return cgs_set_error(CGS_EINVAL, "%s: this call cannot take a sign mask (see cgs_conv_signs_ok)", who);
     if (((uintptr_t)x.sign_out & 3) || ((uintptr_t)x.aux_signs & 3)) return cgs_set_error(CGS_EINVAL, "%s: sign mask must be 4-byte aligned", who);
@@ -159,6 +161,7 @@
     p.in = in; p.bias = bias; p.ep_a = ep_a; p.ep_b = ep_b; p.ep_aux = ep_aux; p.out = out;
     p.stat_part = x.stat_part;
     if (nstats) { p.ns_mean = x.ns.mean; p.ns_inv = x.ns.invstd; p.ns_gamma = x.ns.gamma; p.ns_beta = x.ns.beta; p.ns_leak = x.ns.leak; p.ns_gimg = x.ns.group_images >= B ? 0 : x.ns.group_images; }
+    if (x.form == FORM_UPDATE) { p.up_mom = x.up_mom; p.up_rate = x.up_rate; p.up_alpha = x.up_alpha; p.up_first = x.up_first; }
     p.sign_out = x.sign_out;
     p.sign_plane = (long)B * (dirT ? L.Hb * L.Wb : L.Hs * L.Ws);
     const bool bx6 = fam == CGS_FAMILY_IGEMM_BX6;
@@ -175,6 +178,7 @@
     const size_t chunk = images_per_launch(p), in_img = in_image_floats(p), out_img = out_image_floats(p);
     if (chunk < 1) return cgs_set_error(CGS_EINVAL, "%s: one image exceeds 2 GiB", who);
     if (x.stat_part && !whole_batch_in_one_launch(p)) return cgs_set_error(CGS_EINVAL, "%s: fused statistics need the batch in one launch", who);
+    if (p.up_mom && !whole_batch_in_one_launch(p)) return cgs_set_error(CGS_EINVAL, "%s: the fused update needs the batch in one launch", who);
     for (size_t b0 = 0; b0 < (size_t)B; b0 += chunk) {
         p.B = (int)(B - b0 < chunk ? B - b0 : chunk);
         p.in = in + b0 * in_img;
@@ -234,6 +238,11 @@
         const size_t need = (size_t)G * 2 * (c.bwd ? Cin : Cout) * sizeof(float);
         if (!x.stat_part || x.stat_part_bytes < need) return cgs_set_error(CGS_EWORKSPACE, "%s: partials buffer %zu < %zu bytes", who, x.stat_part_bytes, need);
         if ((uintptr_t)x.stat_part & 15) return cgs_set_error(CGS_EINVAL, "%s: partials buffer must be 16-byte aligned", who);
+    }
+    if (x.form == FORM_UPDATE) {
+        if (!cgs_conv_update_form(op, B, H, W, Cin, Ho, Wo, Cout, kh, kw, sh, sw, ws_bytes, nullptr))
+            return cgs_set_error(CGS_EINVAL, "%s: not available for this call (cgs_conv_update_form == 0)", who);
+        if (!out || !x.up_mom || (((uintptr_t)out | (uintptr_t)x.up_mom) & 15)) return cgs_set_error(CGS_EINVAL, "%s: theta and m must be 16-byte aligned tensors", who);
     }
     return run_dir(c, B, in, w, bias, out, epilogue, ep_a, ep_b, ep_aux, ws, ws_bytes, prepacked, (hipStream_t)stream, who, x);
 }
@@ -321,6 +330,20 @@
     return (int)(cls_rows * p.nclasses);
 }
 
+int cgs_conv_update_form(int op, int B, int H, int W, int Cin, int Ho, int Wo, int Cout, int kh, int kw, int sh, int sw, size_t ws_bytes,
+                         int* row_order) {
+    if (row_order) *row_order = 0;
+    if (op != CGS_CONV_BWD_DATA && op != CGS_DECONV_BWD_DATA) return 0;
+    const ConvPlan q = conv_plan_of(op, B, H, W, Cin, Ho, Wo, Cout, kh, kw, sh, sw, CGS_EPI_NONE, ws_bytes);
+    if (q.fam != CGS_FAMILY_IGEMM || check_layer(q.c.L, "conv_update_form")) return 0;
+    if (q.c.dirT && (sh > 2 || sw > 2)) return 0;
+    if (!whole_batch_in_one_launch(q.g)) return 0;
+    const size_t packed = cgs_packed_floats(q.g) * sizeof(float);
+    if (ws_bytes < packed) return 0;
+    if (row_order) *row_order = cgs_igemm_row_order(q.g);
+    return cgs_igemm_update_form(q.g, ws_bytes - packed);
+}
+
 int cgs_conv_signs_ok(int op, int B, int H, int W, int Cin, int Ho, int Wo, int Cout, int kh, int kw, int sh, int sw, int epilogue,
                       size_t ws_bytes) {
     const ConvPlan q = conv_plan_of(op, B, H, W, Cin, Ho, Wo, Cout, kh, kw, sh, sw, epilogue, ws_bytes);
@@ -393,6 +416,24 @@
     return conv_entry("deconv2d_nhwc_bwd_data_nstats", CGS_DECONV_BWD_DATA, dy, w, nullptr, dx, B, H, W, Cin, Ho, Wo, Cout, kh, kw, sh, sw, CGS_EPI_NONE, nullptr,
                       nullptr, x_norm, ws, ws_bytes, ws_prepacked, stream, ConvExtras{FORM_NSTATS, stat_part, stat_part_bytes, NsArgs{mean, invstd, gamma, beta,
                       leak, group_images}});
+}
+
+int cgs_conv2d_nhwc_bwd_data_update(const float* dy, const float* w, float* theta, float* m, int B, int H, int W, int Cin, int Cout, int kh,
+                                    int kw, int sh, int sw, float rate, float alpha, int first, void* ws, size_t ws_bytes, int ws_prepacked,
+                                    void* stream) {
+    ConvExtras x;
+    x.form = FORM_UPDATE; x.up_mom = m; x.up_rate = rate; x.up_alpha = alpha; x.up_first = first ? 1 : 0;
+    return conv_entry("conv2d_nhwc_bwd_data_update", CGS_CONV_BWD_DATA, dy, w, nullptr, theta, B, H, W, Cin, 0, 0, Cout, kh, kw, sh, sw, CGS_EPI_NONE, nullptr,
+                      nullptr, nullptr, ws, ws_bytes, ws_prepacked, stream, x);
+}
+
+int cgs_deconv2d_nhwc_bwd_data_update(const float* dy, const float* w, float* theta, float* m, int B, int H, int W, int Cin, int Ho, int Wo,
+                                      int Cout, int kh, int kw, int sh, int sw, float rate, float alpha, int first, void* ws, size_t ws_bytes,
+                                      int ws_prepacked, void* stream) {
+    ConvExtras x;
+    x.form = FORM_UPDATE; x.up_mom = m; x.up_rate = rate; x.up_alpha = alpha; x.up_first = first ? 1 : 0;
+    return conv_entry("deconv2d_nhwc_bwd_data_update", CGS_DECONV_BWD_DATA, dy, w, nullptr, theta, B, H, W, Cin, Ho, Wo, Cout, kh, kw, sh, sw, CGS_EPI_NONE,
+                      nullptr, nullptr, nullptr, ws, ws_bytes, ws_prepacked, stream, x);
 }
 
 int cgs_deconv2d_nhwc_fwd_signs(const float* x, const float* w, const float* bias, float* y, int B, int H, int W, int Cin,
diff --git a/collaborative-gan-sampling_amd/csrc/cgs_internal.h b/collaborative-gan-sampling_amd/csrc/cgs_internal.h
--- a/collaborative-gan-sampling_amd/csrc/cgs_internal.h
+++ b/collaborative-gan-sampling_amd/csrc/cgs_internal.h
@@ -79,6 +79,9 @@
     const float* ns_beta = nullptr;
     float ns_leak = 1.f;
     int ns_gimg = 0;
+    float* up_mom = nullptr;
+    float up_rate = 0.f, up_alpha = 0.f;
+    int up_first = 0;
     int vec;
     int prio_t[3];
     int tail_from, tail_n, tail_s;
@@ -108,6 +111,7 @@
 int cgs_pack_weights_bx6(const IgemmParams& p, const CgsLayer& L, bool dirT, const float* w, void* packed, hipStream_t s);
 int cgs_igemm_bx6_launch(const IgemmParams& p, hipStream_t s);
 int cgs_contraction_mode();
+int cgs_igemm_update_form(const IgemmParams& p, size_t slab_bytes);
 int cgs_igemm_row_order(const IgemmParams& p);
 size_t cgs_convt_quad_ws_floats_bound(int kh, int kw, int Cs);
 int cgs_convt_taps_ok(const CgsLayer& L);
@@ -172,6 +176,17 @@
     const float c = fminf(fmaxf(avg + 0.5f, 0.f), 10000.f);
     la.gain[b] = c * c;
 }
+__device__ __forceinline__ void refine_update1(float g, float rate, float alpha, int first, int use_clip, float vmin, float vmax, float& theta,
+                                               float& m) {
+#pragma clang fp contract(off)
+    const float lg = rate * g;
+    const float am = alpha * m;
+    const float mv = first ? lg : am + lg;
+    m = mv;
+    float t = theta - mv;
+    if (use_clip) t = fminf(fmaxf(t, vmin), vmax);
+    theta = t;
+}
 #endif
 
 
diff --git a/collaborative-gan-sampling_amd/csrc/elementwise.hip b/collaborative-gan-sampling_amd/csrc/elementwise.hip
--- a/collaborative-gan-sampling_amd/csrc/elementwise.hip
+++ b/collaborative-gan-sampling_amd/csrc/elementwise.hip
@@ -294,14 +294,10 @@
 __global__ __launch_bounds__(256) void refine_update_kernel(float* __restrict__ theta, float* __restrict__ m,
                                                             const float* __restrict__ g, float rate, float alpha,
                                                             int first, int use_clip, float vmin, float vmax, size_t n) {
-#pragma clang fp contract(off)
-    GRID_STRIDE(i, n) {
-        const float lg = rate * g[i];
-        const float am = alpha * m[i];
-        const float mv = first ? lg : am + lg;
+    GRID_STRIDE(i, n) {
+        float t = theta[i], mv = m[i];
+        refine_update1(g[i], rate, alpha, first, use_clip, vmin, vmax, t, mv);
         m[i] = mv;
-        float t = theta[i] - mv;
-        if (use_clip) t = fminf(fmaxf(t, vmin), vmax);
         theta[i] = t;
     }
 }
diff --git a/collaborative-gan-sampling_amd/csrc/igemm.hip b/collaborative-gan-sampling_amd/csrc/igemm.hip
--- a/collaborative-gan-sampling_amd/csrc/igemm.hip
+++ b/collaborative-gan-sampling_amd/csrc/igemm.hip
@@ -98,8 +98,9 @@
     return CGS_OK;
 }
 
-template <int BM, int BN, int NW, bool VEC, int TBK, bool PAR, bool NS>
+template <int BM, int BN, int NW, bool VEC, int TBK, bool PAR, bool NS, bool UP = false>
 __device__ __forceinline__ void igemm_body(const IgemmParams& p) {
+    static_assert(!(NS && UP), "one twin per launch");
     constexpr int BK = TBK;
     constexpr int LDA = BK + 4;
     constexpr int NT = 64 * NW;
@@ -643,7 +644,9 @@
             __builtin_amdgcn_fence(__ATOMIC_ACQUIRE, "wavefront");
             if (n < p.N) {
                 const int* rp = rowpix + wm * (BM / WM) + ph * ER;
-                if constexpr (NS) {
+                if constexpr (UP) {
+                    epilogue_rows_update<ER, RPP, LDE, ((VEC && TBK == 32) ? 4 : 2)>(p, E, rp, rsub, c4, n, bias);
+                } else if constexpr (NS) {
                     const int mw = min(m0 + wm * (BM / WM), M - 1);
                     const int grp = p.ns_gimg <= 0 ? 0 : (p.pix_major ? (mw % p.B) : (mw / RC)) / p.ns_gimg;
                     const NsLane ns = ns_lane_params(p, grp, n);
@@ -683,6 +686,7 @@
         }
         return;
     }
+    if constexpr (UP) return;
 #pragma unroll
     for (int tn = 0; tn < TN; ++tn) {
         const int n = n0 + wn * WTN + tn * 32 + j;
@@ -711,7 +715,10 @@
 __global__ __launch_bounds__(64 * NW, 2) void igemm_kernel(IgemmParams p) { igemm_body<BM, BN, NW, VEC, TBK, PAR, false>(p); }
 template <int BM, int BN, int NW, bool VEC, int TBK, bool PAR>
 __global__ __launch_bounds__(64 * NW, 2) void igemm_ns_kernel(IgemmParams p) { igemm_body<BM, BN, NW, VEC, TBK, PAR, true>(p); }
-
+template <int BM, int BN, int NW, bool VEC, int TBK, bool PAR>
+__global__ __launch_bounds__(64 * NW, 2) void igemm_up_kernel(IgemmParams p) { igemm_body<BM, BN, NW, VEC, TBK, PAR, false, true>(p); }
+
+template <bool UP>
 __global__ __launch_bounds__(256) void splitk_reduce_kernel(IgemmParams p) {
     const IgemmClass& c = p.cls[blockIdx.y];
     const int RC = c.R * c.C;
@@ -738,6 +745,19 @@
         if (p.pix_major) { rem = m / p.B; b = m - rem * p.B; } else { b = m / RC; rem = m - b * RC; }
         r = rem / c.C; cc = rem - r * c.C;
         const size_t o = (size_t)((b * p.Hout + r * p.So + c.py) * p.Wout + cc * p.So + c.px) * p.N;
+        if constexpr (UP) {
+            if (n >= p.N) continue;
+            f32x4 t = *(const f32x4*)(p.out + o + n), mv = *(const f32x4*)(p.up_mom + o + n);
+#pragma unroll
+            for (int e = 0; e < 4; ++e) {
+                float te = t[e], me = mv[e];
+                refine_update1(a[e] + (p.bias ? p.bias[n + e] : 0.f), p.up_rate, p.up_alpha, p.up_first, 0, 0.f, 0.f, te, me);
+                t[e] = te; mv[e] = me;
+            }
+            *(f32x4*)(p.up_mom + o + n) = mv;
+            *(f32x4*)(p.out + o + n) = t;
+            continue;
+        }
 #pragma unroll
         for (int e = 0; e < 4; ++e) {
             if (n + e >= p.N) break;
@@ -804,6 +824,7 @@
 }
 
 #define TAIL_RSPLIT 16
+template <bool UP>
 __global__ __launch_bounds__(256) void tail_reduce_kernel(IgemmParams p, int BM, int BN) {
     const int cls_i = p.nclasses - 1;
     const IgemmClass& c = p.cls[cls_i];
@@ -846,6 +867,18 @@
         if (p.pix_major) { rem = m / p.B; b = m - rem * p.B; } else { b = m / RC; rem = m - b * RC; }
         const int r = rem / c.C, cc = rem - r * c.C;
         const size_t o = (size_t)((b * p.Hout + r * p.So + c.py) * p.Wout + cc * p.So + c.px) * p.N + n;
+        if constexpr (UP) {
+            f32x4 t = *(const f32x4*)(p.out + o), mv = *(const f32x4*)(p.up_mom + o);
+#pragma unroll
+            for (int e = 0; e < 4; ++e) {
+                float te = t[e], me = mv[e];
+                refine_update1(a[e] + bias[e], p.up_rate, p.up_alpha, p.up_first, 0, 0.f, 0.f, te, me);
+                t[e] = te; mv[e] = me;
+            }
+            *(f32x4*)(p.up_mom + o) = mv;
+            *(f32x4*)(p.out + o) = t;
+            continue;
+        }
         f32x4 aux = {0.f, 0.f, 0.f, 0.f};
         if (p.epilogue >= CGS_EPI_RELU_BWD_AFFINE) aux = *(const f32x4*)(p.ep_aux + o);
         f32x4 y;
@@ -1009,9 +1042,32 @@
     return n * sizeof(float);
 }
 
-template <int BM, int BN, int NW, bool VEC, int TBK, bool PAR, bool NS>
+int cgs_igemm_update_form(const IgemmParams& p_in, size_t slab_bytes) {
+    IgemmParams p = p_in;
+    if (!p.vec || (p.N & 3) || p.epilogue != CGS_EPI_NONE || p.bias || p.stat_part || p.sign_out) return 0;
+    p.splitk = 1; p.slab = nullptr;
+    p.tail_from = p.tail_n = p.tail_s = 0;
+    cgs_igemm_row_policy(p, 128);
+    const size_t need = cgs_igemm_splitk_bytes(p);
+    if (need && slab_bytes >= need) return CGS_UPDATE_SPLITK;
+    IgemmTiles tiles = igemm_choose_tiles(p);
+    IgemmTail tl = igemm_choose_tail(p, tiles);
+    bool tail_fits = tl.s > 1 && slab_bytes >= igemm_tail_bytes(tl, tiles.wide);
+    if (tiles.wide_for_tail && !tail_fits) {
+        tiles = igemm_choose_tiles(p, false);
+        tl = igemm_choose_tail(p, tiles);
+        tail_fits = tl.s > 1 && slab_bytes >= igemm_tail_bytes(tl, tiles.wide);
+    }
+    if (tiles.tall) return 0;
+    return tail_fits ? CGS_UPDATE_TAIL : CGS_UPDATE_EPILOGUE;
+}
+
+template <int BM, int BN, int NW, bool VEC, int TBK, bool PAR, int TW>
 static int launch_cfg(const IgemmParams& p, hipStream_t s) {
-    void (*const kern)(IgemmParams) = NS ? igemm_ns_kernel<BM, BN, NW, VEC, TBK, PAR> : igemm_kernel<BM, BN, NW, VEC, TBK, PAR>;
+    void (*kern)(IgemmParams);
+    if constexpr (TW == 2) kern = igemm_up_kernel<BM, BN, NW, VEC, TBK, PAR>;
+    else if constexpr (TW == 1) kern = igemm_ns_kernel<BM, BN, NW, VEC, TBK, PAR>;
+    else kern = igemm_kernel<BM, BN, NW, VEC, TBK, PAR>;
     constexpr int EH = (VEC && TBK == 16) ? 2 : 1;
     constexpr int WM = BM / 64;
     constexpr size_t kloop_f = (size_t)2 * BM * (TBK + 4) + 2 * TBK * BN, stage_f = (size_t)NW * (BM / WM / EH) * (BN / (NW / WM) + 4);
@@ -1053,7 +1109,8 @@
     hipLaunchKernelGGL(kern, dim3((unsigned)gx, gy, p.splitk > 1 ? p.splitk : 1), dim3(64 * NW), smem, s, q);
     CGS_CHECK_LAUNCH("igemm");
     if (p.tail_s > 1) {
-        hipLaunchKernelGGL(tail_reduce_kernel, dim3((unsigned)p.tail_n, TAIL_RSPLIT), dim3(256), 0, s, q, BM, BN);
+        if (p.up_mom) hipLaunchKernelGGL(tail_reduce_kernel<true>, dim3((unsigned)p.tail_n, TAIL_RSPLIT), dim3(256), 0, s, q, BM, BN);
+        else hipLaunchKernelGGL(tail_reduce_kernel<false>, dim3((unsigned)p.tail_n, TAIL_RSPLIT), dim3(256), 0, s, q, BM, BN);
         CGS_CHECK_LAUNCH("tail_reduce");
     }
     if (p.splitk > 1) {
@@ -1061,11 +1118,12 @@
         for (int i = 0; i < p.nclasses; ++i) { long t = (long)p.B * p.cls[i].R * p.cls[i].C * (p.Np / 4); if (t > tot) tot = t; }
         unsigned rb = (unsigned)((tot + 63) / 64 > 4096 ? 4096 : (tot + 63) / 64);
         if (p.stat_part) hipLaunchKernelGGL(splitk_reduce_stats_kernel, dim3((unsigned)p.stat_cls_rows, (unsigned)((p.N + 31) / 32), p.nclasses), dim3(256), 0, s, p);
-        else hipLaunchKernelGGL(splitk_reduce_kernel, dim3(rb, p.nclasses), dim3(256), 0, s, p);
+        else if (p.up_mom) hipLaunchKernelGGL(splitk_reduce_kernel<true>, dim3(rb, p.nclasses), dim3(256), 0, s, p);
+        else hipLaunchKernelGGL(splitk_reduce_kernel<false>, dim3(rb, p.nclasses), dim3(256), 0, s, p);
         CGS_CHECK_LAUNCH("splitk_reduce");
     }
     static char name[64];
-    snprintf(name, sizeof(name), "%s<%d, %d, %d, %s, %d, %s>", NS ? "igemm_ns_kernel" : "igemm_kernel", BM, BN, NW, VEC ? "true" : "false", TBK, PAR ? "true" : "false");
+    snprintf(name, sizeof(name), "%s<%d, %d, %d, %s, %d, %s>", TW == 2 ? "igemm_up_kernel" : TW == 1 ? "igemm_ns_kernel" : "igemm_kernel", BM, BN, NW, VEC ? "true" : "false", TBK, PAR ? "true" : "false");
     cgs_note_kernel(name);
     return CGS_OK;
 }
@@ -1214,13 +1272,21 @@
     p.uni = !(p.nclasses > 1 && wide && maxRC <= 64);
     bool half = vec && wide && deep && p.splitk > 1 && !p.tap_parity && (long)p.B * maxRC <= 64;
     const bool ns = p.stat_part && p.ns_mean;
-#define LC(...) (ns ? launch_cfg<__VA_ARGS__, true>(p, s) : launch_cfg<__VA_ARGS__, false>(p, s))
+    if (p.up_mom) {
+        const int form = p.splitk > 1 ? CGS_UPDATE_SPLITK : (p.tail_s > 1 ? CGS_UPDATE_TAIL : CGS_UPDATE_EPILOGUE);
+        if (!vec || tall || cgs_igemm_update_form(p_in, slab ? slab_bytes : 0) != form)
+            return cgs_set_error(CGS_EINVAL, "igemm: the fused update is not offered for this launch (cgs_conv_update_form)");
+    }
+    const bool upk = p.up_mom && p.splitk == 1;
+#define LC(...) (ns ? launch_cfg<__VA_ARGS__, 1>(p, s) : launch_cfg<__VA_ARGS__, 0>(p, s))
+#define LCU(...) (upk ? launch_cfg<__VA_ARGS__, 2>(p, s) : LC(__VA_ARGS__))
     if (half) return LC(64, 128, 4, true, 32, false);
     if (tall) return p.tap_parity ? LC(256, 64, 4, true, 16, true) : LC(256, 64, 4, true, 16, false);
-    if (vec && !deep && !p.tap_parity) return wide ? LC(128, 128, 4, true, 16, false) : LC(128, 64, 4, true, 16, false);
-    if (vec && !deep && p.tap_parity) return wide ? LC(128, 128, 4, true, 16, true) : LC(128, 64, 4, true, 16, true);
-    if (vec && p.tap_parity) return wide ? LC(128, 128, 4, true, 32, true) : LC(128, 64, 4, true, 32, true);
-    if (vec) return wide ? LC(128, 128, 4, true, 32, false) : LC(128, 64, 4, true, 32, false);
+    if (vec && !deep && !p.tap_parity) return wide ? LCU(128, 128, 4, true, 16, false) : LCU(128, 64, 4, true, 16, false);
+    if (vec && !deep && p.tap_parity) return wide ? LCU(128, 128, 4, true, 16, true) : LCU(128, 64, 4, true, 16, true);
+    if (vec && p.tap_parity) return wide ? LCU(128, 128, 4, true, 32, true) : LCU(128, 64, 4, true, 32, true);
+    if (vec) return wide ? LCU(128, 128, 4, true, 32, false) : LCU(128, 64, 4, true, 32, false);
     return wide ? LC(128, 128, 4, false, 16, false) : LC(128, 64, 4, false, 16, false);
+#undef LCU
 #undef LC
 }
diff --git a/collaborative-gan-sampling_amd/csrc/igemm_epilogue.h b/collaborative-gan-sampling_amd/csrc/igemm_epilogue.h
--- a/collaborative-gan-sampling_amd/csrc/igemm_epilogue.h
+++ b/collaborative-gan-sampling_amd/csrc/igemm_epilogue.h
@@ -101,3 +101,42 @@
         }
     }
 }
+
+template <int ROWS, int RPP, int LDE, int UPU>
+__device__ __forceinline__ void epilogue_rows_update(const IgemmParams& p, const float* E, const int* rowpix_tile, int rsub, int c4, int n,
+                                                     f32x4 bias) {
+    constexpr int ITERS = ROWS / RPP;
+    static_assert(ITERS % UPU == 0, "row groups");
+    const float rate = p.up_rate, alpha = p.up_alpha;
+    const int first = p.up_first;
+#pragma unroll
+    for (int it0 = 0; it0 < ITERS; it0 += UPU) {
+        f32x4 th[UPU], mo[UPU];
+        int pixs[UPU];
+#pragma unroll
+        for (int u = 0; u < UPU; ++u) {
+            pixs[u] = rowpix_tile[(it0 + u) * RPP + rsub];
+            th[u] = mo[u] = f32x4{0.f, 0.f, 0.f, 0.f};
+            if (pixs[u] >= 0) {
+                const size_t o = (size_t)pixs[u] * p.N + n;
+                th[u] = *(const f32x4*)(p.out + o);
+                mo[u] = *(const f32x4*)(p.up_mom + o);
+            }
+        }
+#pragma unroll
+        for (int u = 0; u < UPU; ++u) {
+            if (pixs[u] < 0) continue;
+            const f32x4 v = *(const f32x4*)(E + ((it0 + u) * RPP + rsub) * LDE + c4);
+            f32x4 t = th[u], m = mo[u];
+#pragma unroll
+            for (int e = 0; e < 4; ++e) {
+                float te = t[e], me = m[e];
+                refine_update1(v[e] + bias[e], rate, alpha, first, 0, 0.f, 0.f, te, me);
+                t[e] = te; m[e] = me;
+            }
+            const size_t o = (size_t)pixs[u] * p.N + n;
+            *(f32x4*)(p.up_mom + o) = m;
+            *(f32x4*)(p.out + o) = t;
+        }
+    }
+}
diff --git a/collaborative-gan-sampling_amd/engine.py b/collaborative-gan-sampling_amd/engine.py
--- a/collaborative-gan-sampling_amd/engine.py
+++ b/collaborative-gan-sampling_amd/engine.py
@@ -66,13 +66,22 @@
             return K.conv2d_fwd_stats(x, self.w, self.b, self.part, self.s, self.s, out=self.out)
         return K.conv2d_fwd(x, self.w, self.b, self.s, self.s, self.epi, out=self.out)
 
-    def bwd(self, dy):
+    def update_form(self):
+        if self.bwd_epi[0] != L.EPI_NONE or self.bwd_nstat is not None:
+            return None
+        B, H, W, Cin = self.dx.shape
+        kh, kw, _, Cout = self.w.shape
+        return K.conv_update_form(L.CONV_BWD_DATA, B, H, W, Cin, 0, 0, Cout, kh, kw, self.s, self.s)
+
+    def bwd(self, dy, update=None):
         if not self.pre_folded:
             if self.epi == L.EPI_LRELU:
                 dy = K.lrelu_bwd(dy, self.out, out=dy)
             elif self.epi == L.EPI_TANH:
                 dy = K.tanh_bwd(dy, self.out, out=dy)
         e, a, aux = self.bwd_epi
+        if update is not None:
+            return K.conv2d_bwd_data(dy, self.w, self.in_hw, self.s, self.s, update=update)
         return K.conv2d_bwd_data(dy, self.w, self.in_hw, self.s, self.s, out=self.dx, epilogue=e, ep_a=a, ep_aux=aux, nstat=self.bwd_nstat)
 
 
@@ -102,13 +111,20 @@
         return K.deconv2d_fwd(x, self.w, self.b, self.out_hw, self.s, self.s, self.epi, self.a, self.c, out=self.out, signs=self.signs,
                               part=self.part)
 
-    def bwd(self, dy):
+    def update_form(self):
+        if self.bwd_epi[0] != L.EPI_NONE or self.bwd_nstat is not None or self.bwd_signs is not None:
+            return None
+        return K.conv_update_form(L.DECONV_BWD_DATA, *self.call_dims(), self.s, self.s)
+
+    def bwd(self, dy, update=None):
         if not self.pre_folded:
             if self.epi == L.EPI_AFFINE_RELU:
                 dy = K.affine_relu_bwd(dy, self.out, self.a, out=dy)
             elif self.epi == L.EPI_TANH:
                 dy = K.tanh_bwd(dy, self.out, out=dy)
         e, a, aux = self.bwd_epi
+        if update is not None:
+            return K.deconv2d_bwd_data(dy, self.w, self.in_hw, self.s, self.s, update=update)
         return K.deconv2d_bwd_data(dy, self.w, self.in_hw, self.s, self.s, out=self.dx, epilogue=e, ep_a=a, ep_aux=aux,
                                    ep_signs=self.bwd_signs, nstat=self.bwd_nstat)
 
@@ -418,9 +434,6 @@
         below.pre_folded = True
 
 
-NSTAT_MAX_BYTES = 48 * 2 ** 20
-
-
 def link_norm_backward_stats(stages, B):
     for below, above in zip(stages[:-1], stages[1:]):
         if isinstance(below, _Residual):
@@ -434,8 +447,6 @@
         else:
             continue
         C = below.out.shape[-1]
-        if below.out.numel() * 4 > NSTAT_MAX_BYTES:
-            continue
         if isinstance(above, _Conv):
             H, W, Cin = above.dx.shape[1:]
             kh, kw, _, Cout = above.w.shape
@@ -461,10 +472,10 @@
             x = st.fwd(x)
         return x
 
-    def backward(self, dy):
-        for st in reversed(self.stages):
+    def backward(self, dy, update=None):
+        for st in reversed(self.stages[1:]):
             dy = st.bwd(dy)
-        return dy
+        return self.stages[0].bwd(dy) if update is None else self.stages[0].bwd(dy, update=update)
 
 
 def _entry(fn):
@@ -559,6 +570,9 @@
                     drop_partials(st.inner)
         drop_partials(self.d.stages); drop_partials(self.g_tail.stages)
         link_norm_backward_stats(self.g_tail.stages + self.d.stages, B)
+        first = self.g_tail.stages[0]
+        self.update_form = first.update_form() if isinstance(first, (_Conv, _Deconv)) else None
+        self.fused_update = self.update_form is not None and self.update_form[0] != "tail"
 
     def _sync_weights(self):
         if self._ws_epoch != K.WS.epoch:
@@ -656,8 +670,8 @@
             K.refine_loss_seed(logits, loss, self.dlogits, logit_out, ladam, first)
         return logits
 
-    def backward_to_feature(self):
-        return self.g_tail.backward(self.d.backward(self.dlogits))
+    def backward_to_feature(self, update=None):
+        return self.g_tail.backward(self.d.backward(self.dlogits), update=update)
 
     @_entry
     def compute_forward_logits_and_grad(self, feature, loss="bce"):
@@ -678,7 +692,13 @@
         self.best_step.fill_(1.0)
         self.tickets.zero_()
         forced = self.forced if probabilistic else None
+        fused = self.fused_update and self.update_form is not None and ladam is None and not (vmin and vmax)
         for i in range(steps):
+            if fused:
+                self.backward_to_feature(update=K.FusedUpdate(th, self.mom, rate, alpha, first=(i == 0)))
+                self.forward_logits(th, self.logit, loss, ladam, False)
+                K.refine_select2(render, self.images, th, self.best_theta, self.logit, forced, i, self.best_logit, self.best_step, self.tickets)
+                continue
             g = self.backward_to_feature()
             if ladam is None:
                 K.refine_update(th, self.mom, g, rate, alpha, first=(i == 0), vmin=vmin, vmax=vmax)
@@ -722,7 +742,7 @@
                     self.mean_square = torch.empty_like(self.mom)
                 ladam = self._ladam
                 ladam.set_real(real_sigmoid_mean)
-            key = (steps, float(rate), alpha, prob, vmin, vmax, loss, method)
+            key = (steps, float(rate), alpha, prob, vmin, vmax, loss, method, bool(self.fused_update))
             if not self.use_graph:
                 self._program(steps, rate, alpha, prob, vmin, vmax, loss, ladam)
             else:
diff --git a/collaborative-gan-sampling_amd/kernels.py b/collaborative-gan-sampling_amd/kernels.py
--- a/collaborative-gan-sampling_amd/kernels.py
+++ b/collaborative-gan-sampling_amd/kernels.py
@@ -249,11 +249,47 @@
         return (_ptr(self.x), _ptr(self.mean), _ptr(self.invstd), _ptr(self.gamma), _ptr(self.beta), self.leak, self.group_images)
 
 
-def conv2d_bwd_data(dy, w, in_hw, sh=2, sw=2, out=None, epilogue=L.EPI_NONE, ep_a=None, ep_aux=None, nstat=None):
+class FusedUpdate:
+    __slots__ = ("theta", "m", "rate", "alpha", "first")
+
+    def __init__(self, theta, m, rate, alpha, first):
+        self.theta, self.m, self.rate, self.alpha, self.first = _chk(theta, "theta"), _chk(m, "m"), float(rate), float(alpha), bool(first)
+
+    def args(self):
+        return (self.rate, self.alpha, 1 if self.first else 0)
+
+
+UPDATE_FORMS = {0: None, 1: "epilogue", 2: "splitk", 3: "tail"}
+
+
+def conv_update_form(op, B, H, W, Cin, Ho, Wo, Cout, kh, kw, sh, sw):
+    import ctypes as C
+    _, nbytes = WS.plan(op, B, H, W, Cin, Ho, Wo, Cout, kh, kw, sh, sw, L.EPI_NONE)
+    order = C.c_int(0)
+    form = int(L.load().cgs_conv_update_form(op, B, H, W, Cin, Ho, Wo, Cout, kh, kw, sh, sw, nbytes, C.addressof(order)))
+    return (UPDATE_FORMS[form], order.value) if form > 0 else None
+
+
+def _update_nbytes(dy, w, update):
+    return _nb(dy, w, update.theta, update.theta, update.m) + (0.0 if update.first else _nb(update.m))
+
+
+def conv2d_bwd_data(dy, w, in_hw, sh=2, sw=2, out=None, epilogue=L.EPI_NONE, ep_a=None, ep_aux=None, nstat=None, update=None):
     _chk(dy, "dy"); _chk(w, "w")
     kh, kw, Cin, Cout = w.shape
     B = dy.shape[0]
     H, W = in_hw
+    if update is not None:
+        if epilogue != L.EPI_NONE or nstat is not None or tuple(update.theta.shape) != (B, H, W, Cin) or update.m.shape != update.theta.shape:
+            raise L.CgsError("conv2d_bwd_data: the fused update comes with no epilogue, on theta and m of the gradient's shape")
+        ws, pre = WS.get(w, L.CONV_BWD_DATA, kh, kw, sh, sw, Cin, Cout, (B, H, W), epilogue, ptrs=(_ptr(dy), _ptr(update.theta), _ptr(update.m)))
+        pr = _Prof(2.0 * B * dy.shape[1] * dy.shape[2] * Cout * kh * kw * Cin, f"conv_bwd {H}x{W} {Cin}<-{Cout}",
+                   _update_nbytes(dy, w, update)) if PROFILE is not None else None
+        L.call("cgs_conv2d_nhwc_bwd_data_update", _ptr(dy), _ptr(w), _ptr(update.theta), _ptr(update.m), B, H, W, Cin, Cout, kh, kw, sh, sw,
+               *update.args(), _ptr(ws), ws.numel() * 4, pre, _stream())
+        if pr is not None:
+            pr.done()
+        return None
     dx = out if out is not None else torch.empty((B, H, W, Cin), dtype=torch.float32, device=dy.device)
     ws, pre = WS.get(w, L.CONV_BWD_DATA, kh, kw, sh, sw, Cin, Cout, (B, H, W), epilogue,
                      ptrs=(_ptr(dy), _ptr(dx), _ptr(ep_a), _ptr(ep_aux)))
@@ -305,11 +341,23 @@
     return y
 
 
-def deconv2d_bwd_data(dy, w, in_hw, sh=2, sw=2, out=None, epilogue=L.EPI_NONE, ep_a=None, ep_aux=None, ep_signs=None, nstat=None):
+def deconv2d_bwd_data(dy, w, in_hw, sh=2, sw=2, out=None, epilogue=L.EPI_NONE, ep_a=None, ep_aux=None, ep_signs=None, nstat=None, update=None):
     _chk(dy, "dy"); _chk(w, "w")
     kh, kw, Cout, Cin = w.shape
     B, Ho, Wo, _ = dy.shape
     H, W = in_hw
+    if update is not None:
+        if epilogue != L.EPI_NONE or nstat is not None or ep_signs is not None or tuple(update.theta.shape) != (B, H, W, Cin) \
+                or update.m.shape != update.theta.shape:
+            raise L.CgsError("deconv2d_bwd_data: the fused update comes with no epilogue, on theta and m of the gradient's shape")
+        ws, pre = WS.get(w, L.DECONV_BWD_DATA, kh, kw, sh, sw, Cin, Cout, (B, H, W), epilogue, (Ho, Wo),
+                         ptrs=(_ptr(dy), _ptr(update.theta), _ptr(update.m)))
+        pr = _Prof(2.0 * B * H * W * Cin * kh * kw * Cout, f"deconv_bwd {H}x{W} {Cin}<-{Cout}", _update_nbytes(dy, w, update)) if PROFILE is not None else None
+        L.call("cgs_deconv2d_nhwc_bwd_data_update", _ptr(dy), _ptr(w), _ptr(update.theta), _ptr(update.m), B, H, W, Cin, Ho, Wo, Cout, kh, kw,
+               sh, sw, *update.args(), _ptr(ws), ws.numel() * 4, pre, _stream())
+        if pr is not None:
+            pr.done()
+        return None
     dx = out if out is not None else torch.empty((B, H, W, Cin), dtype=torch.float32, device=dy.device)
     ws, pre = WS.get(w, L.DECONV_BWD_DATA, kh, kw, sh, sw, Cin, Cout, (B, H, W), epilogue, (Ho, Wo),
                      ptrs=(_ptr(dy), _ptr(dx), _ptr(ep_a), _ptr(ep_aux)))
diff --git a/collaborative-gan-sampling_amd/lib.py b/collaborative-gan-sampling_amd/lib.py
--- a/collaborative-gan-sampling_amd/lib.py
+++ b/collaborative-gan-sampling_amd/lib.py
@@ -48,6 +48,9 @@
     "cgs_conv2d_nhwc_bwd_data": (_i, [_p] * 3 + [_i] * 9 + [_i, _p, _p, _p, _z, _i, _p]),
     "cgs_deconv2d_nhwc_fwd": (_i, [_p] * 4 + [_i] * 11 + [_i, _p, _p, _p, _z, _i, _p]),
     "cgs_deconv2d_nhwc_bwd_data": (_i, [_p] * 3 + [_i] * 11 + [_i, _p, _p, _p, _z, _i, _p]),
+    "cgs_conv_update_form": (_i, [_i] * 12 + [_z, _p]),
+    "cgs_conv2d_nhwc_bwd_data_update": (_i, [_p] * 4 + [_i] * 9 + [_f, _f, _i, _p, _z, _i, _p]),
+    "cgs_deconv2d_nhwc_bwd_data_update": (_i, [_p] * 4 + [_i] * 11 + [_f, _f, _i, _p, _z, _i, _p]),
     "cgs_conv_signs_ok": (_i, [_i] * 13 + [_z]),
     "cgs_deconv2d_nhwc_fwd_signs": (_i, [_p] * 4 + [_i] * 11 + [_i, _p, _p, _p, _p, _z, _i, _p]),
     "cgs_deconv2d_nhwc_bwd_data_signs": (_i, [_p] * 3 + [_i] * 11 + [_i, _p, _p, _p, _z, _i, _p]),
diff --git a/include/cgs_hip.h b/include/cgs_hip.h
--- a/include/cgs_hip.h
+++ b/include/cgs_hip.h
@@ -112,6 +112,20 @@
                                int B, int H, int W, int Cin, int Ho, int Wo, int Cout, int kh, int kw, int sh, int sw,
                                int epilogue, const float* ep_a, const float* ep_aux,
                                void* ws, size_t ws_bytes, int ws_prepacked, void* stream);
+
+#define CGS_UPDATE_EPILOGUE 1
+#define CGS_UPDATE_SPLITK 2
+#define CGS_UPDATE_TAIL 3
+int cgs_conv_update_form(int op, int B, int H, int W, int Cin, int Ho, int Wo, int Cout, int kh, int kw, int sh, int sw,
+                         size_t ws_bytes, int* row_order);
+int cgs_conv2d_nhwc_bwd_data_update(const float* dy, const float* w, float* theta, float* m,
+                                    int B, int H, int W, int Cin, int Cout, int kh, int kw, int sh, int sw,
+                                    float rate, float alpha, int first,
+                                    void* ws, size_t ws_bytes, int ws_prepacked, void* stream);
+int cgs_deconv2d_nhwc_bwd_data_update(const float* dy, const float* w, float* theta, float* m,
+                                      int B, int H, int W, int Cin, int Ho, int Wo, int Cout, int kh, int kw, int sh, int sw,
+                                      float rate, float alpha, int first,
+                                      void* ws, size_t ws_bytes, int ws_prepacked, void* stream);
 
 int cgs_conv_signs_ok(int op, int B, int H, int W, int Cin, int Ho, int Wo, int Cout, int kh, int kw, int sh, int sw,
                       int epilogue, size_t ws_bytes);
```

Result: faster. 6719 samples/s (median of 6 runs) (+1.2%).
